# payakorn/InteriorPointMethod

Hardware: AMD Instinct MI355X
Metric: IPM iterations/sec (m=4096,n=8192 dense LP) (higher is better)
Workload: dtype f64; 1 GPU; dense synthetic LP m=4096 n=8192 fp64, seed 0, start x=s=1 y=0 (BASELINE.json configs[1]); replicas per GPU

## Files before the change

### include/ipm_hip.h

```cpp
#ifndef IPM_HIP_H
#define IPM_HIP_H

#include <stddef.h>
#include <stdint.h>

#ifdef __cplusplus
extern "C" {
#endif

#define IPM_ABI_VERSION 4

enum {
    IPM_OK = 0,
    IPM_ERR_INVALID_ARG = -1,
    IPM_ERR_HIP = -2,
    IPM_ERR_NO_DEVICE = -3,
    IPM_ERR_WORKSPACE = -4,
    IPM_ERR_STATE = -5,
    IPM_ERR_INVALID_INPUT = -6,
    IPM_ERR_SINGULAR = -7
};

enum {
    IPM_STATUS_RUNNING = 0,
    IPM_STATUS_CONVERGED = 1,
    IPM_STATUS_MAX_ITER = 2,
    IPM_STATUS_NAN = 3,
    IPM_STATUS_PRIMAL_INFEASIBLE = 5,
    IPM_STATUS_DUAL_INFEASIBLE = 6
};

enum {
    IPM_FLAG_NO_DEVICE_POLLING = 1,
    IPM_FLAG_NO_AUTO_REGULARIZE = 2,
    IPM_FLAG_SINGLE_STREAM = 4,
    IPM_FLAG_SPARSE_FACTOR = 8,
    IPM_FLAG_LOCKSTEP = 16,
    IPM_FLAG_DETECT_INFEASIBILITY = 32
};

typedef struct ipm_handle ipm_handle;

typedef struct ipm_options {
    double eta;
    double pivot_guard_eps;
    double pivot_guard_big;
    int32_t check_every;
    int32_t flags;
    int64_t sparse_nnz;
    double regularize;
} ipm_options;

typedef struct ipm_stats {
    int32_t status;
    int32_t iterations;
    int32_t pivots_fixed;
    int32_t auto_regularized;
    double objective;
    double rp_norm;
    double rd_norm;
    double gap;
    double b_norm, c_norm;
    double mu, mu_aff, sigma;
    double alpha_aff_p, alpha_aff_d;
    double alpha_p, alpha_d;
    double solve_ms;
    double objective_last_finite;
} ipm_stats;

typedef struct ipm_iter_record {
    int32_t k;
    int32_t pivots_fixed;
    double objective, rp_norm, rd_norm, gap, mu, sigma;
    double alpha_aff_p, alpha_aff_d, alpha_p, alpha_d;
} ipm_iter_record;
#define IPM_HISTORY_CAPACITY 1024

int ipm_abi_version(void);
int ipm_device_count(int* count);
void ipm_default_options(ipm_options* opts);

int ipm_workspace_bytes(int64_t m, int64_t n, size_t* bytes);
int ipm_workspace_bytes_csc(int64_t m, int64_t n, int64_t nnz, size_t* bytes);
int ipm_workspace_bytes_opts(int64_t m, int64_t n, const ipm_options* opts, size_t* bytes);

int ipm_create(int device, int64_t m, int64_t n, const ipm_options* opts,
               void* workspace, size_t workspace_bytes, void* stream, ipm_handle** out);
int ipm_destroy(ipm_handle* h);
const char* ipm_last_error(const ipm_handle* h);

int ipm_set_A_dense(ipm_handle* h, const double* A, int64_t ld, int is_device);
int ipm_set_A_csc(ipm_handle* h, const int32_t* colptr, const int32_t* rowind,
                  const double* val, int64_t nnz);
int ipm_set_bc(ipm_handle* h, const double* b, const double* c);

int ipm_set_state(ipm_handle* h, const double* x, const double* y, const double* s);
int ipm_get_state(ipm_handle* h, double* x, double* y, double* s);
int ipm_init_state(ipm_handle* h, double y0);
int ipm_init_state_mehrotra(ipm_handle* h, int32_t* pivots_fixed);

int ipm_set_bounds(ipm_handle* h, const double* u);
int ipm_set_bound_state(ipm_handle* h, const double* w, const double* z);
int ipm_get_bound_state(ipm_handle* h, double* w, double* z);

int ipm_equilibrate(ipm_handle* h, int32_t max_passes, double info[4]);
int ipm_get_scaling(ipm_handle* h, double* r, double* c);

int ipm_newton_direction(ipm_handle* h, int corrector, double* dx, double* dy, double* ds,
                         ipm_stats* stats);

int ipm_iterate(ipm_handle* h, int32_t n_steps, ipm_stats* stats);
int ipm_solve(ipm_handle* h, double tol_p, double tol_d, double tol_gap, int32_t max_iter,
              ipm_stats* stats);
int ipm_solve_batch(ipm_handle** handles, int32_t n, double tol_p, double tol_d, double tol_gap, int32_t max_iter, ipm_stats* stats);
typedef struct ipm_batch ipm_batch;
int ipm_batch_create(int device, void* stream, ipm_batch** out);
int ipm_batch_destroy(ipm_batch* b);
const char* ipm_batch_last_error(const ipm_batch* b);
int ipm_batch_add(ipm_batch* b, ipm_handle* h, double tol_p, double tol_d, double tol_gap, int32_t max_iter, int32_t* index);
int ipm_batch_step(ipm_batch* b, int32_t* finished, int32_t cap, int32_t* n_finished, int32_t* n_active);
int ipm_batch_stats(ipm_batch* b, int32_t index, ipm_stats* stats);
int ipm_solve_small_batch(ipm_handle** handles, int32_t n, double tol_p, double tol_d, double tol_gap, int32_t max_iter, void* stream,
                          ipm_stats* stats);
int ipm_init_small_batch_mehrotra(ipm_handle** handles, int32_t n, void* stream, int32_t* pivots_fixed);
int ipm_set_infeasibility_tol(ipm_handle* h, double eps_p, double eps_d);
int ipm_get_certificate(ipm_handle* h, double* y, double* z, double* x, double info[4]);
int ipm_get_history(ipm_handle* h, ipm_iter_record* out, int32_t capacity, int32_t* count);
int ipm_get_schedule(ipm_handle* h, int32_t out[12]);

int ipm_order_rows(int64_t m, int64_t n, const int32_t* colptr, const int32_t* rowind, int32_t* perm, double info[8]);
int ipm_get_factor_info(ipm_handle* h, int64_t out[8]);

int ipm_solve_linear(ipm_handle* h, const double* B, int64_t ldb, const double* rhs, double* z,
                     int32_t* pivots_fixed);
int ipm_lu_solve(int device, int64_t n, const double* A, int64_t lda, int64_t nrhs, const double* B, int64_t ldb,
                 double* X, int64_t ldx, int64_t* info);
int ipm_lu_factor(int device, int64_t n, const double* A, int64_t lda, double* LU, int64_t ldlu, int32_t* ipiv,
                  int64_t* info);
int ipm_normal_solve(ipm_handle* h, const double* d, const double* rhs, double* z, int reuse_factor,
                     int32_t* pivots_fixed);
int ipm_form_normal_matrix(ipm_handle* h, const double* d, double* B, int64_t ldb);
int ipm_get_factor(ipm_handle* h, double* L, int64_t ldl);
int ipm_set_profiling(ipm_handle* h, int enable);
int ipm_debug_get_stamps(ipm_handle* h, long long* out);
int ipm_debug_ff_schedule(int32_t nblk, int32_t q, int32_t workers, unsigned char* items, int32_t capacity, int32_t* count,
                          int32_t* tile_items, double sim_us[2]);
int ipm_get_phase_ms(ipm_handle* h, double out[4]);
int ipm_debug_get_block_inverse(ipm_handle* h, int32_t k, double* out);
int ipm_debug_ff_trace(ipm_handle* h, long long* out, int64_t capacity, int64_t* count, unsigned char* items, int32_t* nitems);
int ipm_debug_ls_merge(int32_t n, const int32_t* off, const int32_t* types_flat, int32_t max_group, int32_t aligned,
                       int32_t* out_steps, int32_t cap_steps, int32_t* out_members);

#ifdef __cplusplus
}
#endif
#endif
```

### interiorpointmethod_amd/_lib.py

```python
from __future__ import annotations

import ctypes as C
import os

_HERE = os.path.dirname(os.path.abspath(__file__))
LIB_PATH = os.path.join(_HERE, "libipm_hip.so")

EXPORTS = [
    "ipm_abi_version", "ipm_device_count", "ipm_default_options", "ipm_workspace_bytes", "ipm_workspace_bytes_csc", "ipm_workspace_bytes_opts",
    "ipm_create", "ipm_destroy", "ipm_last_error", "ipm_set_A_dense", "ipm_set_A_csc",
    "ipm_set_bc", "ipm_set_state", "ipm_get_state", "ipm_init_state", "ipm_init_state_mehrotra", "ipm_set_bounds", "ipm_set_bound_state", "ipm_get_bound_state", "ipm_equilibrate", "ipm_get_scaling", "ipm_newton_direction",
    "ipm_iterate", "ipm_solve", "ipm_solve_batch", "ipm_solve_small_batch", "ipm_init_small_batch_mehrotra", "ipm_batch_create", "ipm_batch_destroy", "ipm_batch_last_error", "ipm_batch_add", "ipm_batch_step", "ipm_batch_stats", "ipm_get_history", "ipm_set_infeasibility_tol", "ipm_get_certificate", "ipm_get_schedule", "ipm_order_rows", "ipm_get_factor_info", "ipm_solve_linear", "ipm_lu_solve", "ipm_lu_factor", "ipm_normal_solve", "ipm_form_normal_matrix", "ipm_get_factor",
    "ipm_set_profiling", "ipm_get_phase_ms", "ipm_debug_get_stamps", "ipm_debug_ff_schedule", "ipm_debug_ff_trace", "ipm_debug_get_block_inverse", "ipm_debug_ls_merge",
]

IPM_OK = 0
STATUS_RUNNING, STATUS_CONVERGED, STATUS_MAX_ITER, STATUS_NAN = 0, 1, 2, 3
STATUS_PRIMAL_INFEASIBLE, STATUS_DUAL_INFEASIBLE = 5, 6
FLAG_NO_DEVICE_POLLING = 1
FLAG_NO_AUTO_REGULARIZE = 2
FLAG_SINGLE_STREAM = 4
FLAG_SPARSE_FACTOR = 8
FLAG_LOCKSTEP = 16
FLAG_DETECT_INFEASIBILITY = 32
ERR_WORKSPACE = -4
ABI_VERSION = 4
HISTORY_CAPACITY = 1024
ERR_INVALID_INPUT = -6
ERR_SINGULAR = -7


class IpmLibraryError(RuntimeError):
    """libipm_hip.so is missing or does not export the ABI."""


class IpmError(RuntimeError):
    def __init__(self, code, msg):
        super().__init__("libipm_hip status %d: %s" % (code, msg))
        self.code = code


class Options(C.Structure):
    _fields_ = [("eta", C.c_double), ("pivot_guard_eps", C.c_double), ("pivot_guard_big", C.c_double),
                ("check_every", C.c_int32), ("flags", C.c_int32), ("sparse_nnz", C.c_int64),
                ("regularize", C.c_double)]


class Stats(C.Structure):
    _fields_ = [("status", C.c_int32), ("iterations", C.c_int32), ("pivots_fixed", C.c_int32),
                ("auto_regularized", C.c_int32), ("objective", C.c_double), ("rp_norm", C.c_double),
                ("rd_norm", C.c_double), ("gap", C.c_double), ("b_norm", C.c_double),
                ("c_norm", C.c_double), ("mu", C.c_double), ("mu_aff", C.c_double),
                ("sigma", C.c_double), ("alpha_aff_p", C.c_double), ("alpha_aff_d", C.c_double),
                ("alpha_p", C.c_double), ("alpha_d", C.c_double), ("solve_ms", C.c_double),
                ("objective_last_finite", C.c_double)]

    def as_dict(self):
        return {k: getattr(self, k) for k, _ in self._fields_}


class IterRecord(C.Structure):
    _fields_ = [("k", C.c_int32), ("pivots_fixed", C.c_int32), ("objective", C.c_double), ("rp_norm", C.c_double),
                ("rd_norm", C.c_double), ("gap", C.c_double), ("mu", C.c_double), ("sigma", C.c_double),
                ("alpha_aff_p", C.c_double), ("alpha_aff_d", C.c_double), ("alpha_p", C.c_double),
                ("alpha_d", C.c_double)]


_lib = None


def load():
    global _lib
    if _lib is not None:
        return _lib
    try:
        import torch
    except ImportError:
        pass
    if not os.path.exists(LIB_PATH):
        raise IpmLibraryError(
            "%s not found: the HIP extension has not been built. Build it with "
            "`python -c 'import __graft_entry__ as g; g.build()'` (needs hipcc). "
            "There is no CPU fallback." % LIB_PATH)
    try:
        lib = C.CDLL(LIB_PATH)
    except OSError as e:
        raise IpmLibraryError("cannot load %s: %s" % (LIB_PATH, e)) from e
    missing = [s for s in EXPORTS if not hasattr(lib, s)]
    if missing:
        raise IpmLibraryError("%s lacks symbols %s" % (LIB_PATH, missing))
    vp, i32, i64, dbl = C.c_void_p, C.c_int32, C.c_int64, C.c_double
    pd = C.POINTER(C.c_double)
    lib.ipm_abi_version.restype = C.c_int
    lib.ipm_device_count.argtypes = [C.POINTER(C.c_int)]
    lib.ipm_default_options.argtypes = [C.POINTER(Options)]
    lib.ipm_default_options.restype = None
    lib.ipm_workspace_bytes.argtypes = [i64, i64, C.POINTER(C.c_size_t)]
    lib.ipm_workspace_bytes_csc.argtypes = [i64, i64, i64, C.POINTER(C.c_size_t)]
    lib.ipm_workspace_bytes_opts.argtypes = [i64, i64, C.POINTER(Options), C.POINTER(C.c_size_t)]
    lib.ipm_create.argtypes = [C.c_int, i64, i64, C.POINTER(Options), vp, C.c_size_t, vp, C.POINTER(vp)]
    lib.ipm_destroy.argtypes = [vp]
    lib.ipm_last_error.argtypes = [vp]
    lib.ipm_last_error.restype = C.c_char_p
    lib.ipm_set_A_dense.argtypes = [vp, vp, i64, C.c_int]
    lib.ipm_set_A_csc.argtypes = [vp, C.POINTER(i32), C.POINTER(i32), pd, i64]
    lib.ipm_set_bc.argtypes = [vp, pd, pd]
    lib.ipm_set_state.argtypes = [vp, pd, pd, pd]
    lib.ipm_get_state.argtypes = [vp, pd, pd, pd]
    lib.ipm_init_state.argtypes = [vp, dbl]
    lib.ipm_init_state_mehrotra.argtypes = [vp, C.POINTER(i32)]
    lib.ipm_set_bounds.argtypes = [vp, pd]
    lib.ipm_set_bound_state.argtypes = [vp, pd, pd]
    lib.ipm_get_bound_state.argtypes = [vp, pd, pd]
    lib.ipm_equilibrate.argtypes = [vp, i32, pd]
    lib.ipm_get_scaling.argtypes = [vp, pd, pd]
    lib.ipm_newton_direction.argtypes = [vp, C.c_int, pd, pd, pd, C.POINTER(Stats)]
    lib.ipm_iterate.argtypes = [vp, i32, C.POINTER(Stats)]
    lib.ipm_solve.argtypes = [vp, dbl, dbl, dbl, i32, C.POINTER(Stats)]
    lib.ipm_solve_batch.argtypes = [C.POINTER(vp), i32, dbl, dbl, dbl, i32, C.POINTER(Stats)]
    lib.ipm_solve_small_batch.argtypes = [C.POINTER(vp), i32, dbl, dbl, dbl, i32, vp, C.POINTER(Stats)]
    lib.ipm_init_small_batch_mehrotra.argtypes = [C.POINTER(vp), i32, vp, C.POINTER(i32)]
    lib.ipm_batch_create.argtypes = [C.c_int, vp, C.POINTER(vp)]
    lib.ipm_batch_destroy.argtypes = [vp]
    lib.ipm_batch_last_error.argtypes = [vp]
    lib.ipm_batch_last_error.restype = C.c_char_p
    lib.ipm_batch_add.argtypes = [vp, vp, dbl, dbl, dbl, i32, C.POINTER(i32)]
    lib.ipm_batch_step.argtypes = [vp, C.POINTER(i32), i32, C.POINTER(i32), C.POINTER(i32)]
    lib.ipm_batch_stats.argtypes = [vp, i32, C.POINTER(Stats)]
    lib.ipm_get_history.argtypes = [vp, C.POINTER(IterRecord), i32, C.POINTER(i32)]
    lib.ipm_get_schedule.argtypes = [vp, C.POINTER(i32)]
    lib.ipm_set_infeasibility_tol.argtypes = [vp, dbl, dbl]
    lib.ipm_get_certificate.argtypes = [vp, pd, pd, pd, pd]
    lib.ipm_order_rows.argtypes = [i64, i64, C.POINTER(i32), C.POINTER(i32), C.POINTER(i32), pd]
    lib.ipm_get_factor_info.argtypes = [vp, C.POINTER(i64)]
    lib.ipm_solve_linear.argtypes = [vp, pd, i64, pd, pd, C.POINTER(i32)]
    lib.ipm_lu_solve.argtypes = [C.c_int, i64, pd, i64, i64, pd, i64, pd, i64, C.POINTER(i64)]
    lib.ipm_lu_factor.argtypes = [C.c_int, i64, pd, i64, pd, i64, C.POINTER(i32), C.POINTER(i64)]
    lib.ipm_normal_solve.argtypes = [vp, pd, pd, pd, C.c_int, C.POINTER(i32)]
    lib.ipm_form_normal_matrix.argtypes = [vp, pd, pd, i64]
    lib.ipm_get_factor.argtypes = [vp, pd, i64]
    lib.ipm_set_profiling.argtypes = [vp, C.c_int]
    lib.ipm_get_phase_ms.argtypes = [vp, pd]
    lib.ipm_debug_get_stamps.argtypes = [vp, C.POINTER(C.c_longlong)]
    lib.ipm_debug_ff_schedule.argtypes = [i32, i32, i32, C.POINTER(C.c_ubyte), i32, C.POINTER(i32), C.POINTER(i32), pd]
    lib.ipm_debug_get_block_inverse.argtypes = [vp, i32, pd]
    lib.ipm_debug_ff_trace.argtypes = [vp, C.POINTER(C.c_longlong), i64, C.POINTER(i64), C.POINTER(C.c_ubyte), C.POINTER(i32)]
    lib.ipm_debug_ls_merge.argtypes = [i32, C.POINTER(i32), C.POINTER(i32), i32, i32, C.POINTER(i32), i32, C.POINTER(i32)]
    for name in EXPORTS:
        fn = getattr(lib, name)
        if name not in ("ipm_default_options", "ipm_last_error", "ipm_batch_last_error"):
            fn.restype = C.c_int
    _lib = lib
    return lib


def check(handle, code):
    if code != IPM_OK:
        msg = load().ipm_last_error(handle)
        raise IpmError(code, (msg or b"").decode("utf-8", "replace"))


def device_count():
    n = C.c_int(0)
    load().ipm_device_count(C.byref(n))
    return n.value
```

### interiorpointmethod_amd/csrc/handoff.h

```cpp
#pragma once
#include <hip/hip_runtime.h>

namespace ipm {

__device__ unsigned ipm_spin_limit = 1u << 22;

enum { HD_COUNT = 0, HD_TAG, HD_KIND, HD_TARGET, HD_SEEN, HD_WORDS = 8 };
enum HandoffKind : unsigned {
    HK_FCOUNT = 1,
    HK_TPROG = 2,
    HK_LFINAL_ROW = 3,
    HK_LFINAL_COL = 4,
    HK_POTRFDONE = 5,
    HK_ROLES = 6,
    HK_GEMM = 6,
    HK_POTRF = 7,
    HK_DCOUNT = 8,
};

__device__ __forceinline__ unsigned handoff_load(const unsigned* p) { return __hip_atomic_load(p, __ATOMIC_RELAXED, __HIP_MEMORY_SCOPE_AGENT); }

struct HandoffSink { unsigned* timeout; unsigned* dbg; };
template <int SLEEP, bool NULL_OK, class Ready, class Record>
__device__ __forceinline__ bool handoff_wait(Ready ready, HandoffSink sink, Record record) {
    unsigned* const timeout = sink.timeout; unsigned* const dbg = sink.dbg;
    unsigned spins = 0;
    bool ok = true;
    while (!ready()) {
        __builtin_amdgcn_s_sleep(SLEEP);
        ++spins;
        if (spins > ipm_spin_limit || ((spins & 1023u) == 1u && (!NULL_OK || timeout) && handoff_load(timeout))) {
            if (spins > ipm_spin_limit && dbg && __hip_atomic_fetch_add(dbg + HD_COUNT, 1u, __ATOMIC_RELAXED, __HIP_MEMORY_SCOPE_AGENT) == 0u) record();
            if (!NULL_OK || timeout) __hip_atomic_store(timeout, 1u, __ATOMIC_RELAXED, __HIP_MEMORY_SCOPE_AGENT);
            ok = false;
            break;
        }
    }
    return ok;
}

__device__ __forceinline__ void handoff_record_ge(unsigned* dbg, unsigned tag, unsigned kind, unsigned target, const unsigned* p) {
    dbg[HD_TAG] = tag; dbg[HD_KIND] = kind; dbg[HD_TARGET] = target; dbg[HD_SEEN] = handoff_load(p);
}

template <int SLEEP, bool NULL_OK>
__device__ __forceinline__ bool handoff_wait_ge(const unsigned* p, unsigned count, HandoffSink sink, unsigned tag, unsigned kind) {
    return handoff_wait<SLEEP, NULL_OK>([=] { return handoff_load(p) >= count; }, sink, [=] { handoff_record_ge(sink.dbg, tag, kind, count, p); });
}

template <bool WAIT = true>
__device__ __forceinline__ void handoff_acquire() {
    __builtin_amdgcn_fence(__ATOMIC_ACQUIRE, "agent");
    if (WAIT) asm volatile("s_waitcnt vmcnt(0)" ::: "memory");
}
__device__ __forceinline__ void handoff_acquire_barrier(bool polled) {
    if (polled) handoff_acquire();
    __syncthreads();
}

__device__ __forceinline__ void handoff_publish_begin() {
    asm volatile("s_waitcnt vmcnt(0)" ::: "memory");
    __syncthreads();
    if (threadIdx.x == 0) {
        __builtin_amdgcn_fence(__ATOMIC_RELEASE, "agent");
        asm volatile("s_waitcnt vmcnt(0)" ::: "memory");
    }
}

__device__ __forceinline__ bool handoff_skipped(const int* done, unsigned* signal) {
    if (done && *done) {
        if (signal && threadIdx.x == 0) __hip_atomic_fetch_add(signal, 1u, __ATOMIC_RELAXED, __HIP_MEMORY_SCOPE_AGENT);
        return true;
    }
    return false;
}

}
```

### interiorpointmethod_amd/csrc/host_factor_solve.h

```cpp
#pragma once
static inline bool sp_on(const ipm_handle* h) { return h->spf && !h->spf_off; }
static inline bool sp_level(const ipm_handle* h) {
    if (h->sp_serial || h->sp_level_mode < 0) return false;
    if (h->sp_level_mode > 0 || (h->opt.flags & IPM_FLAG_NO_DEVICE_POLLING)) return true;
    return !alone_on_device(h);
}
static inline unsigned sp_launch_grid(ipm_handle* h) {
    if (h->sp_serial) { ++h->sp_serial_launches; return 1u; }
    return (unsigned)h->sp_grid;
}
template <class Launch>
static void sp_walk(ipm_handle* h, bool by_level, bool leaves_first, Launch launch) {
    if (!by_level) { launch(sp_launch_grid(h), h->spF.rec, 0); return; }
    const size_t nlev = h->sp_lvlptr.empty() ? 0 : h->sp_lvlptr.size() - 1;
    for (size_t i = 0; i < nlev; ++i) {
        const size_t l = leaves_first ? i : nlev - 1 - i;
        const int cnt = h->sp_lvlptr[l + 1] - h->sp_lvlptr[l];
        launch((unsigned)std::min(cnt, h->sp_grid), h->sp_rec_level + h->sp_lvlptr[l], cnt);
    }
}

static int ensure_dense_B(ipm_handle* h) {
    if (h->B && h->invD) return IPM_OK;
    if (!h->no_dense) return fail(h, IPM_ERR_STATE, "handle has no dense normal-matrix buffer");
    if ((!h->B_own && dev_malloc(h->device, h->stream, (void**)&h->B_own, sizeof(double) * (size_t)h->mp * h->mp) != hipSuccess) ||
        (!h->invD_own && dev_malloc(h->device, h->stream, (void**)&h->invD_own, sizeof(double) * (size_t)h->nblk * NB * NB) != hipSuccess))
        return fail(h, IPM_ERR_HIP, "dense normal-matrix buffer (%lld x %lld doubles) could not be allocated", (long long)h->mp, (long long)h->mp);
    HIP_TRY(h, hipMemsetAsync(h->invD_own, 0, sizeof(double) * (size_t)h->nblk * NB * NB, h->stream));
    h->B = h->B_own; h->invD = h->invD_own;
    return IPM_OK;
}

static int enqueue_form(ipm_handle* h, const double* d, bool dense_image = false) {
    if (sp_on(h) && !dense_image) {
        hipLaunchKernelGGL(sp_form_kernel, dim3((unsigned)((h->sp_nslot + 255) / 256)), dim3(256), 0, h->stream, h->sp_fptr, h->sp_fcol,
                           h->sp_fcoef, h->sp_nslot, d, h->spF.L, &h->sc->maxdiag, &h->sc->done);
        hipLaunchKernelGGL(sp_maxdiag_kernel, dim3((unsigned)((h->m + 255) / 256)), dim3(256), 0, h->stream, h->spF.L, h->sp_diagpos, (int)h->m, &h->sc->maxdiag,
                           &h->sc->done);
        HIP_TRY(h, hipGetLastError());
        return IPM_OK;
    }
    if (int rc_ = ensure_dense_B(h)) return rc_;
    if (h->sparse && h->list_form) {
        const int64_t nB = h->mp * h->mp;
        const unsigned zgrid = (unsigned)std::min<int64_t>((nB / 2 + 255) / 256, 4096);
        launch_twin<LS_ZERO>(h, zgrid, {h->B, nB, &h->sc->done});
        const int work = h->sm_nb + (int)(h->mp - h->m);
        launch_twin<LS_ADAT_LIST>(h, (unsigned)((work + 255) / 256), {h->sm_bptr, h->ls_bi, h->ls_bk, h->sm_bcol, h->sm_bcoef, h->ls_bak, h->sm_nb, d, h->B, h->mp, (int)h->m, (int)h->mp, &h->sc->done});
        HIP_TRY(h, hipGetLastError());
        return IPM_OK;
    }
    if (h->sparse) {
        const LsAdatSp ps{sparse_view(h), d, h->B, h->mp, (int)h->mp, &h->sc->done};
        if (h->mp <= SP_LDS_MAX_MP) launch_twin<LS_ADAT_SPARSE>(h, (unsigned)h->mp, ps, nullptr, (unsigned)(h->mp * sizeof(double)));
        else launch_twin<LS_ADAT_SPARSE_GLOBAL>(h, (unsigned)h->mp, ps);
        HIP_TRY(h, hipGetLastError());
        return IPM_OK;
    }
    HIP_TRY(h, launch_adat_syrk(h->A, h->np, d, h->B, h->mp, (int)h->mp, (int)h->np, (int)h->m, factor_done(h),
                                h->d_tile_order, h->stream, h->slab, 512));
    return IPM_OK;
}

static int enqueue_group_inverses(ipm_handle* h, int g0 = 0, int g1 = -1, hipStream_t st = nullptr) {
    if (sp_on(h)) return IPM_OK;
    if (!h->grouped_trsv) return IPM_OK;
    const int GS = h->gsz;
    const int64_t GR = (int64_t)GS * 128;
    if (g1 < 0) g1 = h->nblk / GS;
    if (!st) st = h->stream;
    const int nG = g1 - g0;
    if (nG <= 0) return IPM_OK;
    const int* done = &h->sc->done;
    launch_twin<LS_GROUP_DIAG_T>(h, 16u * (unsigned)(nG * GS), {h->invD, h->gXT, h->gX, g0 * GS, GS, done}, st);
    const int64_t gXs = GR * GR, gL = GR * (h->mp + 1), gSs = (GR / 2) * (GR / 2);
    double* gXT = h->gXT + g0 * gXs; double* gX = h->gX + g0 * gXs; double* gS = h->gS + g0 * gSs;
    const double* Lg = h->B + g0 * gL;
    for (int hs = 128; hs < GR; hs *= 2) {
        const int np = (int)(GR / (2 * hs));
        GemmNT t = gemm_defaults();
        t.done = done;
        t.M = hs; t.N = hs; t.K = hs; t.batch = np; t.batch2 = nG;
        const int64_t pX = (int64_t)2 * hs * (GR + 1);
        const int64_t pL = (int64_t)2 * hs * (h->mp + 1);
        const int64_t pS = (int64_t)hs * hs;
        GemmNT a = t;
        a.P = gXT; a.ldp = GR; a.sP = pX; a.sP2 = gXs;
        a.Q = Lg + (int64_t)hs * h->mp; a.ldq = h->mp; a.sQ = pL; a.sQ2 = gL;
        a.C = gS; a.ldc = hs; a.sC = pS; a.sC2 = gSs;
        HIP_TRY(h, (launch_gemm_nt<32, 32, 32, 2, 2>(a, st)));
        GemmNT b = t;
        b.P = gX + (int64_t)hs * GR + hs; b.ldp = GR; b.sP = pX; b.sP2 = gXs;
        b.Q = gS; b.ldq = hs; b.sQ = pS; b.sQ2 = gSs;
        b.C = gX + (int64_t)hs * GR; b.ldc = GR; b.sC = pX; b.sC2 = gXs; b.alpha = -1.0;
        HIP_TRY(h, (launch_gemm_nt<32, 32, 32, 2, 2>(b, st)));
        GemmNT c = t;
        c.P = gS; c.ldp = hs; c.sP = pS; c.sP2 = gSs;
        c.Q = gX + (int64_t)hs * GR + hs; c.ldq = GR; c.sQ = pX; c.sQ2 = gXs;
        c.C = gXT + hs; c.ldc = GR; c.sC = pX; c.sC2 = gXs; c.alpha = -1.0;
        HIP_TRY(h, (launch_gemm_nt<32, 32, 32, 2, 2>(c, st)));
    }
    HIP_TRY(h, hipGetLastError());
    return IPM_OK;
}

static inline int potrf_panels(const ipm_handle* h, int k) {
    if (h->shift_rel != 0.0) return NB / 16;
    const int64_t real = h->m - (int64_t)k * NB;
    return real >= NB ? NB / 16 : (int)std::max<int64_t>(1, (real + 15) / 16);
}

static int enqueue_factor(ipm_handle* h, bool use_env = false, int mid_step = -1, int ginv_step = -1, const double* sp_fwd_rhs = nullptr) {
    if (sp_on(h)) {
        if (!h->sp_fuse_fwd) sp_fwd_rhs = nullptr;
        h->sp_fwd_fused = sp_fwd_rhs;
        const unsigned ep = ++h->sp_epoch;
        sp_walk(h, sp_level(h), true, [&](unsigned grid, const SpRec* recs, int count) {
            hipLaunchKernelGGL((sp_chol_kernel<SPC_THREADS>), dim3(grid), dim3(SPC_THREADS), h->sp_lds_chol, h->stream, h->spF, ep,
                               &h->sc->maxdiag, h->opt.pivot_guard_eps, h->opt.pivot_guard_big, h->shift_rel, &h->sc->fixed,
                               h->sp_lds_doubles, recs, count, sp_fwd_rhs, h->t2, h->sp_fv_off);
        });
        HIP_TRY(h, hipGetLastError());
        return IPM_OK;
    }
    if (int rc_ = ensure_dense_B(h)) return rc_;
    const int* done = factor_done(h);
    use_env = use_env && h->use_env;
    launch_twin<LS_MAXDIAG>(h, 1u, {h->B, h->mp, (int)h->m, &h->sc->maxdiag, done});
    const bool la = lookahead_on(h);
    int gs = 1;
    if (la && !use_env && h->two_level != 0) {
        if (h->group_steps > 0) gs = h->nblk >= 8 ? h->group_steps : 1;
        else if (h->nblk >= 96) gs = 4;
        else if (h->nblk >= 48) gs = 3;
    }
    std::vector<int> grp_lo(h->nblk), grp_hi(h->nblk);
    for (int k = 0; k < h->nblk; ++k) {
        if (gs > 1) { grp_lo[k] = (k / gs) * gs; grp_hi[k] = std::min(grp_lo[k] + gs, h->nblk); }
        else { grp_lo[k] = k; grp_hi[k] = k + 1; }
    }
    h->last_gs = gs;
    hipStream_t sm = h->stream, sb = la ? h->stream2 : h->stream;
    const bool fs = polls_device(h);
    h->n_counter_steps = 0; h->n_event_steps = 0;
    std::vector<unsigned> bulk_wgs(h->nblk, 0u);
    if (la) {
        if (fs) HIP_TRY(h, hipMemsetAsync(h->d_bulk_done, 0, sizeof(unsigned) * 2 * (size_t)h->nblk, sm));
        HIP_TRY(h, hipEventRecord(h->ev_fork, sm));
        HIP_TRY(h, hipStreamWaitEvent(sb, h->ev_fork, 0));
    }
    for (int k = 0; k < h->nblk; ++k) {
        PotrfDiag pd;
        pd.Bkk = h->B + (int64_t)k * NB * (h->mp + 1); pd.ld = h->mp;
        pd.inv = h->invD + (int64_t)k * NB * NB;
        pd.maxdiag = &h->sc->maxdiag; pd.eps = h->opt.pivot_guard_eps; pd.big = h->opt.pivot_guard_big; pd.shift_rel = h->shift_rel;
        pd.fixed = &h->sc->fixed; pd.done = done; pd.stamps = nullptr;
        pd.wait_on = nullptr; pd.wait_count = 0; pd.signal = nullptr; pd.timeout = nullptr; pd.dbg = nullptr; pd.dbg_tag = 0;
        pd.trace = nullptr;
        pd.nt = potrf_panels(h, k);
        pd.rows = (int)(h->m - (int64_t)k * NB);
        if (h->stamp_buf && k == 0) {
            pd.stamps = h->stamp_buf;
            if (getenv("IPM_POTRF_SKIP")) pd.dbg_tag = (unsigned)atoi(getenv("IPM_POTRF_SKIP"));
            launch_untwinned(h, potrf_diag_kernel<true>, dim3(1), dim3(PD_THREADS), sm, pd);
        } else launch_twin<LS_POTRF>(h, 1u, pd, sm);
        if (k == ginv_step) {
            HIP_TRY(h, hipEventRecord(h->ev_grp, sm));
            HIP_TRY(h, hipStreamWaitEvent(h->stream3, h->ev_grp, 0));
            int rc_ = enqueue_group_inverses(h, 0, (k + 1) / h->gsz, h->stream3);
            if (rc_) return rc_;
        }
        if (k == mid_step) { int rc_ = enqueue_residual_stream(h, sm); if (rc_) return rc_; }
        int rem = (int)(h->mp - (int64_t)(k + 1) * NB);
        if (rem <= 0) break;
        if (use_env) {
            rem = std::min(rem, (h->env_last[k] - k) * NB);
            if (rem <= 0) {
                if (la) HIP_TRY(h, hipEventRecord(h->ev_bulk[k], sb));
                continue;
            }
        }
        double* panel = h->B + (int64_t)(k + 1) * NB * h->mp + (int64_t)k * NB;
        GemmNT t = gemm_defaults();
        t.P = panel; t.ldp = h->mp; t.Q = pd.inv; t.ldq = NB;
        t.C = panel; t.ldc = h->mp; t.M = rem; t.N = NB; t.K = NB;
        t.lower = 0; t.done = done;
        GemmNT u = gemm_defaults();
        u.P = panel; u.ldp = h->mp; u.Q = panel; u.ldq = h->mp;
        u.C = h->B + (int64_t)(k + 1) * NB * (h->mp + 1); u.ldc = h->mp; u.M = rem; u.N = rem; u.K = NB;
        u.alpha = -1.0; u.beta = 1.0; u.lower = 1; u.done = done;
        if (!la) {
            if (rem <= h->ss_small_blocks * NB) {
                HIP_TRY(h, (launch_gemm_nt<32, 128, 32, 1, 8>(t, sm)));
                HIP_TRY(h, (launch_gemm_nt<64, 64, 16, 2, 2>(u, sm)));
                continue;
            }
            HIP_TRY(h, (launch_gemm_nt<64, 128, 16, 2, 2>(t, sm)));
            if (h->bulk_variant == 7) HIP_TRY(h, (launch_gemm_nt<128, 128, 16, 2, 2>(u, sm)));
            else HIP_TRY(h, launch_chol_update(u, sm));
            continue;
        }
        GemmNT tc = t; tc.M = NB;
        if (k >= 1) {
            if (bulk_wgs[k - 1] > 0) { tc.wait_on = h->d_bulk_done + (k - 1); tc.wait_count = bulk_wgs[k - 1]; tc.timeout = timeout_word(h); }
            else HIP_TRY(h, hipStreamWaitEvent(sm, h->ev_bulk[k - 1], 0));
        }
        const int tb_wgs = (rem - NB) / 64;
        const bool crit_flag = fs && rem > NB && tb_wgs <= 64;
        if (crit_flag) tc.signal = h->d_bulk_done + h->nblk + k;
        HIP_TRY(h, (launch_gemm_nt<32, 128, 32, 1, 8>(tc, sm)));
        if (!crit_flag) HIP_TRY(h, hipEventRecord(h->ev_crit[k], sm));
        const int g0 = grp_lo[k], gend = grp_hi[k];
        const bool grouped = gend - g0 > 1;
        const bool grp_inner = grouped && k + 1 < gend;
        const bool grp_last = grouped && !grp_inner;
        if (grp_last && k > g0) {
            u.P = panel - (int64_t)(k - g0) * NB; u.Q = u.P; u.K = (k - g0 + 1) * NB;
        }
        GemmNT uc = u; uc.M = NB; uc.N = NB;
        HIP_TRY(h, (launch_gemm_nt<32, 32, 32, 2, 2>(uc, sm)));
        if (!crit_flag) HIP_TRY(h, hipStreamWaitEvent(sb, h->ev_crit[k], 0));
        if (rem > NB) {
            GemmNT tb = t; tb.C = panel + (int64_t)NB * h->mp; tb.P = tb.C; tb.M = rem - NB;
            if (crit_flag) { tb.wait_on = h->d_bulk_done + h->nblk + k; tb.wait_count = NB / 32; tb.timeout = timeout_word(h); }
            HIP_TRY(h, (launch_gemm_nt<64, 128, 16, 2, 2>(tb, sb)));
            GemmNT ub = u;
            const int nt = rem / NB;
            if (grp_inner) {
                const int wn = gend - (k + 1);
                ub.P = panel + (int64_t)NB * h->mp; ub.Q = panel;
                ub.C = h->B + (int64_t)(k + 2) * NB * h->mp + (int64_t)(k + 1) * NB;
                ub.M = rem - NB; ub.N = std::min(wn * NB, rem); ub.lower = 0;
                if (fs) { bulk_wgs[k] = (unsigned)((ub.M / NB) * (ub.N / NB)); ub.signal = h->d_bulk_done + k; ++h->n_counter_steps; }
                else ++h->n_event_steps;
                if (h->bulk_variant == 7) HIP_TRY(h, (launch_gemm_nt<128, 128, 16, 2, 2>(ub, sb)));
                else HIP_TRY(h, launch_chol_update(ub, sb));
                HIP_TRY(h, hipEventRecord(h->ev_bulk[k], sb));
                continue;
            }
            const int ub_wgs = nt * (nt + 1) / 2 - 1;
            if (fs && ub_wgs <= 1024) {
                bulk_wgs[k] = (unsigned)ub_wgs;
                ub.signal = h->d_bulk_done + k;
                ++h->n_counter_steps;
            } else ++h->n_event_steps;
            if (h->bulk_variant == 7) HIP_TRY(h, (launch_gemm_nt<128, 128, 16, 2, 2>(ub, sb, nullptr, 512, 1)));
            else HIP_TRY(h, launch_chol_update(ub, sb, 1));
        }
        HIP_TRY(h, hipEventRecord(h->ev_bulk[k], sb));
    }
    if (la) HIP_TRY(h, hipStreamWaitEvent(sm, h->ev_bulk[h->nblk - 2], 0));
    HIP_TRY(h, hipGetLastError());
    return IPM_OK;
}

static void launch_dense_gemv_n(ipm_handle* h, const double* A, int64_t lda, int rows, int cols, const double* v, double sa,
                                double sb, const double* add, double* out) {
    launch_twin<LS_GEMV_N>(h, (unsigned)((rows + 3) / 4), {A, lda, rows, cols, v, sa, sb, add, out, &h->sc->done});
}

static void enqueue_block_steps(ipm_handle* h, int k0, double* r, double* z, double* out) {
    TrsvStep a;
    a.L = h->B; a.ld = h->mp; a.inv = h->invD; a.done = &h->sc->done;
    a.r = r; a.z = z; a.j0 = 0;
    for (int k = k0; k < h->nblk; ++k) {
        a.k = k;
        const int nb = h->use_env ? h->env_last[k] - k + 1 : h->nblk - k;
        launch_twin<LS_TRSV_FWD>(h, (unsigned)nb, a);
    }
    a.r = z; a.z = out;
    for (int k = h->nblk - 1; k >= k0; --k) {
        a.k = k;
        a.j0 = h->use_env ? h->env_first[k] : 0;
        launch_twin<LS_TRSV_BWD>(h, (unsigned)(k - a.j0 + 1), a);
    }
}

static int enqueue_potrs_grouped(ipm_handle* h, double* r, double* out, hipEvent_t wait_last = nullptr) {
    const int GS = h->gsz;
    const int GR = GS * 128;
    const int nG = h->nblk / GS;
    const int* done = &h->sc->done;
    double* z = h->t2;
    for (int g = 0; g < nG; ++g) {
        if (wait_last && g == nG - 1) HIP_TRY(h, hipStreamWaitEvent(h->stream, wait_last, 0));
        launch_dense_gemv_n(h, h->gX + (int64_t)g * GR * GR, GR, GR, GR, r + (int64_t)g * GR, 1.0, 0.0, nullptr, z + (int64_t)g * GR);
        int below = (int)(h->mp - (int64_t)(g + 1) * GR);
        if (h->use_env) below = std::min(below, (int)((int64_t)(h->env_last[(g + 1) * GS - 1] + 1) * NB - (int64_t)(g + 1) * GR));
        if (below > 0) {
            double* rb = r + (int64_t)(g + 1) * GR;
            launch_dense_gemv_n(h, h->B + (int64_t)(g + 1) * GR * h->mp + (int64_t)g * GR, h->mp, below, GR, z + (int64_t)g * GR, -1.0, 1.0,
                                rb, rb);
        }
    }
    enqueue_block_steps(h, nG * GS, r, z, out);
    for (int g = nG - 1; g >= 0; --g) {
        launch_dense_gemv_n(h, h->gXT + (int64_t)g * GR * GR, GR, GR, GR, z + (int64_t)g * GR, 1.0, 0.0, nullptr, out + (int64_t)g * GR);
        int left = g * GR;
        const int c0 = h->use_env ? std::min(left, h->env_first[g * GS] * NB) : 0;
        left -= c0;
        if (left > 0) {
            const unsigned gx = (unsigned)((left + 511) / 512);
            launch_twin<LS_GEMV_T>(h, gx * 16u, {h->B + (int64_t)g * GR * h->mp + c0, h->mp, GR / 16, left, out + (int64_t)g * GR, h->gPart, done, gx});
            launch_twin<LS_SUB_PARTIALS>(h, (unsigned)((left + 255) / 256), {z + c0, h->gPart, left, 16, done});
        }
    }
    HIP_TRY(h, hipGetLastError());
    return IPM_OK;
}

static int enqueue_potrs(ipm_handle* h, double* r, double* out, hipEvent_t wait_last = nullptr) {
    if (sp_on(h)) {
        const int rm = std::max(16, h->sp_rmax);
        unsigned ep = ++h->sp_epoch;
        const bool fwd_done = h->sp_fwd_fused != nullptr && h->sp_fwd_fused == r;
        h->sp_fwd_fused = nullptr;
        const bool by_level = sp_level(h);
        if (!fwd_done) sp_walk(h, by_level, true, [&](unsigned grid, const SpRec* recs, int count) {
            hipLaunchKernelGGL((sp_fwd_kernel<SPC_THREADS>), dim3(grid), dim3(SPC_THREADS), h->sp_lds_solve, h->stream, h->spF, ep, r, h->t2, rm, recs, count);
        });
        if (!by_level) ep = ++h->sp_epoch;
        sp_walk(h, by_level, false, [&](unsigned grid, const SpRec* recs, int count) {
            hipLaunchKernelGGL((sp_bwd_kernel<SPC_THREADS>), dim3(grid), dim3(SPC_THREADS), 0, h->stream, h->spF, ep, h->t2, out, recs, count);
        });
        HIP_TRY(h, hipGetLastError());
        return IPM_OK;
    }
    if (h->grouped_trsv) return enqueue_potrs_grouped(h, r, out, wait_last);
    if (wait_last) HIP_TRY(h, hipStreamWaitEvent(h->stream, wait_last, 0));
    enqueue_block_steps(h, 0, r, h->t2, out);
    HIP_TRY(h, hipGetLastError());
    return IPM_OK;
}

static int enqueue_mehrotra_start(ipm_handle* h) {
    int rc;
    const unsigned gn = (unsigned)((h->n + 255) / 256);
    hipLaunchKernelGGL(fill_kernel, dim3(gn), dim3(256), 0, h->stream, h->d, (int)h->n, 1.0);
    if ((rc = enqueue_form(h, h->d))) return rc;
    if ((rc = enqueue_factor(h, true))) return rc;
    if ((rc = enqueue_group_inverses(h))) return rc;
    const VecArgs va = vec_args(h);
    const dim3 g(h->vblk), b(VBLK);
    HIP_TRY(h, hipMemcpyAsync(h->t1, h->b, sizeof(double) * h->mp, hipMemcpyDeviceToDevice, h->stream));
    if ((rc = enqueue_potrs(h, h->t1, h->dy))) return rc;
    launch_gemv_t(h, h->dy);
    if (h->bnd) hipLaunchKernelGGL(start_primal_bounded_kernel, g, b, 0, h->stream, va, bnd_args(h));
    else hipLaunchKernelGGL(start_primal_kernel, g, b, 0, h->stream, va);
    launch_gemv_n(h, h->c, 1.0, 0.0, nullptr, h->t1);
    if ((rc = enqueue_potrs(h, h->t1, h->dy))) return rc;
    launch_gemv_t(h, h->dy);
    if (h->bnd) {
        const BndArgs bd = bnd_args(h);
        hipLaunchKernelGGL(start_dual_bounded_kernel, g, b, 0, h->stream, va, bd);
        hipLaunchKernelGGL(start_shift_bounded_kernel, g, b, 0, h->stream, va, bd);
        hipLaunchKernelGGL(start_primal_correct_bounded_kernel, g, b, 0, h->stream, va, bd);
        hipLaunchKernelGGL(start_dual_correct_bounded_kernel, g, b, 0, h->stream, va, bd);
    } else {
        hipLaunchKernelGGL(start_dual_kernel, g, b, 0, h->stream, va);
        hipLaunchKernelGGL(start_shift_kernel, g, b, 0, h->stream, va);
        hipLaunchKernelGGL(start_primal_correct_kernel, g, b, 0, h->stream, va);
        hipLaunchKernelGGL(start_dual_correct_kernel, g, b, 0, h->stream, va);
    }
    HIP_TRY(h, hipGetLastError());
    return IPM_OK;
}
```

### interiorpointmethod_amd/csrc/host_handle.h

```cpp
#pragma once
static thread_local char g_err[512] = "";

static const int MAX_DEVICES = 64;
static std::atomic<int> g_live[MAX_DEVICES];
static std::atomic<bool> g_attr_set[MAX_DEVICES];

struct ipm_handle {
    int device = 0;
    hipStream_t stream = nullptr;
    bool own_stream = false;
    hipStream_t stream2 = nullptr;
    hipStream_t stream3 = nullptr;
    hipEvent_t ev_mid = nullptr, ev_res = nullptr, ev_grp = nullptr, ev_last = nullptr;
    std::vector<hipEvent_t> ev_crit, ev_bulk;
    hipEvent_t ev_fork = nullptr;
    int lookahead = 1;
    int grouped_trsv = 1;
    int gsz = 0;
    double *gXT = nullptr, *gX = nullptr, *gS = nullptr, *gPart = nullptr;
    unsigned* d_bulk_done = nullptr;
    bool no_dense = false;
    double* B_own = nullptr; double* invD_own = nullptr;
    int group_steps = 0;
    int two_level = 1;
    int bulk_variant = 0;
    int ss_small_blocks = 16;
    int flag_sync = 1;
    int last_gs = 1, n_counter_steps = 0, n_event_steps = 0, timeouts_recovered = 0;
    bool counted = false;
    bool small = false;
    int fused_small = 1;
    bool list_form = false;
    int list_form_opt = 1;
    int *ls_bi = nullptr, *ls_bk = nullptr;
    double* ls_bak = nullptr;
    int sm_nb = 0;
    int *sm_bptr = nullptr, *sm_bcol = nullptr;
    unsigned short *sm_bi = nullptr, *sm_bk = nullptr;
    double* sm_bcoef = nullptr;
    bool spf = false;
    bool spf_off = false;
    bool sp_serial = false;
    SpFactor spF;
    std::vector<void*> sp_allocs;
    int *sp_fptr = nullptr, *sp_fcol = nullptr;
    double* sp_fcoef = nullptr;
    long long* sp_diagpos = nullptr;
    long long sp_nslot = 0, sp_nu = 0, sp_terms = 0;
    int sp_height = 0, sp_rmax = 0, sp_grid = 1, sp_serial_launches = 0, sp_nvirtual = 0;
    size_t sp_lds_chol = 0, sp_lds_solve = 0;
    int sp_fv_off = 0;
    int sp_fuse_fwd = 1;
    const double* sp_fwd_fused = nullptr;
    int sp_lds_doubles = 16, sp_threads = 256;
    int sp_level_mode = 0;
    std::vector<int> sp_lvlptr;
    SpRec* sp_rec_level = nullptr;
    unsigned sp_epoch = 0;
    double shift_rel = 0.0;
    int auto_reg = 0;
    unsigned* d_flags = nullptr;
    int64_t m = 0, n = 0, mp = 0, np = 0;
    int nblk = 0, rc_chunks = 0, rows_per_chunk = 0, vblk = 0;
    ipm_options opt;
    void* ws = nullptr;
    size_t ws_bytes = 0;
    bool own_ws = false;
    double *A = nullptr, *B = nullptr, *invD = nullptr;
    double *x = nullptr, *s = nullptr, *c = nullptr, *rc = nullptr, *d = nullptr, *v = nullptr, *q = nullptr;
    double *dxa = nullptr, *dsa = nullptr, *dx = nullptr, *ds = nullptr;
    double *y = nullptr, *b = nullptr, *rb = nullptr, *t1 = nullptr, *t2 = nullptr, *dya = nullptr, *dy = nullptr;
    double *atp = nullptr, *part = nullptr, *slab = nullptr;
    int ff_enabled = 1;
    int ff_min_nblk = 16, ff_max_nblk = 72;
    bool ff_forced = false;
    bool ff_ref_engine = false;
    int ff_q = 4;
    int ff_workers = 0;
    int* d_ff_tile_items = nullptr;
    int ff_qmax = 16;
    bool ff_built = false, ff_last = false;
    FFSchedule ff_sched;
    FFItem* d_ff_items = nullptr;
    unsigned* d_ff_flags = nullptr;
    size_t ff_flag_words = 0;
    double* ff_slab = nullptr;
    long long* ff_trace = nullptr;
    long long* ff_prof = nullptr;
    const int* fdone = nullptr;
    std::vector<int> env_last, env_first;
    bool use_env = false;
    int envelope = 1;
    bool sparse = false;
    int64_t nnz_cap = 0, nnz = 0;
    int* d_tile_order = nullptr;
    int *d_rowptr = nullptr, *d_colind = nullptr, *d_colptr = nullptr, *d_rowind = nullptr;
    double *d_rval = nullptr, *d_cval = nullptr;
    long long* stamp_buf = nullptr;
    unsigned* ff_potrfdone = nullptr;
    Scalars* sc = nullptr;
    IterRec* hist = nullptr;
    double* snap = nullptr;
    bool bnd = false;
    int bnd_nU = 0;
    double* bnd_mem = nullptr;
    bool detect = false;
    double det_eps_p = 1e-8, det_eps_d = 1e-8;
    double* det = nullptr;
    double* cert_mem = nullptr;
    bool scaled = false;
    std::vector<double> eq_r, eq_c;
    int* fixed = nullptr;
    Scalars* h_sc = nullptr;
    bool haveA = false, haveBC = false, haveState = false, predictor_valid = false;
    bool fresh_state = true;
    int profiling = 0;
    double phase_ms[4] = {0, 0, 0, 0};
    hipEvent_t ev0 = nullptr, ev1 = nullptr;
    std::vector<struct LsLaunch>* ls_rec = nullptr;
    bool ls_cut = false;
    int lockstep = 0;
    unsigned spin_limit = 1u << 22;
    bool ragged_groups = true;
    bool ls_block_steps = false, potrf_stamps = false, ff_chain_mode0 = false;
    char err[512] = "";
};
struct LsLaunch { int type; LsRec rec; };
template <LsType T> static void record_twin(ipm_handle* h, unsigned gridx, const LsArgs<T>& a, unsigned lds = 0) {
    LsLaunch L{};
    L.type = T; L.rec.gridx = gridx; L.rec.lds = lds;
    memcpy(L.rec.args, &a, sizeof a);
    h->ls_rec->push_back(L);
}
template <LsType T> static void launch_twin(ipm_handle* h, unsigned grid, const LsArgs<T>& a, hipStream_t st = nullptr, unsigned lds = 0) {
    if (h->ls_rec) record_twin<T>(h, grid, a, lds);
    else LsTwin<T>::single(a, grid, lds, st ? st : h->stream);
}
template <class... P, class... Q> static void launch_untwinned(ipm_handle* h, void (*kernel)(P...), dim3 grid, dim3 block, hipStream_t st, const Q&... args) {
    if (h->ls_rec) h->ls_cut = true;
    else hipLaunchKernelGGL(kernel, grid, block, 0, st ? st : h->stream, args...);
}

static int vfail(char* err, int code, const char* fmt, va_list ap) {
    char buf[512];
    vsnprintf(buf, sizeof buf, fmt, ap);
    snprintf(g_err, sizeof g_err, "%s", buf);
    if (err) snprintf(err, 512, "%s", buf);
    return code;
}
static int fail(ipm_handle* h, int code, const char* fmt, ...) { va_list ap; va_start(ap, fmt); code = vfail(h ? h->err : nullptr, code, fmt, ap); va_end(ap); return code; }

#define HIP_TRY(h, call)                                                                      \
    do {                                                                                      \
        hipError_t e_ = (call);                                                               \
        if (e_ != hipSuccess)                                                                 \
            return fail((h), IPM_ERR_HIP, "%s failed: %s (%s:%d)", #call, hipGetErrorString(e_), \
                        __FILE__, __LINE__);                                                  \
    } while (0)

static inline int64_t round_up(int64_t v, int64_t q) { return (v + q - 1) / q * q; }

static inline int live_on_device(const ipm_handle* h) { return h->device < MAX_DEVICES ? g_live[h->device].load(std::memory_order_acquire) : 1; }
static inline bool alone_on_device(const ipm_handle* h) { return live_on_device(h) <= 1; }
static inline bool lookahead_on(const ipm_handle* h) { return h->lookahead != 0 && h->nblk > 2 && h->stream2 != nullptr; }
static inline bool wants_polling(const ipm_handle* h) { return lookahead_on(h) && h->flag_sync != 0; }
static inline bool polls_device(const ipm_handle* h) { return wants_polling(h) && alone_on_device(h); }
static inline unsigned* timeout_word(const ipm_handle* h) { return h->d_flags + 2 * (size_t)h->nblk; }
static inline const int* factor_done(const ipm_handle* h) { return h->fdone ? h->fdone : &h->sc->done; }

static std::atomic<int> g_pool_state[64];
static hipMemPool_t g_pool[64];
static std::mutex g_pool_mutex;
static bool async_alloc_ok(int device) {
    if (device < 0 || device >= 64) return false;
    int st = g_pool_state[device].load(std::memory_order_acquire);
    if (st == 0) {
        std::lock_guard<std::mutex> lock(g_pool_mutex);
        st = g_pool_state[device].load(std::memory_order_acquire);
        if (st != 0) return st == 1;
        int supported = 0;
        if (hipDeviceGetAttribute(&supported, hipDeviceAttributeMemoryPoolsSupported, device) == hipSuccess && supported) {
            hipMemPoolProps props;
            memset(&props, 0, sizeof props);
            props.allocType = hipMemAllocationTypePinned;
            props.handleTypes = hipMemHandleTypeNone;
            props.location.type = hipMemLocationTypeDevice;
            props.location.id = device;
            hipMemPool_t pool = nullptr;
            if (hipMemPoolCreate(&pool, &props) == hipSuccess && pool) {
                uint64_t keep = (uint64_t)2 << 30;
                (void)hipMemPoolSetAttribute(pool, hipMemPoolAttrReleaseThreshold, &keep);
                g_pool[device] = pool;
                st = 1;
            }
        }
        if (st == 0) st = 2;
        g_pool_state[device].store(st, std::memory_order_release);
    }
    return st == 1;
}
static hipError_t dev_malloc(int device, hipStream_t stream, void** p, size_t bytes) {
    if (bytes == 0) bytes = 16;
    if (async_alloc_ok(device)) return hipMallocFromPoolAsync(p, bytes, g_pool[device], stream);
    return hipMalloc(p, bytes);
}
static void dev_free(int device, hipStream_t stream, void* p) {
    if (!p) return;
    if (async_alloc_ok(device)) (void)hipFreeAsync(p, stream); else (void)hipFree(p);
}
static std::mutex g_hsc_mutex;
static std::vector<Scalars*> g_hsc_pool;

static GemmNT gemm_defaults() {
    GemmNT g;
    memset(&g, 0, sizeof g);
    g.alpha = 1.0; g.unit_diag_from = -1; g.batch = 1; g.batch2 = 1;
    return g;
}

struct Layout {
    int64_t mp, np;
    int nblk, rc_chunks, rows_per_chunk, vblk;
    size_t off_A, off_B, off_inv, off_nvec, off_mvec, off_atp, off_part, off_det, off_sc, off_fixed, off_hist, off_snap, off_slab, total;
    size_t off_rowptr, off_colind, off_rval, off_colptr, off_rowind, off_cval, off_order;
};
static const int N_NVEC = 11;
static const int N_MVEC = 7;

static bool layout_no_dense(int64_t m, int64_t sparse_nnz, unsigned flags) { return sparse_nnz > 0 && (flags & IPM_FLAG_SPARSE_FACTOR) && m > 128; }
static Layout make_layout(int64_t m, int64_t n, int64_t sparse_nnz = 0, bool no_dense = false) {
    Layout L;
    L.mp = round_up(m, NB);
    {
        const int64_t nb = L.mp / NB, nb8 = round_up(nb, 8);
        if (nb >= 16 && (nb8 - nb) * 8 <= nb) L.mp = nb8 * NB;
    }
    L.np = round_up(n, 64);
    L.nblk = (int)(L.mp / NB);
    int64_t c64 = L.mp / 64;
    L.rc_chunks = (int)(c64 <= 32 ? c64 : 32);
    while (L.mp % L.rc_chunks) --L.rc_chunks;
    L.rows_per_chunk = (int)(L.mp / L.rc_chunks);
    while ((int64_t)L.rc_chunks * L.rows_per_chunk < L.mp) ++L.rows_per_chunk;
    int64_t mx = m > n ? m : n;
    int64_t vb = (mx + VBLK - 1) / VBLK;
    L.vblk = (int)(vb < 1 ? 1 : (vb > MAXPART ? MAXPART : vb));
    size_t off = 0;
    auto take = [&](size_t bytes) { size_t o = off; off += (bytes + 255) / 256 * 256; return o; };
    if (sparse_nnz > 0) { L.rc_chunks = 1; L.rows_per_chunk = (int)L.mp; }
    L.off_A = take(sparse_nnz > 0 ? 0 : sizeof(double) * L.mp * L.np);
    L.off_B = take(no_dense ? 0 : sizeof(double) * L.mp * L.mp);
    L.off_inv = take(no_dense ? 0 : sizeof(double) * L.nblk * NB * NB);
    L.off_nvec = take(sizeof(double) * L.np * N_NVEC);
    L.off_mvec = take(sizeof(double) * L.mp * N_MVEC);
    L.off_atp = take(sizeof(double) * L.rc_chunks * L.np);
    L.off_part = take(sizeof(double) * P_NSLOT_DETECT * MAXPART);
    L.off_det = take(sizeof(double) * 4);
    L.off_sc = take(sizeof(Scalars));
    L.off_fixed = take(256);
    L.off_hist = take(sizeof(IterRec) * HIST_CAP);
    L.off_snap = take(sizeof(double) * (2 * L.np + L.mp) + sizeof(Scalars));
    L.off_slab = take(no_dense ? 0 : sizeof(double) * (size_t)kSlabTiles * 128 * 128);
    L.off_order = take(sizeof(int) * ((size_t)L.nblk * (L.nblk + 1) / 2));
    L.off_rowptr = take(sparse_nnz > 0 ? sizeof(int) * (m + 1) : 0);
    L.off_colptr = take(sparse_nnz > 0 ? sizeof(int) * (n + 1) : 0);
    L.off_colind = take(sparse_nnz > 0 ? sizeof(int) * sparse_nnz : 0);
    L.off_rowind = take(sparse_nnz > 0 ? sizeof(int) * sparse_nnz : 0);
    L.off_rval = take(sparse_nnz > 0 ? sizeof(double) * sparse_nnz : 0);
    L.off_cval = take(sparse_nnz > 0 ? sizeof(double) * sparse_nnz : 0);
    L.total = off;
    return L;
}

__global__ void set_params_kernel(Scalars* sc, double e1, double e2, double e3, double eta, int max_iter,
                                  int force, int reset) { start_solve(sc, e1, e2, e3, eta, max_iter, force, reset); }

static VecArgs vec_args(ipm_handle* h) {
    VecArgs a;
    a.m = (int)h->m; a.n = (int)h->n; a.np = (int)h->np; a.rc_chunks = h->rc_chunks; a.nblk = h->vblk;
    a.atp = h->atp; a.x = h->x; a.y = h->y; a.s = h->s; a.b = h->b; a.c = h->c;
    a.rb = h->rb; a.rc = h->rc; a.d = h->d; a.v = h->v; a.q = h->q;
    a.dxa = h->dxa; a.dya = h->dya; a.dsa = h->dsa; a.dx = h->dx; a.dy = h->dy; a.ds = h->ds;
    a.part = h->part; a.sc = h->sc; a.hist = h->hist;
    return a;
}

static SparseA sparse_view(const ipm_handle* h) {
    SparseA A;
    A.rowptr = h->d_rowptr; A.colind = h->d_colind; A.rval = h->d_rval;
    A.colptr = h->d_colptr; A.rowind = h->d_rowind; A.cval = h->d_cval;
    A.m = (int)h->m; A.n = (int)h->n;
    return A;
}

static const int BND_VECS = 10;
static BndArgs bnd_args(ipm_handle* h) {
    const size_t np = (size_t)h->np;
    double* p = h->bnd_mem;
    BndArgs b;
    b.u = p; b.w = p + np; b.z = p + 2 * np; b.dwa = p + 3 * np; b.dza = p + 4 * np; b.dw = p + 5 * np; b.dz = p + 6 * np;
    b.qz = p + 7 * np; b.nU = h->bnd_nU;
    return b;
}

static DetArgs det_args(const ipm_handle* h) { return DetArgs{h->det_eps_p, h->det_eps_d, h->det}; }
```

### interiorpointmethod_amd/csrc/host_iteration.h

```cpp
#pragma once
static int enqueue_solve_direction(ipm_handle* h, hipEvent_t* ev, double* dy, int corr, hipEvent_t wait_last = nullptr) {
    if (ev) HIP_TRY(h, hipEventRecord(ev[0], h->stream));
    int rc = enqueue_potrs(h, h->t1, dy, wait_last);
    if (rc) return rc;
    if (ev) HIP_TRY(h, hipEventRecord(ev[1], h->stream));
    launch_gemv_t(h, dy);
    launch_direction(h, corr);
    HIP_TRY(h, hipGetLastError());
    return IPM_OK;
}
static int enqueue_predictor(ipm_handle* h, hipEvent_t* ev, bool have_rhs = false, hipEvent_t wait_last = nullptr) {
    if (!have_rhs) launch_gemv_n(h, h->v, -1.0, -1.0, h->rb, h->t1);
    return enqueue_solve_direction(h, ev, h->dya, 0, wait_last);
}
static int enqueue_corrector(ipm_handle* h, hipEvent_t* ev) {
    launch_mu_aff(h);
    launch_corrector_rhs(h);
    launch_gemv_n(h, h->v, -1.0, -1.0, h->rb, h->t1);
    return enqueue_solve_direction(h, ev, h->dy, 1);
}

static const int EV_PER_IT = 9;

static int enqueue_iteration(ipm_handle* h, hipEvent_t* ev) {
    int rc;
    const bool all = ev && h->profiling >= 2;
    if (overlap_residuals(h)) {
        launch_scaling(h);
        const bool fused = ff_use(h);
        if (ev && !fused) HIP_TRY(h, hipEventRecord(ev[1], h->stream));
        struct Latch { ipm_handle* h; ~Latch() { h->fdone = nullptr; } } latch{h};
        h->fdone = &h->sc->done_f;
        h->ff_last = false;
        if (!fused) {
            if ((rc = enqueue_form(h, h->d))) return rc;
            if (ev) HIP_TRY(h, hipEventRecord(ev[2], h->stream));
        }
        const int rstep = h->nblk * 13 / 16;
        const int nG = h->grouped_trsv ? h->nblk / h->gsz : 0;
        const int gstep = (nG >= 2 && (nG - 1) * h->gsz - 1 < rstep) ? (nG - 1) * h->gsz - 1 : -1;
        if (fused) { if ((rc = enqueue_form_factor(h, ev, rstep, gstep))) return rc; }
        else if ((rc = enqueue_factor(h, true, rstep, gstep))) return rc;
        h->fdone = nullptr;
        if (gstep >= 0) {
            if (h->ff_last && h->ff_potrfdone) {
                hipLaunchKernelGGL(ff_gate_kernel, dim3(1), dim3(64), 0, h->stream3, h->ff_potrfdone + (h->nblk - 1), 1u, timeout_word(h), &h->sc->done);
            } else {
                HIP_TRY(h, hipEventRecord(h->ev_grp, h->stream));
                HIP_TRY(h, hipStreamWaitEvent(h->stream3, h->ev_grp, 0));
            }
            if ((rc = enqueue_group_inverses(h, nG - 1, nG, h->stream3))) return rc;
            HIP_TRY(h, hipEventRecord(h->ev_last, h->stream3));
            HIP_TRY(h, hipStreamWaitEvent(h->stream, h->ev_res, 0));
            if ((rc = enqueue_predictor(h, nullptr, true, h->ev_last))) return rc;
        } else {
            if ((rc = enqueue_group_inverses(h, 0, nG, nullptr))) return rc;
            HIP_TRY(h, hipStreamWaitEvent(h->stream, h->ev_res, 0));
            if ((rc = enqueue_predictor(h, nullptr, true))) return rc;
        }
        if ((rc = enqueue_corrector(h, nullptr))) return rc;
        launch_update(h);
        HIP_TRY(h, hipGetLastError());
        return IPM_OK;
    }
    if (all) HIP_TRY(h, hipEventRecord(ev[0], h->stream));
    if ((rc = enqueue_residuals(h))) return rc;
    h->ff_last = false;
    bool have_rhs = false;
    if (h->profiling < 2 && ff_use(h)) {
        if ((rc = enqueue_form_factor(h, ev, -1, -1))) return rc;
    } else {
        if (ev) HIP_TRY(h, hipEventRecord(ev[1], h->stream));
        if ((rc = enqueue_form(h, h->d))) return rc;
        if (ev) HIP_TRY(h, hipEventRecord(ev[2], h->stream));
        if (sp_on(h) && h->sp_fuse_fwd) {
            launch_gemv_n(h, h->v, -1.0, -1.0, h->rb, h->t1);
            have_rhs = true;
            if ((rc = enqueue_factor(h, true, -1, -1, h->t1))) return rc;
        } else if ((rc = enqueue_factor(h, true))) return rc;
    }
    if ((rc = enqueue_group_inverses(h))) return rc;
    if (all) HIP_TRY(h, hipEventRecord(ev[3], h->stream));
    if ((rc = enqueue_predictor(h, all ? ev + 4 : nullptr, have_rhs))) return rc;
    if ((rc = enqueue_corrector(h, all ? ev + 6 : nullptr))) return rc;
    launch_update(h);
    HIP_TRY(h, hipGetLastError());
    if (all) HIP_TRY(h, hipEventRecord(ev[8], h->stream));
    return IPM_OK;
}

static int read_scalars(ipm_handle* h, bool* timed_out = nullptr) {
    unsigned tmo = 0;
    unsigned* word = timeout_word(h);
    HIP_TRY(h, hipMemcpyAsync(h->h_sc, h->sc, sizeof(Scalars), hipMemcpyDeviceToHost, h->stream));
    HIP_TRY(h, hipMemcpyAsync(&tmo, word, sizeof(unsigned), hipMemcpyDeviceToHost, h->stream));
    HIP_TRY(h, hipStreamSynchronize(h->stream));
    if (tmo) {
        if (h->stream2) HIP_TRY(h, hipStreamSynchronize(h->stream2));
        if (h->ff_built && h->ff_last && getenv("IPM_FF_DEBUG")) ff_dump_handoffs(h);
        HIP_TRY(h, hipMemsetAsync(word, 0, sizeof(unsigned), h->stream));
        if (!timed_out) return fail(h, IPM_ERR_HIP, "a device-side hand-off poll timed out (persistent solve)");
    }
    if (timed_out) *timed_out = tmo != 0;
    return IPM_OK;
}

static void poll_fallback(ipm_handle* h) {
    if (h->spf) h->sp_serial = true;
    if (h->ff_last) h->ff_enabled = 0;
    else h->flag_sync = 0;
    ++h->timeouts_recovered;
}

__global__ __launch_bounds__(256) void snapshot_kernel(double* x, double* y, double* s, Scalars* sc, double* snap, int np,
                                                       int mp, int restore) {
    const int gid = blockIdx.x * 256 + threadIdx.x, gsz = gridDim.x * 256;
    double *sx = snap, *ss = snap + np, *sy = snap + 2 * (size_t)np;
    Scalars* ssc = (Scalars*)(snap + 2 * (size_t)np + mp);
    if (restore) {
        for (int j = gid; j < np; j += gsz) { x[j] = sx[j]; s[j] = ss[j]; }
        for (int i = gid; i < mp; i += gsz) y[i] = sy[i];
        if (gid == 0) *sc = *ssc;
    } else {
        for (int j = gid; j < np; j += gsz) { sx[j] = x[j]; ss[j] = s[j]; }
        for (int i = gid; i < mp; i += gsz) sy[i] = y[i];
        if (gid == 0) *ssc = *sc;
    }
}
__global__ __launch_bounds__(256) void snapshot_bounds_kernel(double* w, double* z, double* sw, double* sz, int np, int restore) {
    const int gid = blockIdx.x * 256 + threadIdx.x, gsz = gridDim.x * 256;
    for (int j = gid; j < np; j += gsz) {
        if (restore) { w[j] = sw[j]; z[j] = sz[j]; }
        else { sw[j] = w[j]; sz[j] = z[j]; }
    }
}
static int enqueue_snapshot(ipm_handle* h, int restore, hipStream_t st = nullptr) {
    const int64_t mx = h->np > h->mp ? h->np : h->mp;
    const unsigned grid = (unsigned)std::min<int64_t>((mx + 255) / 256, 256);
    hipLaunchKernelGGL(snapshot_kernel, dim3(grid), dim3(256), 0, st ? st : h->stream, h->x, h->y, h->s, h->sc, h->snap, (int)h->np,
                       (int)h->mp, restore);
    if (h->bnd) {
        const BndArgs b = bnd_args(h);
        double* sw = h->bnd_mem + 8 * (size_t)h->np;
        hipLaunchKernelGGL(snapshot_bounds_kernel, dim3(grid), dim3(256), 0, st ? st : h->stream, b.w, b.z, sw, sw + h->np, (int)h->np, restore);
    }
    HIP_TRY(h, hipGetLastError());
    return IPM_OK;
}
static bool may_poll(const ipm_handle* h) { return (h->spf && !h->sp_serial && !sp_level(h)) || wants_polling(h); }

static void fill_stats(ipm_handle* h, ipm_stats* st, double ms) {
    if (!st) return;
    const Scalars& s = *h->h_sc;
    memset(st, 0, sizeof *st);
    st->status = s.status; st->iterations = s.k; st->pivots_fixed = s.fixed; st->auto_regularized = h->auto_reg;
    st->objective_last_finite = s.obj_last_finite;
    st->objective = s.obj; st->rp_norm = s.rb_norm; st->rd_norm = s.rc_norm; st->gap = s.gap;
    st->b_norm = s.b_norm; st->c_norm = s.c_norm; st->mu = s.mu; st->mu_aff = s.mu_aff; st->sigma = s.sigma;
    st->alpha_aff_p = s.alpha_aff_p; st->alpha_aff_d = s.alpha_aff_d; st->alpha_p = s.alpha_p; st->alpha_d = s.alpha_d;
    st->solve_ms = ms;
}

static int check_ready(ipm_handle* h, const char* who) {
    if (!h) return fail(h, IPM_ERR_INVALID_ARG, "%s: NULL handle", who);
    if (!h->haveA || !h->haveBC || !h->haveState) return fail(h, IPM_ERR_STATE, "%s: A, (b,c) and a state must be set first", who);
    return IPM_OK;
}

extern "C" int ipm_newton_direction(ipm_handle* h, int corrector, double* dx, double* dy, double* ds, ipm_stats* stats) {
    int rc = check_ready(h, "ipm_newton_direction");
    if (rc) return rc;
    HIP_TRY(h, hipSetDevice(h->device));
    if (!corrector) {
        for (int attempt = 0;; ++attempt) {
            hipLaunchKernelGGL(set_params_kernel, dim3(1), dim3(1), 0, h->stream, h->sc, 1e-8, 1e-8, 1e-8, h->opt.eta, 1 << 30, 1, 0);
            if ((rc = enqueue_residuals(h))) return rc;
            if ((rc = enqueue_form(h, h->d))) return rc;
            if ((rc = enqueue_factor(h, true))) return rc;
            if ((rc = enqueue_group_inverses(h))) return rc;
            if ((rc = enqueue_predictor(h, nullptr))) return rc;
            launch_mu_aff(h);
            bool tmo = false;
            if ((rc = read_scalars(h, &tmo))) return rc;
            if (!tmo) break;
            if (attempt) return fail(h, IPM_ERR_HIP, "hand-off time-out persists with stream events");
            poll_fallback(h);
        }
        h->predictor_valid = true;
        if (dx) HIP_TRY(h, hipMemcpyAsync(dx, h->dxa, sizeof(double) * h->n, hipMemcpyDeviceToHost, h->stream));
        if (dy) HIP_TRY(h, hipMemcpyAsync(dy, h->dya, sizeof(double) * h->m, hipMemcpyDeviceToHost, h->stream));
        if (ds) HIP_TRY(h, hipMemcpyAsync(ds, h->dsa, sizeof(double) * h->n, hipMemcpyDeviceToHost, h->stream));
    } else {
        if (!h->predictor_valid) return fail(h, IPM_ERR_STATE, "corrector requested without a predictor at this state");
        if ((rc = enqueue_corrector(h, nullptr))) return rc;
        if (dx) HIP_TRY(h, hipMemcpyAsync(dx, h->dx, sizeof(double) * h->n, hipMemcpyDeviceToHost, h->stream));
        if (dy) HIP_TRY(h, hipMemcpyAsync(dy, h->dy, sizeof(double) * h->m, hipMemcpyDeviceToHost, h->stream));
        if (ds) HIP_TRY(h, hipMemcpyAsync(ds, h->ds, sizeof(double) * h->n, hipMemcpyDeviceToHost, h->stream));
    }
    if (corrector && (rc = read_scalars(h))) return rc;
    HIP_TRY(h, hipStreamSynchronize(h->stream));
    eq_out(h, dx, h->eq_c, false); eq_out(h, dy, h->eq_r, false); eq_out(h, ds, h->eq_c, true);
    fill_stats(h, stats, 0.0);
    return IPM_OK;
}

static SmallLP small_args(ipm_handle* h, int max_steps, int auto_reg) {
    SmallLP a;
    a.A = sparse_view(h); a.m = (int)h->m; a.n = (int)h->n; a.nt = (int)((h->m + 15) / 16);
    a.bptr = h->sm_bptr; a.bi = h->sm_bi; a.bk = h->sm_bk; a.bcol = h->sm_bcol; a.bcoef = h->sm_bcoef; a.nb = h->sm_nb;
    a.x = h->x; a.y = h->y; a.s = h->s; a.b = h->b; a.c = h->c;
    a.rc = h->rc; a.d = h->d; a.v = h->v; a.q = h->q; a.dxa = h->dxa; a.dsa = h->dsa; a.dx = h->dx; a.ds = h->ds;
    a.sc = h->sc; a.hist = h->hist;
    a.eps = h->opt.pivot_guard_eps; a.big = h->opt.pivot_guard_big; a.shift_rel = h->shift_rel;
    a.max_steps = max_steps; a.auto_reg = auto_reg;
    return a;
}

static int small_variant(const ipm_handle* h) { return (h->bnd ? SMALL_BOUNDED : 0) | (h->detect ? SMALL_DETECT : 0); }
static SmallItem small_item(ipm_handle* h, int index, int max_steps, int auto_reg) {
    SmallItem it;
    memset(&it, 0, sizeof it);
    it.lp = small_args(h, max_steps, auto_reg);
    if (h->bnd) it.bd = bnd_args(h);
    it.dt = det_args(h);
    it.eta = h->opt.eta;
    it.variant = small_variant(h);
    it.index = index;
    return it;
}
static void launch_small(int v, hipStream_t S, const SmallItem* one, const SmallItem* d_items, unsigned grid) {
    const dim3 g(one ? 1u : grid), b(PD_THREADS);
    if (v == SMALL_PLAIN) { if (one) hipLaunchKernelGGL(small_lp_kernel, g, b, 0, S, one->lp); else hipLaunchKernelGGL(small_lp_batch_kernel, g, b, 0, S, d_items); }
    else if (v == SMALL_BOUNDED) { if (one) hipLaunchKernelGGL(small_lp_bounded_kernel, g, b, 0, S, one->lp, one->bd); else hipLaunchKernelGGL(small_lp_batch_bounded_kernel, g, b, 0, S, d_items); }
    else if (v == SMALL_DETECT) { if (one) hipLaunchKernelGGL(small_lp_detect_kernel, g, b, 0, S, one->lp, one->dt); else hipLaunchKernelGGL(small_lp_batch_detect_kernel, g, b, 0, S, d_items); }
    else { if (one) hipLaunchKernelGGL(small_lp_bounded_detect_kernel, g, b, 0, S, one->lp, one->bd, one->dt); else hipLaunchKernelGGL(small_lp_batch_bounded_detect_kernel, g, b, 0, S, d_items); }
}

static int enqueue_small(ipm_handle* h, int max_steps, int auto_reg) {
    const SmallItem it = small_item(h, 0, max_steps, auto_reg);
    launch_small(it.variant, h->stream, &it, nullptr, 1);
    HIP_TRY(h, hipGetLastError());
    return IPM_OK;
}

static void launch_small_start(bool bounded, hipStream_t S, const SmallItem* one, const SmallItem* d_items, unsigned grid) {
    const dim3 g(one ? 1u : grid), b(PD_THREADS);
    if (!bounded) { if (one) hipLaunchKernelGGL(small_start_kernel, g, b, 0, S, one->lp); else hipLaunchKernelGGL(small_start_batch_kernel, g, b, 0, S, d_items); }
    else { if (one) hipLaunchKernelGGL(small_start_bounded_kernel, g, b, 0, S, one->lp, one->bd); else hipLaunchKernelGGL(small_start_batch_bounded_kernel, g, b, 0, S, d_items); }
}

static void mark_fresh_state(ipm_handle* h) {
    h->haveState = true; h->predictor_valid = false; h->fresh_state = true;
    h->h_sc->status = 0;
}

extern "C" int ipm_init_state_mehrotra(ipm_handle* h, int32_t* pivots_fixed) {
    if (!h) return fail(h, IPM_ERR_INVALID_ARG, "ipm_init_state_mehrotra: NULL handle");
    if (!h->haveA) return fail(h, IPM_ERR_STATE, "ipm_init_state_mehrotra: A not set");
    if (!h->haveBC) return fail(h, IPM_ERR_STATE, "ipm_init_state_mehrotra: (b, c) not set");
    HIP_TRY(h, hipSetDevice(h->device));
    int rc;
    for (int attempt = 0;; ++attempt) {
        hipLaunchKernelGGL(set_params_kernel, dim3(1), dim3(1), 0, h->stream, h->sc, 1e-8, 1e-8, 1e-8, h->opt.eta, 1 << 30, 1, 1);
        if (h->small) {
            const SmallItem it = small_item(h, 0, 0, 0);
            launch_small_start(h->bnd, h->stream, &it, nullptr, 1);
            HIP_TRY(h, hipGetLastError());
        } else if ((rc = enqueue_mehrotra_start(h))) return rc;
        bool tmo = false;
        if ((rc = read_scalars(h, &tmo))) return rc;
        if (!tmo) break;
        if (attempt) return fail(h, IPM_ERR_HIP, "hand-off time-out persists with stream events");
        poll_fallback(h);
    }
    if (pivots_fixed) *pivots_fixed = h->h_sc->fixed;
    mark_fresh_state(h);
    return IPM_OK;
}

extern "C" int ipm_iterate(ipm_handle* h, int32_t n_steps, ipm_stats* stats) {
    int rc = check_ready(h, "ipm_iterate");
    if (rc) return rc;
    if (n_steps < 0) return fail(h, IPM_ERR_INVALID_ARG, "n_steps < 0");
    HIP_TRY(h, hipSetDevice(h->device));
    h->predictor_valid = false;
    std::vector<hipEvent_t> evs;
    struct EvGuard {
        std::vector<hipEvent_t>& v;
        ~EvGuard() { for (auto& e : v) if (e) (void)hipEventDestroy(e); }
    } guard{evs};
    if (h->profiling) {
        evs.assign((size_t)EV_PER_IT * n_steps, nullptr);
        for (auto& e : evs) HIP_TRY(h, hipEventCreate(&e));
    }
    float ms = 0.f;
    const int reset_k = h->fresh_state ? 1 : 0;
    h->fresh_state = false;
    if (h->small && !h->profiling) {
        hipLaunchKernelGGL(set_params_kernel, dim3(1), dim3(1), 0, h->stream, h->sc, 1e-8, 1e-8, 1e-8, h->opt.eta, 1 << 30, 1, reset_k);
        HIP_TRY(h, hipEventRecord(h->ev0, h->stream));
        if ((rc = enqueue_small(h, n_steps, 0))) return rc;
        HIP_TRY(h, hipEventRecord(h->ev1, h->stream));
        if ((rc = read_scalars(h))) return rc;
        HIP_TRY(h, hipEventElapsedTime(&ms, h->ev0, h->ev1));
        fill_stats(h, stats, ms);
        return IPM_OK;
    }
    for (int attempt = 0;; ++attempt) {
        hipLaunchKernelGGL(set_params_kernel, dim3(1), dim3(1), 0, h->stream, h->sc, 1e-8, 1e-8, 1e-8, h->opt.eta, 1 << 30, 1,
                           attempt == 0 ? reset_k : 0);
        const bool guard_poll = may_poll(h) && n_steps > 0;
        if (guard_poll && (rc = enqueue_snapshot(h, 0))) return rc;
        HIP_TRY(h, hipEventRecord(h->ev0, h->stream));
        for (int it = 0; it < n_steps; ++it)
            if ((rc = enqueue_iteration(h, h->profiling ? &evs[(size_t)it * EV_PER_IT] : nullptr))) return rc;
        if ((rc = enqueue_residuals(h))) return rc;
        HIP_TRY(h, hipEventRecord(h->ev1, h->stream));
        bool tmo = false;
        if ((rc = read_scalars(h, &tmo))) return rc;
        if (!tmo) break;
        if (attempt >= 2 || !guard_poll) return fail(h, IPM_ERR_HIP, "hand-off time-out persists with stream events");
        poll_fallback(h);
        if ((rc = enqueue_snapshot(h, 1))) return rc;
    }
    HIP_TRY(h, hipEventElapsedTime(&ms, h->ev0, h->ev1));
    if (h->profiling && n_steps > 0) {
        double ph[4] = {0, 0, 0, 0};
        for (int it = 0; it < n_steps; ++it) {
            hipEvent_t* e = &evs[(size_t)it * EV_PER_IT];
            float f = 0.f, total = 0.f;
            (void)hipEventElapsedTime(&f, e[1], e[2]); ph[0] += f;
            if (h->profiling < 2) continue;
            (void)hipEventElapsedTime(&f, e[2], e[3]); ph[1] += f;
            float s1 = 0.f, s2 = 0.f;
            (void)hipEventElapsedTime(&s1, e[4], e[5]); (void)hipEventElapsedTime(&s2, e[6], e[7]); ph[2] += s1 + s2;
            (void)hipEventElapsedTime(&total, e[0], e[8]);
            float f12 = 0.f, f23 = 0.f;
            (void)hipEventElapsedTime(&f12, e[1], e[2]); (void)hipEventElapsedTime(&f23, e[2], e[3]);
            ph[3] += total - f12 - f23 - s1 - s2;
        }
        for (int i = 0; i < 4; ++i) h->phase_ms[i] = ph[i] / n_steps;
    }
    fill_stats(h, stats, ms);
    return IPM_OK;
}

extern "C" int ipm_solve(ipm_handle* h, double tol_p, double tol_d, double tol_gap, int32_t max_iter, ipm_stats* stats) {
    int rc = check_ready(h, "ipm_solve");
    if (rc) return rc;
    if (max_iter < 0) return fail(h, IPM_ERR_INVALID_ARG, "max_iter < 0");
    HIP_TRY(h, hipSetDevice(h->device));
    h->predictor_valid = false; h->fresh_state = false;
    if (h->auto_reg) { h->auto_reg = 0; h->shift_rel = h->opt.regularize; }
    hipLaunchKernelGGL(set_params_kernel, dim3(1), dim3(1), 0, h->stream, h->sc, tol_p, tol_d, tol_gap, h->opt.eta, max_iter, 0, 1);
    HIP_TRY(h, hipEventRecord(h->ev0, h->stream));
    const int chunk = h->opt.check_every;
    const bool may_auto = h->opt.regularize == 0.0 && !(h->opt.flags & IPM_FLAG_NO_AUTO_REGULARIZE);
    if (h->small) {
        if ((rc = enqueue_small(h, 1 << 30, may_auto ? 1 : 0))) return rc;
        if ((rc = read_scalars(h))) return rc;
        if (h->h_sc->status == IPM_STATUS_NEEDS_SHIFT) {
            h->shift_rel = 1e-14; h->auto_reg = 1;
            hipLaunchKernelGGL(set_params_kernel, dim3(1), dim3(1), 0, h->stream, h->sc, tol_p, tol_d, tol_gap, h->opt.eta, max_iter, 0, 1);
            if ((rc = enqueue_small(h, 1 << 30, 0))) return rc;
            if ((rc = read_scalars(h))) return rc;
        }
        HIP_TRY(h, hipEventRecord(h->ev1, h->stream));
        HIP_TRY(h, hipEventSynchronize(h->ev1));
        float ms_ = 0.f;
        HIP_TRY(h, hipEventElapsedTime(&ms_, h->ev0, h->ev1));
        fill_stats(h, stats, ms_);
        return IPM_OK;
    }
    bool first = true;
    int recovered = 0;
    for (;;) {
        const bool snap = first || may_poll(h);
        if (snap && (rc = enqueue_snapshot(h, 0))) return rc;
        for (int i = 0; i < chunk; ++i)
            if ((rc = enqueue_iteration(h, nullptr))) return rc;
        bool tmo = false;
        if ((rc = read_scalars(h, &tmo))) return rc;
        if (tmo) {
            if (!snap || ++recovered > 2) return fail(h, IPM_ERR_HIP, "hand-off time-out persists with stream events");
            poll_fallback(h);
            if ((rc = enqueue_snapshot(h, 1))) return rc;
            continue;
        }
        if (first && may_auto && h->h_sc->k > 0 && (double)h->h_sc->fixed_first > 0.05 * (double)h->m) {
            h->shift_rel = 1e-14; h->auto_reg = 1;
            if ((rc = enqueue_snapshot(h, 1))) return rc;
            first = false;
            continue;
        }
        first = false;
        if (h->h_sc->done) break;
    }
    HIP_TRY(h, hipEventRecord(h->ev1, h->stream));
    HIP_TRY(h, hipEventSynchronize(h->ev1));
    float ms = 0.f;
    HIP_TRY(h, hipEventElapsedTime(&ms, h->ev0, h->ev1));
    fill_stats(h, stats, ms);
    return IPM_OK;
}
```

### interiorpointmethod_amd/csrc/host_residuals.h

```cpp
#pragma once
static void launch_gemv_n(ipm_handle* h, const double* v, double sa, double sb, const double* add, double* out,
                          hipStream_t st = nullptr) {
    if (h->sparse) launch_twin<LS_SPMV_CSR>(h, (unsigned)((h->mp + 15) / 16), {sparse_view(h), (int)h->mp, v, sa, sb, add, out, &h->sc->done}, st);
    else launch_untwinned(h, gemv_n_kernel, dim3((unsigned)(h->mp / 4)), dim3(256), st, h->A, h->np, (int)h->mp, (int)h->np, v, sa, sb, add, out, &h->sc->done);
}
static void launch_gemv_t(ipm_handle* h, const double* u, hipStream_t st = nullptr) {
    if (h->sparse) launch_twin<LS_SPMV_CSC_T>(h, (unsigned)((h->np + 15) / 16), {sparse_view(h), (int)h->np, u, h->atp, &h->sc->done}, st);
    else launch_untwinned(h, gemv_t_kernel, dim3((unsigned)((h->np + 511) / 512), (unsigned)h->rc_chunks), dim3(256), st, h->A, h->np, h->rows_per_chunk, (int)h->np, u, h->atp, &h->sc->done);
}

template <LsType T> static void launch_vec_step(ipm_handle* h, void (*bounded)(VecArgs, BndArgs), hipStream_t st = nullptr) {
    if (h->bnd) launch_untwinned(h, bounded, dim3(h->vblk), dim3(VBLK), st, vec_args(h), bnd_args(h));
    else launch_twin<T>(h, (unsigned)h->vblk, {vec_args(h), 0}, st);
}
static void launch_prepare(ipm_handle* h, hipStream_t st) {
    if (h->bnd && h->detect) launch_untwinned(h, prepare_bounded_detect_kernel, dim3(h->vblk), dim3(VBLK), st, vec_args(h), bnd_args(h));
    else if (h->detect) launch_twin<LS_PREPARE_DETECT>(h, (unsigned)h->vblk, {vec_args(h), det_args(h)}, st);
    else launch_vec_step<LS_PREPARE>(h, prepare_bounded_kernel, st);
}
static void launch_stop_test(ipm_handle* h, hipStream_t st) {
    if (h->bnd && h->detect) launch_untwinned(h, stop_test_bounded_detect_kernel, dim3(1), dim3(64), st, vec_args(h), bnd_args(h), det_args(h));
    else if (h->bnd) launch_untwinned(h, stop_test_bounded_kernel, dim3(1), dim3(64), st, vec_args(h), bnd_args(h));
    else if (h->detect) launch_twin<LS_STOP_TEST_DETECT>(h, 1u, {vec_args(h), det_args(h)}, st);
    else launch_twin<LS_STOP_TEST>(h, 1u, {vec_args(h), 0}, st);
}
static void launch_scaling(ipm_handle* h) {
    if (h->bnd) hipLaunchKernelGGL(scaling_bounded_kernel, dim3(h->vblk), dim3(VBLK), 0, h->stream, vec_args(h), bnd_args(h));
    else hipLaunchKernelGGL(scaling_kernel, dim3(h->vblk), dim3(VBLK), 0, h->stream, vec_args(h));
}
static void launch_direction(ipm_handle* h, int corr) {
    if (h->bnd) launch_untwinned(h, direction_bounded_kernel, dim3(h->vblk), dim3(VBLK), nullptr, vec_args(h), corr, bnd_args(h));
    else launch_twin<LS_DIRECTION>(h, (unsigned)h->vblk, {vec_args(h), corr});
}
static void launch_mu_aff(ipm_handle* h) { launch_vec_step<LS_MU_AFF>(h, mu_aff_bounded_kernel); }
static void launch_corrector_rhs(ipm_handle* h) { launch_vec_step<LS_CORR_RHS>(h, corrector_rhs_bounded_kernel); }
static void launch_update(ipm_handle* h) { launch_vec_step<LS_UPDATE>(h, update_bounded_kernel); }

static int enqueue_residuals(ipm_handle* h, hipStream_t st = nullptr) {
    launch_gemv_n(h, h->x, 1.0, -1.0, h->b, h->rb, st);
    launch_gemv_t(h, h->y, st);
    launch_prepare(h, st);
    launch_stop_test(h, st);
    HIP_TRY(h, hipGetLastError());
    return IPM_OK;
}

static int enqueue_residual_stream(ipm_handle* h, hipStream_t chain) {
    HIP_TRY(h, hipEventRecord(h->ev_mid, chain));
    HIP_TRY(h, hipStreamWaitEvent(h->stream3, h->ev_mid, 0));
    int rc = enqueue_residuals(h, h->stream3);
    if (rc) return rc;
    launch_gemv_n(h, h->v, -1.0, -1.0, h->rb, h->t1, h->stream3);
    HIP_TRY(h, hipEventRecord(h->ev_res, h->stream3));
    HIP_TRY(h, hipGetLastError());
    return IPM_OK;
}
static bool overlap_residuals(const ipm_handle* h) {
    return h->stream3 != nullptr && h->profiling < 2;
}
```

### interiorpointmethod_amd/csrc/ipm_api.hip

```cpp
#include <hip/hip_runtime.h>
#include <hip/hip_ext.h>
#include <math.h>
#include <stdarg.h>
#include <stdio.h>
#include <stdlib.h>
#include <string.h>

#include <deque>
#include <vector>

#include "../../include/ipm_hip.h"
#include "gemm_nt_f64.h"
#include "adat_syrk_f64.h"
#include "chol_update_f64.h"
#include "potrf_f64.h"
#include "sparse_ops.h"
#include "trsv_grouped.h"
#include "getrf_f64.h"
#include "small_lp.h"
#include "sparse_chol.h"
#include "sparse_symbolic.h"
#include "vector_ops.h"
#include "form_factor.h"
#include "lockstep.h"
#include "lockstep_merge.h"
#include "equilibrate.h"

#include <algorithm>
#include <atomic>
#include <mutex>
#include <chrono>
#include <limits>
#include <utility>

using namespace ipm;

#include "host_handle.h"
#include "host_equilibrate.h"
#include "host_sparse_setup.h"
#include "host_residuals.h"
#include "host_factor_solve.h"
#include "host_fused.h"
#include "host_iteration.h"
#include "host_lockstep.h"
#include "host_lu.h"
#include "host_small_batch.h"

extern "C" int ipm_abi_version(void) { return IPM_ABI_VERSION; }

extern "C" int ipm_device_count(int* count) {
    if (!count) return fail(nullptr, IPM_ERR_INVALID_ARG, "count is NULL");
    int c = 0;
    hipError_t e = hipGetDeviceCount(&c);
    if (e != hipSuccess) { *count = 0; return fail(nullptr, IPM_ERR_NO_DEVICE, "hipGetDeviceCount: %s", hipGetErrorString(e)); }
    *count = c;
    return IPM_OK;
}

extern "C" void ipm_default_options(ipm_options* o) {
    if (!o) return;
    memset(o, 0, sizeof *o);
    o->eta = 0.91;
    o->pivot_guard_eps = 1e-30;
    o->pivot_guard_big = 1e64;
    o->check_every = 4;
}

extern "C" const char* ipm_last_error(const ipm_handle* h) { return h ? h->err : g_err; }

extern "C" int ipm_workspace_bytes(int64_t m, int64_t n, size_t* bytes) {
    if (!bytes || m <= 0 || n <= 0) return fail(nullptr, IPM_ERR_INVALID_ARG, "bad arguments to ipm_workspace_bytes");
    *bytes = make_layout(m, n).total;
    return IPM_OK;
}

extern "C" int ipm_workspace_bytes_csc(int64_t m, int64_t n, int64_t nnz, size_t* bytes) {
    if (!bytes || m <= 0 || n <= 0 || nnz <= 0) return fail(nullptr, IPM_ERR_INVALID_ARG, "bad arguments to ipm_workspace_bytes_csc");
    *bytes = make_layout(m, n, nnz).total;
    return IPM_OK;
}

extern "C" int ipm_workspace_bytes_opts(int64_t m, int64_t n, const ipm_options* opts, size_t* bytes) {
    if (!bytes || m <= 0 || n <= 0) return fail(nullptr, IPM_ERR_INVALID_ARG, "bad arguments to ipm_workspace_bytes_opts");
    const int64_t nnz = opts && opts->sparse_nnz > 0 ? opts->sparse_nnz : 0;
    *bytes = make_layout(m, n, nnz, layout_no_dense(m, nnz, opts ? opts->flags : 0u)).total;
    return IPM_OK;
}

static void read_env_switches(ipm_handle* h) {
    if (const char* e = getenv("IPM_TEST_SPIN_LIMIT")) h->spin_limit = (unsigned)std::max(1, atoi(e));
    if (const char* e = getenv("IPM_ENVELOPE")) h->envelope = atoi(e);
    if (const char* e = getenv("IPM_LOOKAHEAD")) h->lookahead = atoi(e);
    if (const char* e = getenv("IPM_GROUPED_TRSV")) h->grouped_trsv = atoi(e);
    if (getenv("IPM_LS_BLOCK_STEPS")) h->ls_block_steps = true;
    if (const char* e = getenv("IPM_RAGGED_GROUPS")) h->ragged_groups = atoi(e) != 0;
    if (const char* e = getenv("IPM_FLAG_SYNC")) h->flag_sync = atoi(e);
    if (const char* e = getenv("IPM_BULK_VARIANT")) h->bulk_variant = atoi(e);
    if (const char* e = getenv("IPM_TWO_LEVEL")) h->two_level = atoi(e);
    if (const char* e = getenv("IPM_GROUP_STEPS")) h->group_steps = atoi(e);
    if (const char* e = getenv("IPM_FUSED_SMALL")) h->fused_small = atoi(e);
    if (const char* e = getenv("IPM_LIST_FORM")) h->list_form_opt = atoi(e);
    if (getenv("IPM_POTRF_STAMPS")) h->potrf_stamps = true;
    if (const char* e = getenv("IPM_FUSED_FACTOR")) { if (!strcmp(e, "force")) { h->ff_enabled = 1; h->ff_min_nblk = 3; h->ff_forced = true; } else h->ff_enabled = atoi(e); }
    if (const char* e = getenv("IPM_FF_MAX_NBLK")) h->ff_max_nblk = atoi(e);
    if (const char* e = getenv("IPM_FF_CHAIN_MODE")) h->ff_chain_mode0 = atoi(e) == 0;
    if (const char* e = getenv("IPM_FF_REF_ENGINE")) h->ff_ref_engine = atoi(e) != 0;
    if (const char* e = getenv("IPM_FF_Q")) h->ff_q = std::max(1, std::min(16, atoi(e)));
}

extern "C" int ipm_create(int device, int64_t m, int64_t n, const ipm_options* opts, void* workspace,
                          size_t workspace_bytes, void* stream, ipm_handle** out) {
    if (!out) return fail(nullptr, IPM_ERR_INVALID_ARG, "out is NULL");
    *out = nullptr;
    if (m <= 0 || n <= 0 || m > (1 << 20) || n > (1 << 24)) return fail(nullptr, IPM_ERR_INVALID_ARG, "bad problem size %lld x %lld", (long long)m, (long long)n);
    int ndev = 0;
    if (hipGetDeviceCount(&ndev) != hipSuccess || ndev <= 0) return fail(nullptr, IPM_ERR_NO_DEVICE, "no HIP device visible");
    if (device < 0 || device >= ndev) return fail(nullptr, IPM_ERR_INVALID_ARG, "device %d out of range (%d visible)", device, ndev);
    ipm_handle* h = new ipm_handle();
    h->device = device;
    if (opts) h->opt = *opts; else ipm_default_options(&h->opt);
    if (h->opt.check_every < 1) h->opt.check_every = 1;
    if (!(h->opt.eta > 0.0)) h->opt.eta = 0.91;
    if (!(h->opt.pivot_guard_big > 0.0)) h->opt.pivot_guard_big = 1e64;
    if (!(h->opt.regularize >= 0.0)) h->opt.regularize = 0.0;
    h->shift_rel = h->opt.regularize;
    read_env_switches(h);
    if (h->opt.sparse_nnz < 0) h->opt.sparse_nnz = 0;
    h->sparse = h->opt.sparse_nnz > 0;
    h->nnz_cap = h->opt.sparse_nnz;
    h->no_dense = layout_no_dense(m, h->opt.sparse_nnz, h->opt.flags);
    Layout L = make_layout(m, n, h->opt.sparse_nnz, h->no_dense);
    h->m = m; h->n = n; h->mp = L.mp; h->np = L.np; h->nblk = L.nblk;
    h->rc_chunks = L.rc_chunks; h->rows_per_chunk = L.rows_per_chunk; h->vblk = L.vblk;
    h->ws_bytes = L.total;
#define CREATE_TRY(call)                                                                       \
    do {                                                                                       \
        hipError_t e_ = (call);                                                                \
        if (e_ != hipSuccess) {                                                                \
            int rc_ = fail(nullptr, IPM_ERR_HIP, "%s failed: %s", #call, hipGetErrorString(e_)); \
            ipm_destroy(h);                                                                    \
            return rc_;                                                                        \
        }                                                                                      \
    } while (0)
    CREATE_TRY(hipSetDevice(device));
    if (stream) { h->stream = (hipStream_t)stream; }
    else { CREATE_TRY(hipStreamCreateWithFlags(&h->stream, hipStreamNonBlocking)); h->own_stream = true; }
    if (workspace) {
        if (workspace_bytes < L.total || ((uintptr_t)workspace & 255)) {
            int rc_ = fail(nullptr, IPM_ERR_WORKSPACE, "workspace too small or not 256-byte aligned (%zu < %zu)", workspace_bytes, L.total);
            ipm_destroy(h);
            return rc_;
        }
        h->ws = workspace;
    } else {
        CREATE_TRY(hipMalloc(&h->ws, L.total));
        h->own_ws = true;
    }
    char* base = (char*)h->ws;
    h->A = (double*)(base + L.off_A);
    h->B = h->no_dense ? nullptr : (double*)(base + L.off_B);
    h->invD = h->no_dense ? nullptr : (double*)(base + L.off_inv);
    double* nv = (double*)(base + L.off_nvec);
    h->x = nv; h->s = nv + L.np; h->c = nv + 2 * L.np; h->rc = nv + 3 * L.np; h->d = nv + 4 * L.np;
    h->v = nv + 5 * L.np; h->q = nv + 6 * L.np; h->dxa = nv + 7 * L.np; h->dsa = nv + 8 * L.np;
    h->dx = nv + 9 * L.np; h->ds = nv + 10 * L.np;
    double* mv = (double*)(base + L.off_mvec);
    h->y = mv; h->b = mv + L.mp; h->rb = mv + 2 * L.mp; h->t1 = mv + 3 * L.mp; h->t2 = mv + 4 * L.mp;
    h->dya = mv + 5 * L.mp; h->dy = mv + 6 * L.mp;
    h->atp = (double*)(base + L.off_atp);
    h->part = (double*)(base + L.off_part);
    h->det = (double*)(base + L.off_det);
    h->sc = (Scalars*)(base + L.off_sc);
    h->fixed = (int*)(base + L.off_fixed);
    h->hist = (IterRec*)(base + L.off_hist);
    h->snap = (double*)(base + L.off_snap);
    h->slab = h->no_dense ? nullptr : (double*)(base + L.off_slab);
    h->d_tile_order = (int*)(base + L.off_order);
    {
        std::vector<int> order;
        const int nT = L.nblk, PB = 8;
        order.reserve((size_t)nT * (nT + 1) / 2);
        for (int I = 0; I * PB < nT; ++I)
            for (int J = 0; J <= I; ++J)
                for (int ti = I * PB; ti < nT && ti < (I + 1) * PB; ++ti)
                    for (int tj = J * PB; tj <= ti && tj < (J + 1) * PB; ++tj) order.push_back((ti << 16) | tj);
        CREATE_TRY(hipMemcpyAsync(h->d_tile_order, order.data(), sizeof(int) * order.size(), hipMemcpyHostToDevice, h->stream));
        CREATE_TRY(hipStreamSynchronize(h->stream));
    }
    h->d_rowptr = (int*)(base + L.off_rowptr); h->d_colptr = (int*)(base + L.off_colptr);
    h->d_colind = (int*)(base + L.off_colind); h->d_rowind = (int*)(base + L.off_rowind);
    h->d_rval = (double*)(base + L.off_rval); h->d_cval = (double*)(base + L.off_cval);
    {
        CREATE_TRY(hipMemcpyToSymbolAsync(HIP_SYMBOL(ipm_spin_limit), &h->spin_limit, sizeof h->spin_limit, 0, hipMemcpyHostToDevice, h->stream));
        CREATE_TRY(hipStreamSynchronize(h->stream));
    }
    CREATE_TRY(hipMemsetAsync(base + L.off_inv, 0, L.off_slab - L.off_inv, h->stream));
    {
        std::lock_guard<std::mutex> lock(g_hsc_mutex);
        if (!g_hsc_pool.empty()) { h->h_sc = g_hsc_pool.back(); g_hsc_pool.pop_back(); }
    }
    if (!h->h_sc) CREATE_TRY(hipHostMalloc((void**)&h->h_sc, sizeof(Scalars), hipHostMallocDefault));
    memset(h->h_sc, 0, sizeof(Scalars));
    CREATE_TRY(hipEventCreate(&h->ev0));
    CREATE_TRY(hipEventCreate(&h->ev1));
    h->detect = (h->opt.flags & IPM_FLAG_DETECT_INFEASIBILITY) != 0;
    if (h->opt.flags & IPM_FLAG_LOCKSTEP) { h->lockstep = 1; h->opt.flags |= IPM_FLAG_SINGLE_STREAM | IPM_FLAG_NO_DEVICE_POLLING; }
    if (h->opt.flags & IPM_FLAG_SINGLE_STREAM) h->lookahead = 0;
    if (h->lockstep && h->ls_block_steps) h->grouped_trsv = 0;
    if (h->lockstep) h->ss_small_blocks = 1 << 20;
    if (h->no_dense) h->grouped_trsv = 0;
    h->gsz = 0;
    if (h->grouped_trsv) {
        const bool ragged = h->ragged_groups;
        if (h->nblk >= 2 * GS_MAX) { if (ragged || h->nblk % GS_MAX == 0) h->gsz = GS_MAX; }
        else {
            for (int p2 = GS_MAX; p2 >= 2; p2 /= 2) if (h->nblk % p2 == 0) { h->gsz = p2; break; }
            if (ragged && h->nblk > GS_MAX && h->gsz < 4) h->gsz = GS_MAX;
        }
    }
    if (h->gsz > 0) {
        const size_t nG = (size_t)h->nblk / h->gsz, GR = (size_t)h->gsz * 128;
        CREATE_TRY(dev_malloc(device, h->stream, (void**)&h->gXT, sizeof(double) * nG * GR * GR));
        CREATE_TRY(dev_malloc(device, h->stream, (void**)&h->gX, sizeof(double) * nG * GR * GR));
        CREATE_TRY(dev_malloc(device, h->stream, (void**)&h->gS, sizeof(double) * nG * (GR / 2) * (GR / 2)));
        CREATE_TRY(dev_malloc(device, h->stream, (void**)&h->gPart, sizeof(double) * 16 * (size_t)h->mp));
        CREATE_TRY(hipMemsetAsync(h->gXT, 0, sizeof(double) * nG * GR * GR, h->stream));
        CREATE_TRY(hipMemsetAsync(h->gX, 0, sizeof(double) * nG * GR * GR, h->stream));
    } else {
        h->grouped_trsv = 0;
    }
    CREATE_TRY(dev_malloc(device, h->stream, (void**)&h->d_flags, sizeof(unsigned) * (2 * (size_t)h->nblk + 4)));
    CREATE_TRY(hipMemsetAsync(h->d_flags, 0, sizeof(unsigned) * (2 * (size_t)h->nblk + 4), h->stream));
    CREATE_TRY(dev_malloc(device, h->stream, (void**)&h->d_bulk_done, sizeof(unsigned) * (2 * (size_t)h->nblk + 4)));
    CREATE_TRY(hipMemsetAsync(h->d_bulk_done, 0, sizeof(unsigned) * (2 * (size_t)h->nblk + 4), h->stream));
    if (h->opt.flags & IPM_FLAG_NO_DEVICE_POLLING) h->flag_sync = 0;
    if (h->potrf_stamps) { CREATE_TRY(dev_malloc(device, h->stream, (void**)&h->stamp_buf, 8 * 64 * sizeof(long long))); CREATE_TRY(hipMemsetAsync(h->stamp_buf, 0, 8 * 64 * sizeof(long long), h->stream)); }
    if (h->lookahead != 0 && h->nblk > 2)
        CREATE_TRY(hipStreamCreateWithFlags(&h->stream2, hipStreamNonBlocking));
    CREATE_TRY(hipEventCreateWithFlags(&h->ev_fork, hipEventDisableTiming));
    if (!h->sparse && h->lookahead != 0 && h->nblk >= 16)
        CREATE_TRY(hipStreamCreateWithFlags(&h->stream3, hipStreamNonBlocking));
    CREATE_TRY(hipEventCreateWithFlags(&h->ev_mid, hipEventDisableTiming));
    CREATE_TRY(hipEventCreateWithFlags(&h->ev_res, hipEventDisableTiming));
    CREATE_TRY(hipEventCreateWithFlags(&h->ev_grp, hipEventDisableTiming));
    CREATE_TRY(hipEventCreateWithFlags(&h->ev_last, hipEventDisableTiming));
    if (h->ff_chain_mode0) {
        int rc_ = fail(nullptr, IPM_ERR_INVALID_ARG, "IPM_FF_CHAIN_MODE=0 is not supported (that structure of the fused launch was removed)");
        ipm_destroy(h);
        return rc_;
    }
    h->ev_crit.assign(h->nblk, nullptr); h->ev_bulk.assign(h->nblk, nullptr);
    for (int k = 0; k < h->nblk; ++k) {
        CREATE_TRY(hipEventCreateWithFlags(&h->ev_crit[k], hipEventDisableTiming));
        CREATE_TRY(hipEventCreateWithFlags(&h->ev_bulk[k], hipEventDisableTiming));
    }
    if (h->sparse && h->mp <= SP_LDS_MAX_MP && device < MAX_DEVICES && !g_attr_set[device].load(std::memory_order_acquire)) {
        CREATE_TRY(hipFuncSetAttribute((const void*)adat_sparse_kernel, hipFuncAttributeMaxDynamicSharedMemorySize, SP_LDS_MAX_MP * 8));
        g_attr_set[device].store(true, std::memory_order_release);
    }
    hipLaunchKernelGGL(set_params_kernel, dim3(1), dim3(1), 0, h->stream, h->sc, 1e-8, 1e-8, 1e-8, h->opt.eta, 5000, 0, 1);
    CREATE_TRY(hipGetLastError());
    CREATE_TRY(hipStreamSynchronize(h->stream));
#undef CREATE_TRY
    if (device < MAX_DEVICES) { g_live[device].fetch_add(1, std::memory_order_acq_rel); h->counted = true; }
    *out = h;
    return IPM_OK;
}

extern "C" int ipm_destroy(ipm_handle* h) {
    if (!h) return IPM_OK;
    (void)hipSetDevice(h->device);
    if (h->ff_prof) ff_dump_profile(h);
    if (h->counted) g_live[h->device].fetch_sub(1, std::memory_order_acq_rel);
    if (h->stream) (void)hipStreamSynchronize(h->stream);
    if (h->stream2) (void)hipStreamSynchronize(h->stream2);
    for (auto& v : {&h->ev_crit, &h->ev_bulk})
        for (hipEvent_t e : *v) if (e) (void)hipEventDestroy(e);
    if (h->ev_fork) (void)hipEventDestroy(h->ev_fork);
    if (h->stream3) { (void)hipStreamSynchronize(h->stream3); (void)hipStreamDestroy(h->stream3); }
    if (h->ev_mid) (void)hipEventDestroy(h->ev_mid);
    if (h->ev_res) (void)hipEventDestroy(h->ev_res);
    if (h->ev_grp) (void)hipEventDestroy(h->ev_grp);
    if (h->ev_last) (void)hipEventDestroy(h->ev_last);
    if (h->stream2) (void)hipStreamDestroy(h->stream2);
    if (h->ev0) (void)hipEventDestroy(h->ev0);
    if (h->ev1) (void)hipEventDestroy(h->ev1);
    if (h->h_sc) { std::lock_guard<std::mutex> lock(g_hsc_mutex); g_hsc_pool.push_back(h->h_sc); h->h_sc = nullptr; }
    for (void* p : {(void*)h->stamp_buf, (void*)h->d_flags, (void*)h->d_bulk_done, (void*)h->B_own, (void*)h->invD_own, (void*)h->bnd_mem, (void*)h->cert_mem, (void*)h->gXT, (void*)h->gX, (void*)h->gS, (void*)h->gPart})
        dev_free(h->device, h->stream, p);
    ff_release(h);
    free_sparse_factor(h);
    for (void* p : {(void*)h->sm_bptr, (void*)h->sm_bcol, (void*)h->sm_bi, (void*)h->sm_bk, (void*)h->sm_bcoef, (void*)h->ls_bi, (void*)h->ls_bk, (void*)h->ls_bak})
        dev_free(h->device, h->stream, p);
    if (h->own_ws && h->ws) (void)hipFree(h->ws);
    if (h->own_stream && h->stream) (void)hipStreamDestroy(h->stream);
    delete h;
    return IPM_OK;
}

static bool all_finite(const double* p, int64_t rows, int64_t cols, int64_t ld) {
    for (int64_t i = 0; i < rows; ++i)
        for (int64_t j = 0; j < cols; ++j)
            if (!isfinite(p[i * ld + j])) return false;
    return true;
}

extern "C" int ipm_set_A_dense(ipm_handle* h, const double* A, int64_t ld, int is_device) {
    if (!h || !A || ld < h->n) return fail(h, IPM_ERR_INVALID_ARG, "ipm_set_A_dense: bad arguments");
    if (h->sparse) return fail(h, IPM_ERR_STATE, "ipm_set_A_dense: the handle was created for a sparse A (sparse_nnz > 0)");
    HIP_TRY(h, hipSetDevice(h->device));
    if (!is_device && !all_finite(A, h->m, h->n, ld)) return fail(h, IPM_ERR_INVALID_INPUT, "A has non-finite entries");
    if (int rc_ = eq_reset(h)) return rc_;
    HIP_TRY(h, hipMemsetAsync(h->A, 0, sizeof(double) * h->mp * h->np, h->stream));
    HIP_TRY(h, hipMemcpy2DAsync(h->A, sizeof(double) * h->np, A, sizeof(double) * ld, sizeof(double) * h->n, h->m,
                                is_device ? hipMemcpyDeviceToDevice : hipMemcpyHostToDevice, h->stream));
    HIP_TRY(h, hipStreamSynchronize(h->stream));
    h->haveA = true; h->predictor_valid = false;
    return IPM_OK;
}

extern "C" int ipm_set_bc(ipm_handle* h, const double* b, const double* c) {
    if (!h || !b || !c) return fail(h, IPM_ERR_INVALID_ARG, "ipm_set_bc: bad arguments");
    if (!all_finite(b, 1, h->m, h->m) || !all_finite(c, 1, h->n, h->n)) return fail(h, IPM_ERR_INVALID_INPUT, "b or c has non-finite entries");
    HIP_TRY(h, hipSetDevice(h->device));
    std::vector<double> bs, cs;
    const double *b0 = b, *c0 = c;
    b = eq_in(h, bs, b, h->eq_r, false); c = eq_in(h, cs, c, h->eq_c, false);
    if (!eq_in_range(h, b0, b, (size_t)h->m) || !eq_in_range(h, c0, c, (size_t)h->n))
        return fail(h, IPM_ERR_INVALID_INPUT, "ipm_set_bc: the handle's scaling would push an entry of b or c out of the normal fp64 range");
    HIP_TRY(h, hipMemcpyAsync(h->b, b, sizeof(double) * h->m, hipMemcpyHostToDevice, h->stream));
    HIP_TRY(h, hipMemcpyAsync(h->c, c, sizeof(double) * h->n, hipMemcpyHostToDevice, h->stream));
    enqueue_bc_norms(h);
    HIP_TRY(h, hipGetLastError());
    HIP_TRY(h, hipStreamSynchronize(h->stream));
    h->haveBC = true; h->predictor_valid = false;
    return IPM_OK;
}

extern "C" int ipm_set_state(ipm_handle* h, const double* x, const double* y, const double* s) {
    if (!h || !x || !y || !s) return fail(h, IPM_ERR_INVALID_ARG, "ipm_set_state: bad arguments");
    HIP_TRY(h, hipSetDevice(h->device));
    std::vector<double> xs, ys, ss;
    x = eq_in(h, xs, x, h->eq_c, true); y = eq_in(h, ys, y, h->eq_r, true); s = eq_in(h, ss, s, h->eq_c, false);
    HIP_TRY(h, hipMemcpyAsync(h->x, x, sizeof(double) * h->n, hipMemcpyHostToDevice, h->stream));
    HIP_TRY(h, hipMemcpyAsync(h->y, y, sizeof(double) * h->m, hipMemcpyHostToDevice, h->stream));
    HIP_TRY(h, hipMemcpyAsync(h->s, s, sizeof(double) * h->n, hipMemcpyHostToDevice, h->stream));
    HIP_TRY(h, hipStreamSynchronize(h->stream));
    mark_fresh_state(h);
    return IPM_OK;
}

extern "C" int ipm_get_state(ipm_handle* h, double* x, double* y, double* s) {
    if (!h) return fail(h, IPM_ERR_INVALID_ARG, "ipm_get_state: NULL handle");
    HIP_TRY(h, hipSetDevice(h->device));
    if (x) HIP_TRY(h, hipMemcpyAsync(x, h->x, sizeof(double) * h->n, hipMemcpyDeviceToHost, h->stream));
    if (y) HIP_TRY(h, hipMemcpyAsync(y, h->y, sizeof(double) * h->m, hipMemcpyDeviceToHost, h->stream));
    if (s) HIP_TRY(h, hipMemcpyAsync(s, h->s, sizeof(double) * h->n, hipMemcpyDeviceToHost, h->stream));
    HIP_TRY(h, hipStreamSynchronize(h->stream));
    eq_out(h, x, h->eq_c, false); eq_out(h, y, h->eq_r, false); eq_out(h, s, h->eq_c, true);
    return IPM_OK;
}

extern "C" int ipm_set_bounds(ipm_handle* h, const double* u) {
    if (!h) return fail(h, IPM_ERR_INVALID_ARG, "ipm_set_bounds: NULL handle");
    HIP_TRY(h, hipSetDevice(h->device));
    int nU = 0;
    if (u) {
        for (int64_t j = 0; j < h->n; ++j) {
            const double v = u[j];
            if (!(v >= 0.0)) return fail(h, IPM_ERR_INVALID_INPUT, "ipm_set_bounds: u[%lld] = %g (bounds must be >= 0, +inf for none)", (long long)j, v);
            if (v < std::numeric_limits<double>::infinity()) ++nU;
        }
    }
    h->predictor_valid = false;
    if (nU == 0) {
        h->bnd = false; h->bnd_nU = 0;
        if (h->haveBC) hipLaunchKernelGGL(norm2_kernel, dim3(1), dim3(VBLK), 0, h->stream, h->b, (int)h->m, &h->sc->b_norm);
        HIP_TRY(h, hipGetLastError());
        HIP_TRY(h, hipStreamSynchronize(h->stream));
        return IPM_OK;
    }
    const size_t np = (size_t)h->np;
    if (!h->bnd_mem) {
        if (dev_malloc(h->device, h->stream, (void**)&h->bnd_mem, sizeof(double) * BND_VECS * np) != hipSuccess)
            return fail(h, IPM_ERR_HIP, "ipm_set_bounds: %d x %lld doubles could not be allocated", BND_VECS, (long long)np);
        HIP_TRY(h, hipMemsetAsync(h->bnd_mem, 0, sizeof(double) * BND_VECS * np, h->stream));
    }
    std::vector<double> uu(np, std::numeric_limits<double>::infinity());
    std::copy(u, u + h->n, uu.begin());
    eq_out(h, uu.data(), h->eq_c, true);
    if (!eq_in_range(h, u, uu.data(), (size_t)h->n))
        return fail(h, IPM_ERR_INVALID_INPUT, "ipm_set_bounds: the handle's scaling would push a bound out of the normal fp64 range");
    HIP_TRY(h, hipMemcpyAsync(h->bnd_mem, uu.data(), sizeof(double) * np, hipMemcpyHostToDevice, h->stream));
    h->bnd = true; h->bnd_nU = nU;
    const BndArgs bd = bnd_args(h);
    hipLaunchKernelGGL(bnd_fill_kernel, dim3((unsigned)((np + 255) / 256)), dim3(256), 0, h->stream, bd.u, bd.w, bd.z, (int)np, 1.0, 0);
    if (h->haveBC) hipLaunchKernelGGL(bnd_norm2_kernel, dim3(1), dim3(VBLK), 0, h->stream, h->b, (int)h->m, bd.u, (int)h->n, &h->sc->b_norm);
    HIP_TRY(h, hipGetLastError());
    HIP_TRY(h, hipStreamSynchronize(h->stream));
    return IPM_OK;
}

extern "C" int ipm_set_bound_state(ipm_handle* h, const double* w, const double* z) {
    if (!h || !w || !z) return fail(h, IPM_ERR_INVALID_ARG, "ipm_set_bound_state: bad arguments");
    if (!h->bnd) return fail(h, IPM_ERR_STATE, "ipm_set_bound_state: no finite bound is set (ipm_set_bounds)");
    HIP_TRY(h, hipSetDevice(h->device));
    const BndArgs bd = bnd_args(h);
    std::vector<double> wsc, zsc;
    w = eq_in(h, wsc, w, h->eq_c, true); z = eq_in(h, zsc, z, h->eq_c, false);
    HIP_TRY(h, hipMemcpyAsync(bd.w, w, sizeof(double) * h->n, hipMemcpyHostToDevice, h->stream));
    HIP_TRY(h, hipMemcpyAsync(bd.z, z, sizeof(double) * h->n, hipMemcpyHostToDevice, h->stream));
    hipLaunchKernelGGL(bnd_fill_kernel, dim3((unsigned)((h->n + 255) / 256)), dim3(256), 0, h->stream, bd.u, bd.w, bd.z, (int)h->n, 0.0, 1);
    HIP_TRY(h, hipGetLastError());
    HIP_TRY(h, hipStreamSynchronize(h->stream));
    h->predictor_valid = false; h->fresh_state = true;
    return IPM_OK;
}

extern "C" int ipm_get_bound_state(ipm_handle* h, double* w, double* z) {
    if (!h) return fail(h, IPM_ERR_INVALID_ARG, "ipm_get_bound_state: NULL handle");
    if (!h->bnd) return fail(h, IPM_ERR_STATE, "ipm_get_bound_state: no finite bound is set (ipm_set_bounds)");
    HIP_TRY(h, hipSetDevice(h->device));
    const BndArgs bd = bnd_args(h);
    if (w) HIP_TRY(h, hipMemcpyAsync(w, bd.w, sizeof(double) * h->n, hipMemcpyDeviceToHost, h->stream));
    if (z) HIP_TRY(h, hipMemcpyAsync(z, bd.z, sizeof(double) * h->n, hipMemcpyDeviceToHost, h->stream));
    HIP_TRY(h, hipStreamSynchronize(h->stream));
    eq_out(h, w, h->eq_c, false); eq_out(h, z, h->eq_c, true);
    return IPM_OK;
}

static int enqueue_init_state(ipm_handle* h, double y0) {
    int gn = (int)((h->n + 255) / 256), gm = (int)((h->m + 255) / 256);
    hipLaunchKernelGGL(fill_kernel, dim3(gn), dim3(256), 0, h->stream, h->x, (int)h->n, 1.0);
    hipLaunchKernelGGL(fill_kernel, dim3(gn), dim3(256), 0, h->stream, h->s, (int)h->n, 1.0);
    hipLaunchKernelGGL(fill_kernel, dim3(gm), dim3(256), 0, h->stream, h->y, (int)h->m, y0);
    if (h->bnd) {
        const BndArgs bd = bnd_args(h);
        hipLaunchKernelGGL(bnd_fill_kernel, dim3(gn), dim3(256), 0, h->stream, bd.u, bd.w, bd.z, (int)h->n, 1.0, 0);
    }
    HIP_TRY(h, hipGetLastError());
    return IPM_OK;
}

extern "C" int ipm_init_state(ipm_handle* h, double y0) {
    if (!h) return fail(h, IPM_ERR_INVALID_ARG, "ipm_init_state: NULL handle");
    HIP_TRY(h, hipSetDevice(h->device));
    int rc = enqueue_init_state(h, y0);
    if (rc) return rc;
    HIP_TRY(h, hipStreamSynchronize(h->stream));
    mark_fresh_state(h);
    return IPM_OK;
}

extern "C" int ipm_debug_get_stamps(ipm_handle* h, long long* out) {
    if (!h || !out || !h->stamp_buf) return fail(h, IPM_ERR_STATE, "stamps not enabled (IPM_POTRF_STAMPS=1)");
    HIP_TRY(h, hipMemcpyAsync(out, h->stamp_buf, 8 * 64 * sizeof(long long), hipMemcpyDeviceToHost, h->stream));
    HIP_TRY(h, hipStreamSynchronize(h->stream));
    return IPM_OK;
}

extern "C" int ipm_set_profiling(ipm_handle* h, int enable) {
    if (!h) return fail(h, IPM_ERR_INVALID_ARG, "ipm_set_profiling: NULL handle");
    h->profiling = enable < 0 ? 0 : (enable > 2 ? 2 : enable);
    return IPM_OK;
}
extern "C" int ipm_get_phase_ms(ipm_handle* h, double out[4]) {
    if (!h || !out) return fail(h, IPM_ERR_INVALID_ARG, "ipm_get_phase_ms: bad arguments");
    for (int i = 0; i < 4; ++i) out[i] = h->phase_ms[i];
    return IPM_OK;
}

extern "C" int ipm_set_infeasibility_tol(ipm_handle* h, double eps_p, double eps_d) {
    if (!h || !(eps_p > 0.0) || !(eps_d > 0.0) || !(eps_p < 1.0) || !(eps_d < 1.0))
        return fail(h, IPM_ERR_INVALID_ARG, "ipm_set_infeasibility_tol: tolerances must lie in (0, 1)");
    h->det_eps_p = eps_p; h->det_eps_d = eps_d;
    return IPM_OK;
}

extern "C" int ipm_get_certificate(ipm_handle* h, double* y, double* z, double* x, double info[4]) {
    if (!h) return fail(h, IPM_ERR_INVALID_ARG, "ipm_get_certificate: NULL handle");
    const int status = h->h_sc ? h->h_sc->status : 0;
    if (status != IPM_STATUS_PRIMAL_INFEASIBLE && status != IPM_STATUS_DUAL_INFEASIBLE)
        return fail(h, IPM_ERR_STATE, "ipm_get_certificate: the last solve ended in status %d, not in an infeasibility detection (5 / 6)", status);
    HIP_TRY(h, hipSetDevice(h->device));
    const size_t n = (size_t)h->n, m = (size_t)h->m;
    if (!h->cert_mem) HIP_TRY(h, dev_malloc(h->device, h->stream, (void**)&h->cert_mem, sizeof(double) * (2 * n + m)));
    const unsigned grid = (unsigned)std::min<size_t>((std::max(n, m) + 255) / 256, 256);
    hipLaunchKernelGGL(certificate_kernel, dim3(grid), dim3(256), 0, h->stream, h->x, h->y, h->bnd ? bnd_args(h).z : nullptr, h->det,
                       (int)m, (int)n, h->cert_mem);
    HIP_TRY(h, hipGetLastError());
    double rec[4];
    HIP_TRY(h, hipMemcpyAsync(rec, h->det, sizeof rec, hipMemcpyDeviceToHost, h->stream));
    if (x) HIP_TRY(h, hipMemcpyAsync(x, h->cert_mem, sizeof(double) * n, hipMemcpyDeviceToHost, h->stream));
    if (y) HIP_TRY(h, hipMemcpyAsync(y, h->cert_mem + n, sizeof(double) * m, hipMemcpyDeviceToHost, h->stream));
    if (z) HIP_TRY(h, hipMemcpyAsync(z, h->cert_mem + n + m, sizeof(double) * n, hipMemcpyDeviceToHost, h->stream));
    HIP_TRY(h, hipStreamSynchronize(h->stream));
    eq_out(h, x, h->eq_c, false); eq_out(h, y, h->eq_r, false); eq_out(h, z, h->eq_c, true);
    if (info) for (int i = 0; i < 4; ++i) info[i] = rec[i];
    return IPM_OK;
}

extern "C" int ipm_get_history(ipm_handle* h, ipm_iter_record* out, int32_t capacity, int32_t* count) {
    if (!h || !count || capacity < 0 || (capacity > 0 && !out)) return fail(h, IPM_ERR_INVALID_ARG, "ipm_get_history: bad arguments");
    static_assert(sizeof(ipm_iter_record) == sizeof(IterRec), "history record layout");
    HIP_TRY(h, hipSetDevice(h->device));
    int k = 0;
    HIP_TRY(h, hipMemcpyAsync(&k, &h->sc->k, sizeof(int), hipMemcpyDeviceToHost, h->stream));
    HIP_TRY(h, hipStreamSynchronize(h->stream));
    int nrec = std::min(std::min(k, HIST_CAP), (int)capacity);
    if (nrec > 0) {
        std::vector<IterRec> ring(HIST_CAP);
        HIP_TRY(h, hipMemcpyAsync(ring.data(), h->hist, sizeof(IterRec) * HIST_CAP, hipMemcpyDeviceToHost, h->stream));
        HIP_TRY(h, hipStreamSynchronize(h->stream));
        for (int i = 0; i < nrec; ++i) memcpy(&out[i], &ring[(size_t)(k - nrec + i) % HIST_CAP], sizeof(IterRec));
    }
    *count = nrec;
    return IPM_OK;
}

extern "C" int ipm_get_schedule(ipm_handle* h, int32_t out[12]) {
    if (!h || !out) return fail(h, IPM_ERR_INVALID_ARG, "ipm_get_schedule: bad arguments");
    const int live = live_on_device(h);
    out[0] = h->nblk; out[1] = h->last_gs; out[2] = h->grouped_trsv;
    out[3] = (may_poll(h) && live <= 1) ? 1 : 0;
    out[4] = h->n_counter_steps; out[5] = h->n_event_steps; out[6] = h->use_env ? 1 : 0; out[7] = live;
    out[8] = h->timeouts_recovered; out[9] = h->small ? 1 : 0;
    out[10] = h->ff_last ? 1 : 0; out[11] = (h->spf && sp_level(h)) ? 1 : 0;
    return IPM_OK;
}

extern "C" int ipm_form_normal_matrix(ipm_handle* h, const double* d, double* B, int64_t ldb) {
    if (!h || !d || !B || ldb < h->m) return fail(h, IPM_ERR_INVALID_ARG, "ipm_form_normal_matrix: bad arguments");
    if (!h->haveA) return fail(h, IPM_ERR_STATE, "ipm_form_normal_matrix: A not set");
    HIP_TRY(h, hipSetDevice(h->device));
    hipLaunchKernelGGL(set_params_kernel, dim3(1), dim3(1), 0, h->stream, h->sc, 1e-8, 1e-8, 1e-8, h->opt.eta, 1 << 30, 1, 0);
    HIP_TRY(h, hipMemcpyAsync(h->d, d, sizeof(double) * h->n, hipMemcpyHostToDevice, h->stream));
    int rc = enqueue_form(h, h->d, true);
    if (rc) return rc;
    std::vector<double> tmp((size_t)h->mp * h->mp);
    HIP_TRY(h, hipMemcpyAsync(tmp.data(), h->B, sizeof(double) * h->mp * h->mp, hipMemcpyDeviceToHost, h->stream));
    HIP_TRY(h, hipStreamSynchronize(h->stream));
    for (int64_t i = 0; i < h->m; ++i)
        for (int64_t j = 0; j < h->m; ++j)
            B[i * ldb + j] = (j <= i) ? tmp[i * h->mp + j] : tmp[j * h->mp + i];
    h->predictor_valid = false;
    return IPM_OK;
}

extern "C" int ipm_normal_solve(ipm_handle* h, const double* d, const double* rhs, double* z, int reuse_factor,
                                int32_t* pivots_fixed) {
    if (!h || !rhs || !z) return fail(h, IPM_ERR_INVALID_ARG, "ipm_normal_solve: bad arguments");
    if (!h->haveA) return fail(h, IPM_ERR_STATE, "ipm_normal_solve: A not set");
    HIP_TRY(h, hipSetDevice(h->device));
    int rc;
    for (int attempt = 0;; ++attempt) {
        hipLaunchKernelGGL(set_params_kernel, dim3(1), dim3(1), 0, h->stream, h->sc, 1e-8, 1e-8, 1e-8, h->opt.eta, 1 << 30, 1, 1);
        if (!reuse_factor) {
            if (d) {
                HIP_TRY(h, hipMemcpyAsync(h->d, d, sizeof(double) * h->n, hipMemcpyHostToDevice, h->stream));
            } else {
                hipLaunchKernelGGL(fill_kernel, dim3((unsigned)((h->n + 255) / 256)), dim3(256), 0, h->stream, h->d, (int)h->n, 1.0);
            }
            if ((rc = enqueue_form(h, h->d))) return rc;
            if ((rc = enqueue_factor(h, true))) return rc;
            if ((rc = enqueue_group_inverses(h))) return rc;
        }
        HIP_TRY(h, hipMemsetAsync(h->t1, 0, sizeof(double) * h->mp, h->stream));
        HIP_TRY(h, hipMemcpyAsync(h->t1, rhs, sizeof(double) * h->m, hipMemcpyHostToDevice, h->stream));
        if ((rc = enqueue_potrs(h, h->t1, h->dy))) return rc;
        bool tmo = false;
        if ((rc = read_scalars(h, &tmo))) return rc;
        if (!tmo) break;
        if (attempt || reuse_factor) return fail(h, IPM_ERR_HIP, "hand-off time-out persists with stream events");
        poll_fallback(h);
    }
    HIP_TRY(h, hipMemcpyAsync(z, h->dy, sizeof(double) * h->m, hipMemcpyDeviceToHost, h->stream));
    HIP_TRY(h, hipStreamSynchronize(h->stream));
    if (pivots_fixed) *pivots_fixed = h->h_sc->fixed;
    h->predictor_valid = false;
    return IPM_OK;
}

extern "C" int ipm_get_factor(ipm_handle* h, double* L, int64_t ldl) {
    if (!h || !L || ldl < h->m) return fail(h, IPM_ERR_INVALID_ARG, "ipm_get_factor: bad arguments");
    HIP_TRY(h, hipSetDevice(h->device));
    if (int rc_ = ensure_dense_B(h)) return rc_;
    if (h->spf) {
        HIP_TRY(h, hipMemsetAsync(h->B, 0, sizeof(double) * h->mp * h->mp, h->stream));
        hipLaunchKernelGGL(sp_expand_kernel, dim3((unsigned)h->spF.nsn), dim3(256), 0, h->stream, h->spF, h->B, (long long)h->mp);
        HIP_TRY(h, hipGetLastError());
    }
    std::vector<double> tmp((size_t)h->mp * h->mp);
    HIP_TRY(h, hipMemcpyAsync(tmp.data(), h->B, sizeof(double) * h->mp * h->mp, hipMemcpyDeviceToHost, h->stream));
    HIP_TRY(h, hipStreamSynchronize(h->stream));
    for (int64_t i = 0; i < h->m; ++i)
        for (int64_t j = 0; j < h->m; ++j) L[i * ldl + j] = (j <= i) ? tmp[i * h->mp + j] : 0.0;
    return IPM_OK;
}

extern "C" int ipm_solve_linear(ipm_handle* h, const double* B, int64_t ldb, const double* rhs, double* z, int32_t* pivots_fixed) {
    if (!h || !B || !rhs || !z || ldb < h->m) return fail(h, IPM_ERR_INVALID_ARG, "ipm_solve_linear: bad arguments");
    HIP_TRY(h, hipSetDevice(h->device));
    if (int rc_ = ensure_dense_B(h)) return rc_;
    const int64_t m = h->m, mp = h->mp;
    std::vector<double> img((size_t)mp * mp, 0.0);
    for (int64_t i = 0; i < mp; ++i) {
        if (i < m) memcpy(&img[(size_t)i * mp], B + i * ldb, sizeof(double) * m);
        else img[(size_t)i * mp + i] = 1.0;
    }
    const bool saved_env = h->use_env;
    h->use_env = false;
    struct SpOff { ipm_handle* h; ~SpOff() { h->spf_off = false; } } sp_off{h};
    h->spf_off = true;
    int rc = IPM_OK;
    for (int attempt = 0;; ++attempt) {
        hipLaunchKernelGGL(set_params_kernel, dim3(1), dim3(1), 0, h->stream, h->sc, 1e-8, 1e-8, 1e-8, h->opt.eta, 1 << 30, 1, 1);
        hipError_t e = hipMemcpyAsync(h->B, img.data(), sizeof(double) * mp * mp, hipMemcpyHostToDevice, h->stream);
        if (e == hipSuccess) e = hipMemsetAsync(h->t1, 0, sizeof(double) * mp, h->stream);
        if (e == hipSuccess) e = hipMemcpyAsync(h->t1, rhs, sizeof(double) * m, hipMemcpyHostToDevice, h->stream);
        if (e != hipSuccess) { h->use_env = saved_env; return fail(h, IPM_ERR_HIP, "ipm_solve_linear: upload failed: %s", hipGetErrorString(e)); }
        rc = enqueue_factor(h);
        if (!rc) rc = enqueue_group_inverses(h);
        if (!rc) rc = enqueue_potrs(h, h->t1, h->dy);
        bool tmo = false;
        if (!rc) rc = read_scalars(h, &tmo);
        if (rc || !tmo) break;
        if (attempt) { rc = fail(h, IPM_ERR_HIP, "hand-off time-out persists with stream events"); break; }
        poll_fallback(h);
    }
    h->use_env = saved_env;
    if (rc) return rc;
    HIP_TRY(h, hipMemcpyAsync(z, h->dy, sizeof(double) * m, hipMemcpyDeviceToHost, h->stream));
    HIP_TRY(h, hipStreamSynchronize(h->stream));
    if (pivots_fixed) *pivots_fixed = h->h_sc->fixed;
    h->predictor_valid = false;
    return IPM_OK;
}
```

### interiorpointmethod_amd/csrc/vector_ops.h

```cpp
#pragma once
#include <hip/hip_runtime.h>
#include <stdint.h>
#include "gemm_nt_f64.h"
#include "iteration_rules.h"

namespace ipm {

constexpr int VBLK = 256;
constexpr int MAXPART = 64;

enum { P_RC2 = 0, P_XS, P_CX, P_RB2, P_MINP_AFF, P_MIND_AFF, P_MUAFF, P_MINP, P_MIND, P_NSLOT };
enum { P_BY = P_NSLOT, P_UZ, P_MATY, P_MAX, P_MXU, P_NSLOT_DETECT };

__device__ __forceinline__ double block_sum(double v, double* red) {
    const int tid = threadIdx.x;
    red[tid] = v;
    __syncthreads();
    for (int s = VBLK / 2; s > 0; s >>= 1) {
        if (tid < s) red[tid] += red[tid + s];
        __syncthreads();
    }
    double r = red[0];
    __syncthreads();
    return r;
}
__device__ __forceinline__ double block_min(double v, double* red) {
    const int tid = threadIdx.x;
    red[tid] = v;
    __syncthreads();
    for (int s = VBLK / 2; s > 0; s >>= 1) {
        if (tid < s) red[tid] = fmin(red[tid], red[tid + s]);
        __syncthreads();
    }
    double r = red[0];
    __syncthreads();
    return r;
}
__device__ __forceinline__ double block_max(double v, double* red) { return -block_min(-v, red); }
__device__ __forceinline__ double sum_partials(const double* part, int slot, int nblk) {
    double s = 0.0;
    for (int i = 0; i < nblk; ++i) s += part[slot * MAXPART + i];
    return s;
}
__device__ __forceinline__ double min_partials(const double* part, int slot, int nblk) {
    double s = 1.0;
    for (int i = 0; i < nblk; ++i) s = fmin(s, part[slot * MAXPART + i]);
    return s;
}
__device__ __forceinline__ double max_partials(const double* part, int slot, int nblk) {
    double s = 0.0;
    for (int i = 0; i < nblk; ++i) s = fmax(s, part[slot * MAXPART + i]);
    return s;
}

__device__ __forceinline__ void gemv_n_kernel_body(const double* __restrict__ A, int64_t lda, int mp,
                                                     int np, const double* __restrict__ v, double sa,
                                                     double sb, const double* __restrict__ add,
                                                     double* out, const int* done, const unsigned bx_, const unsigned gx_) {
    if (done && *done) return;
    const int lane = threadIdx.x & 63;
    const int row = bx_ * 4 + (threadIdx.x >> 6);
    if (row >= mp) return;
    const double* ar = A + (int64_t)row * lda;
    double acc0 = 0.0, acc1 = 0.0;
    for (int c = lane * 2; c < np; c += 128) {
        f64x2 a2 = *reinterpret_cast<const f64x2*>(ar + c);
        f64x2 v2 = *reinterpret_cast<const f64x2*>(v + c);
        acc0 += a2.x * v2.x;
        acc1 += a2.y * v2.y;
    }
    double s = acc0 + acc1;
    for (int off = 32; off > 0; off >>= 1) s += __shfl_xor(s, off, 64);
    if (lane == 0) out[row] = sa * s + (add ? sb * add[row] : 0.0);
}
__global__ __launch_bounds__(256) void gemv_n_kernel(const double* __restrict__ A, int64_t lda, int mp,
                                                     int np, const double* __restrict__ v, double sa,
                                                     double sb, const double* __restrict__ add,
                                                     double* out, const int* done) { gemv_n_kernel_body(A, lda, mp, np, v, sa, sb, add, out, done, blockIdx.x, gridDim.x); }

__device__ __forceinline__ void gemv_t_kernel_body(const double* __restrict__ A, int64_t lda, int rows_per_chunk,
                                                     int np, const double* __restrict__ u, double* part,
                                                     const int* done, const unsigned bx_, const unsigned by_) {
    if (done && *done) return;
    const int c = (bx_ * 256 + threadIdx.x) * 2;
    if (c >= np) return;
    const int r0 = by_ * rows_per_chunk;
    double a0 = 0.0, a1 = 0.0;
    const double* ap = A + (int64_t)r0 * lda + c;
#pragma unroll 8
    for (int r = 0; r < rows_per_chunk; ++r) {
        f64x2 a2 = *reinterpret_cast<const f64x2*>(ap + (int64_t)r * lda);
        double ur = u[r0 + r];
        a0 += a2.x * ur;
        a1 += a2.y * ur;
    }
    *reinterpret_cast<f64x2*>(part + (int64_t)by_ * np + c) = (f64x2){a0, a1};
}
__global__ __launch_bounds__(256) void gemv_t_kernel(const double* __restrict__ A, int64_t lda, int rows_per_chunk,
                                                     int np, const double* __restrict__ u, double* part,
                                                     const int* done) { gemv_t_kernel_body(A, lda, rows_per_chunk, np, u, part, done, blockIdx.x, blockIdx.y); }

struct VecArgs {
    int m, n, np, rc_chunks;
    int nblk;
    const double* atp;
    double *x, *y, *s;
    const double *b, *c;
    double *rb, *rc, *d, *v, *q;
    double *dxa, *dya, *dsa, *dx, *dy, *ds;
    double* part;
    Scalars* sc;
    IterRec* hist;
};

__device__ __forceinline__ double col_sum(const double* atp, int rc_chunks, int np, int j) {
    double s = 0.0;
    int r = 0;
    for (; r + 8 <= rc_chunks; r += 8) {
        double t[8];
#pragma unroll
        for (int q = 0; q < 8; ++q) t[q] = atp[(int64_t)(r + q) * np + j];
#pragma unroll
        for (int q = 0; q < 8; ++q) s += t[q];
    }
    for (; r < rc_chunks; ++r) s += atp[(int64_t)r * np + j];
    return s;
}

template <bool Bounded = false, bool Detect = false>
__device__ __forceinline__ void prepare_kernel_body(VecArgs a, const unsigned bx_, const unsigned gx_, BndArgs bd = BndArgs{}) {
    __shared__ double red[VBLK];
    const int gid = bx_ * VBLK + threadIdx.x, gsz = gx_ * VBLK;
    double rc2 = 0.0, xs = 0.0, cx = 0.0, rb2 = 0.0;
    double by = 0.0, uz = 0.0, maty = 0.0, max_ = 0.0, mxu = 0.0;
    for (int j = gid; j < a.n; j += gsz) {
        double xj = a.x[j], sj = a.s[j];
        if constexpr (Bounded) {
            const double uj = bd.u[j];
            if (bnd_in(uj)) {
                const double wj = bd.w[j], zj = bd.z[j];
                const double atyj = col_sum(a.atp, a.rc_chunks, a.np, j);
                const double rcj = atyj + sj - zj - a.c[j];
                const double ruj = xj + wj - uj;
                const double dj = bnd_theta(xj, sj, wj, zj);
                const double r3 = xj * sj, r4 = wj * zj;
                a.rc[j] = rcj;
                a.d[j] = dj;
                a.q[j] = r3 / xj;
                bd.qz[j] = r4 / wj;
                a.v[j] = dj * (rcj - r3 / xj + (r4 - zj * ruj) / wj);
                rc2 += rcj * rcj;
                xs += r3;
                xs += r4;
                cx += a.c[j] * xj;
                rb2 += ruj * ruj;
                if constexpr (Detect) { uz += uj * zj; maty = fmax(maty, atyj - zj); mxu = fmax(mxu, xj); }
                continue;
            }
        }
        const double atyj = col_sum(a.atp, a.rc_chunks, a.np, j);
        double rcj = atyj + sj - a.c[j];
        double dj = xj / sj;
        double r3 = xj * sj;
        a.rc[j] = rcj;
        a.d[j] = dj;
        a.q[j] = r3 / xj;
        a.v[j] = dj * (rcj - r3 / xj);
        rc2 += rcj * rcj;
        xs += r3;
        cx += a.c[j] * xj;
        if constexpr (Detect) maty = fmax(maty, atyj);
    }
    for (int i = gid; i < a.m; i += gsz) {
        double r = a.rb[i]; rb2 += r * r;
        if constexpr (Detect) { const double bi = a.b[i]; by += bi * a.y[i]; max_ = fmax(max_, fabs(r + bi)); }
    }
    rc2 = block_sum(rc2, red); xs = block_sum(xs, red); cx = block_sum(cx, red); rb2 = block_sum(rb2, red);
    if constexpr (Detect) { by = block_sum(by, red); uz = block_sum(uz, red); maty = block_max(maty, red); max_ = block_max(max_, red); mxu = block_max(mxu, red); }
    if (threadIdx.x == 0) {
        a.part[P_RC2 * MAXPART + bx_] = rc2;
        a.part[P_XS * MAXPART + bx_] = xs;
        a.part[P_CX * MAXPART + bx_] = cx;
        a.part[P_RB2 * MAXPART + bx_] = rb2;
        if constexpr (Detect) {
            a.part[P_BY * MAXPART + bx_] = by;
            a.part[P_UZ * MAXPART + bx_] = uz;
            a.part[P_MATY * MAXPART + bx_] = maty;
            a.part[P_MAX * MAXPART + bx_] = max_;
            a.part[P_MXU * MAXPART + bx_] = mxu;
        }
    }
}
__global__ __launch_bounds__(VBLK) void prepare_kernel(VecArgs a) { prepare_kernel_body(a, blockIdx.x, gridDim.x); }
__global__ __launch_bounds__(VBLK) void prepare_bounded_kernel(VecArgs a, BndArgs bd) { prepare_kernel_body<true>(a, blockIdx.x, gridDim.x, bd); }
__global__ __launch_bounds__(VBLK) void prepare_detect_kernel(VecArgs a) { prepare_kernel_body<false, true>(a, blockIdx.x, gridDim.x); }
__global__ __launch_bounds__(VBLK) void prepare_bounded_detect_kernel(VecArgs a, BndArgs bd) { prepare_kernel_body<true, true>(a, blockIdx.x, gridDim.x, bd); }

template <bool Bounded = false>
__device__ __forceinline__ void scaling_kernel_body(VecArgs a, BndArgs bd = BndArgs{}) {
    if (blockIdx.x == 0 && threadIdx.x == 0) a.sc->done_f = a.sc->done;
    if (a.sc->done) return;
    const int gid = blockIdx.x * VBLK + threadIdx.x, gsz = gridDim.x * VBLK;
    for (int j = gid; j < a.n; j += gsz) {
        if constexpr (Bounded) {
            if (bnd_in(bd.u[j])) { a.d[j] = bnd_theta(a.x[j], a.s[j], bd.w[j], bd.z[j]); continue; }
        }
        a.d[j] = a.x[j] / a.s[j];
    }
}
__global__ __launch_bounds__(VBLK) void scaling_kernel(VecArgs a) { scaling_kernel_body(a); }
__global__ __launch_bounds__(VBLK) void scaling_bounded_kernel(VecArgs a, BndArgs bd) { scaling_kernel_body<true>(a, bd); }

template <bool Bounded = false, bool Detect = false>
__device__ __forceinline__ void stop_test_kernel_body(VecArgs a, const unsigned bx_, const unsigned gx_, BndArgs bd = BndArgs{}, DetArgs dt = DetArgs{}) {
    if (threadIdx.x != 0 || bx_ != 0) return;
    Scalars* sc = a.sc;
    if (sc->done) return;
    double rb = sqrt(sum_partials(a.part, P_RB2, a.nblk));
    double rc = sqrt(sum_partials(a.part, P_RC2, a.nblk));
    double gap = sum_partials(a.part, P_XS, a.nblk);
    sc->rb_norm = rb; sc->rc_norm = rc; sc->gap = gap;
    const double obj = sum_partials(a.part, P_CX, a.nblk);
    sc->obj = obj;
    if (fabs(obj) < 1.7e308) sc->obj_last_finite = obj;
    if constexpr (Bounded) sc->mu = gap / (double)(a.n + bd.nU);
    else sc->mu = gap / (double)a.n;
    bool cont = (sc->e1 * (1.0 + sc->b_norm) < rb) || (sc->e2 * (1.0 + sc->c_norm) < rc) || (sc->e3 < gap);
    if (sc->force) return;
    if (!cont) {
        bool finite = (rb == rb) && (rc == rc) && (gap == gap) && (fabs(rb) < 1.7e308) && (fabs(rc) < 1.7e308) &&
                      (fabs(gap) < 1.7e308);
        sc->status = finite ? 1 : 3;
        sc->done = 1;
    } else if (Detect && detect_fire(dt, sc, sum_partials(a.part, P_BY, a.nblk) - sum_partials(a.part, P_UZ, a.nblk),
                                     max_partials(a.part, P_MATY, a.nblk), -obj,
                                     fmax(max_partials(a.part, P_MAX, a.nblk), max_partials(a.part, P_MXU, a.nblk)))) {
    } else if (sc->k >= sc->max_iter) {
        sc->status = 2;
        sc->done = 1;
    }
}
__global__ void stop_test_kernel(VecArgs a) { stop_test_kernel_body(a, blockIdx.x, gridDim.x); }
__global__ void stop_test_bounded_kernel(VecArgs a, BndArgs bd) { stop_test_kernel_body<true>(a, blockIdx.x, gridDim.x, bd); }
__global__ void stop_test_detect_kernel(VecArgs a, DetArgs dt) { stop_test_kernel_body<false, true>(a, blockIdx.x, gridDim.x, BndArgs{}, dt); }
__global__ void stop_test_bounded_detect_kernel(VecArgs a, BndArgs bd, DetArgs dt) { stop_test_kernel_body<true, true>(a, blockIdx.x, gridDim.x, bd, dt); }

__global__ __launch_bounds__(256) void certificate_kernel(const double* x, const double* y, const double* z, const double* det, int m, int n,
                                                          double* out) {
    const int gid = blockIdx.x * 256 + threadIdx.x, gsz = gridDim.x * 256;
    const bool primal = det[0] == (double)IPM_STATUS_PRIMAL_INFEASIBLE_;
    const double sc = 1.0 / det[1];
    double *ox = out, *oy = out + n, *oz = out + n + m;
    for (int j = gid; j < n; j += gsz) {
        ox[j] = primal ? 0.0 : x[j] * sc;
        oz[j] = (primal && z) ? z[j] * sc : 0.0;
    }
    for (int i = gid; i < m; i += gsz) oy[i] = primal ? y[i] * sc : 0.0;
}

template <bool Bounded = false>
__device__ __forceinline__ void direction_kernel_body(VecArgs a, int corr, const unsigned bx_, const unsigned gx_, BndArgs bd = BndArgs{}) {
    if (a.sc->done) return;
    __shared__ double red[VBLK];
    const int gid = bx_ * VBLK + threadIdx.x, gsz = gx_ * VBLK;
    double* DX = corr ? a.dx : a.dxa;
    double* DS = corr ? a.ds : a.dsa;
    double mp_ = 1.0, md_ = 1.0;
    for (int j = gid; j < a.n; j += gsz) {
        const double xj = a.x[j], sj = a.s[j];
        const double w = col_sum(a.atp, a.rc_chunks, a.np, j);
        direction_column<Bounded>(a, bd, j, w, DX, DS, corr ? bd.dw : bd.dwa, corr ? bd.dz : bd.dza, xj, sj, mp_, md_);
    }
    mp_ = block_min(mp_, red); md_ = block_min(md_, red);
    if (threadIdx.x == 0) {
        a.part[(corr ? P_MINP : P_MINP_AFF) * MAXPART + bx_] = mp_;
        a.part[(corr ? P_MIND : P_MIND_AFF) * MAXPART + bx_] = md_;
    }
}
__global__ __launch_bounds__(VBLK) void direction_kernel(VecArgs a, int corr) { direction_kernel_body(a, corr, blockIdx.x, gridDim.x); }
__global__ __launch_bounds__(VBLK) void direction_bounded_kernel(VecArgs a, int corr, BndArgs bd) { direction_kernel_body<true>(a, corr, blockIdx.x, gridDim.x, bd); }

template <bool Bounded = false>
__device__ __forceinline__ void mu_aff_kernel_body(VecArgs a, const unsigned bx_, const unsigned gx_, BndArgs bd = BndArgs{}) {
    if (a.sc->done) return;
    __shared__ double red[VBLK];
    const int gid = bx_ * VBLK + threadIdx.x, gsz = gx_ * VBLK;
    const double ap = min_partials(a.part, P_MINP_AFF, a.nblk);
    const double ad = min_partials(a.part, P_MIND_AFF, a.nblk);
    double acc = 0.0;
    for (int j = gid; j < a.n; j += gsz) mu_aff_column<Bounded>(a, bd, j, ap, ad, acc);
    acc = block_sum(acc, red);
    if (threadIdx.x == 0) {
        a.part[P_MUAFF * MAXPART + bx_] = acc;
        if (bx_ == 0) { a.sc->alpha_aff_p = ap; a.sc->alpha_aff_d = ad; }
    }
}
__global__ __launch_bounds__(VBLK) void mu_aff_kernel(VecArgs a) { mu_aff_kernel_body(a, blockIdx.x, gridDim.x); }
__global__ __launch_bounds__(VBLK) void mu_aff_bounded_kernel(VecArgs a, BndArgs bd) { mu_aff_kernel_body<true>(a, blockIdx.x, gridDim.x, bd); }

template <bool Bounded = false>
__device__ __forceinline__ void corrector_rhs_kernel_body(VecArgs a, const unsigned bx_, const unsigned gx_, BndArgs bd = BndArgs{}) {
    if (a.sc->done) return;
    const int gid = bx_ * VBLK + threadIdx.x, gsz = gx_ * VBLK;
    const double mu = a.sc->mu;
    const Centring ct = centring<Bounded>(sum_partials(a.part, P_MUAFF, a.nblk), mu, a.n, bd);
    const double sm = ct.sigma * mu;
    for (int j = gid; j < a.n; j += gsz) corrector_column<Bounded>(a, bd, j, sm);
    if (gid == 0) { a.sc->mu_aff = ct.mu_aff; a.sc->sigma = ct.sigma; }
}
__global__ __launch_bounds__(VBLK) void corrector_rhs_kernel(VecArgs a) { corrector_rhs_kernel_body(a, blockIdx.x, gridDim.x); }
__global__ __launch_bounds__(VBLK) void corrector_rhs_bounded_kernel(VecArgs a, BndArgs bd) { corrector_rhs_kernel_body<true>(a, blockIdx.x, gridDim.x, bd); }

template <bool Bounded = false>
__device__ __forceinline__ void update_kernel_body(VecArgs a, const unsigned bx_, const unsigned gx_, BndArgs bd = BndArgs{}) {
    if (a.sc->done) return;
    const int gid = bx_ * VBLK + threadIdx.x, gsz = gx_ * VBLK;
    const double eta = a.sc->eta;
    const double ap = damped_step(eta, min_partials(a.part, P_MINP, a.nblk));
    const double ad = damped_step(eta, min_partials(a.part, P_MIND, a.nblk));
    for (int j = gid; j < a.n; j += gsz) update_column<Bounded>(a, bd, j, ap, ad);
    for (int i = gid; i < a.m; i += gsz) a.y[i] += ad * a.dy[i];
    if (gid == 0) {
        Scalars* sc = a.sc;
        if (sc->k == 0) sc->fixed_first = sc->fixed;
        record_iteration(sc, a.hist, sc->mu, sc->sigma, sc->alpha_aff_p, sc->alpha_aff_d, ap, ad);
    }
}
__global__ __launch_bounds__(VBLK) void update_kernel(VecArgs a) { update_kernel_body(a, blockIdx.x, gridDim.x); }
__global__ __launch_bounds__(VBLK) void update_bounded_kernel(VecArgs a, BndArgs bd) { update_kernel_body<true>(a, blockIdx.x, gridDim.x, bd); }

enum { PS_MIN_P = 0, PS_MIN_D, PS_XS, PS_SS, PS_SX, PS_SX2 };

__device__ __forceinline__ double start_min_partials(const double* part, int slot, int nblk) {
    double s = __builtin_inf();
    for (int i = 0; i < nblk; ++i) s = fmin(s, part[slot * MAXPART + i]);
    return s;
}
struct StartSums { double xs, ss, sx; };
__device__ __forceinline__ StartSums start_sums(const double* part, int nblk) {
    return {0.5 * sum_partials(part, PS_XS, nblk), sum_partials(part, PS_SS, nblk), sum_partials(part, PS_SX, nblk)};
}

template <bool Bounded, bool Dual>
__device__ __forceinline__ void start_ls_kernel_body(VecArgs a, BndArgs bd = BndArgs{}) {
    __shared__ double red[VBLK];
    const int gid = blockIdx.x * VBLK + threadIdx.x, gsz = gridDim.x * VBLK;
    double mn = __builtin_inf();
    for (int j = gid; j < a.n; j += gsz) {
        const double t = col_sum(a.atp, a.rc_chunks, a.np, j);
        if constexpr (Dual) start_dual_column<Bounded>(a, bd, j, a.c[j] - t, mn);
        else start_primal_column<Bounded>(a, bd, j, t, mn);
    }
    if constexpr (Dual) for (int i = gid; i < a.m; i += gsz) a.y[i] = a.dy[i];
    mn = block_min(mn, red);
    if (threadIdx.x == 0) a.part[(Dual ? PS_MIN_D : PS_MIN_P) * MAXPART + blockIdx.x] = mn;
}
__global__ __launch_bounds__(VBLK) void start_primal_kernel(VecArgs a) { start_ls_kernel_body<false, false>(a); }
__global__ __launch_bounds__(VBLK) void start_primal_bounded_kernel(VecArgs a, BndArgs bd) { start_ls_kernel_body<true, false>(a, bd); }
__global__ __launch_bounds__(VBLK) void start_dual_kernel(VecArgs a) { start_ls_kernel_body<false, true>(a); }
__global__ __launch_bounds__(VBLK) void start_dual_bounded_kernel(VecArgs a, BndArgs bd) { start_ls_kernel_body<true, true>(a, bd); }

template <bool Bounded>
__device__ __forceinline__ void start_shift_kernel_body(VecArgs a, BndArgs bd = BndArgs{}) {
    __shared__ double red[VBLK];
    const int gid = blockIdx.x * VBLK + threadIdx.x, gsz = gridDim.x * VBLK;
    const double dp = start_shift(start_min_partials(a.part, PS_MIN_P, a.nblk));
    const double dd = start_shift(start_min_partials(a.part, PS_MIN_D, a.nblk));
    double xs = 0.0, ss = 0.0, sx = 0.0;
    for (int j = gid; j < a.n; j += gsz) start_shift_column<Bounded>(a, bd, j, dp, dd, xs, ss, sx);
    xs = block_sum(xs, red); ss = block_sum(ss, red); sx = block_sum(sx, red);
    if (threadIdx.x == 0) {
        a.part[PS_XS * MAXPART + blockIdx.x] = xs;
        a.part[PS_SS * MAXPART + blockIdx.x] = ss;
        a.part[PS_SX * MAXPART + blockIdx.x] = sx;
    }
}
__global__ __launch_bounds__(VBLK) void start_shift_kernel(VecArgs a) { start_shift_kernel_body<false>(a); }
__global__ __launch_bounds__(VBLK) void start_shift_bounded_kernel(VecArgs a, BndArgs bd) { start_shift_kernel_body<true>(a, bd); }

template <bool Bounded>
__device__ __forceinline__ void start_primal_correct_kernel_body(VecArgs a, BndArgs bd = BndArgs{}) {
    __shared__ double red[VBLK];
    const int gid = blockIdx.x * VBLK + threadIdx.x, gsz = gridDim.x * VBLK;
    const StartSums t = start_sums(a.part, a.nblk);
    if (start_degenerate(t.xs, t.ss, t.sx)) {
        for (int j = gid; j < a.n; j += gsz) start_reference_column<Bounded>(a, bd, j);
        for (int i = gid; i < a.m; i += gsz) a.y[i] = 1.0;
        return;
    }
    const double pc = t.xs / t.ss;
    double sx = 0.0;
    for (int j = gid; j < a.n; j += gsz) start_primal_correct_column<Bounded>(a, bd, j, pc, sx);
    sx = block_sum(sx, red);
    if (threadIdx.x == 0) a.part[PS_SX2 * MAXPART + blockIdx.x] = sx;
}
__global__ __launch_bounds__(VBLK) void start_primal_correct_kernel(VecArgs a) { start_primal_correct_kernel_body<false>(a); }
__global__ __launch_bounds__(VBLK) void start_primal_correct_bounded_kernel(VecArgs a, BndArgs bd) { start_primal_correct_kernel_body<true>(a, bd); }

template <bool Bounded>
__device__ __forceinline__ void start_dual_correct_kernel_body(VecArgs a, BndArgs bd = BndArgs{}) {
    const int gid = blockIdx.x * VBLK + threadIdx.x, gsz = gridDim.x * VBLK;
    const StartSums t = start_sums(a.part, a.nblk);
    if (start_degenerate(t.xs, t.ss, t.sx)) return;
    const double dc = t.xs / sum_partials(a.part, PS_SX2, a.nblk);
    for (int j = gid; j < a.n; j += gsz) start_dual_correct_column<Bounded>(a, bd, j, dc);
}
__global__ __launch_bounds__(VBLK) void start_dual_correct_kernel(VecArgs a) { start_dual_correct_kernel_body<false>(a); }
__global__ __launch_bounds__(VBLK) void start_dual_correct_bounded_kernel(VecArgs a, BndArgs bd) { start_dual_correct_kernel_body<true>(a, bd); }

__global__ void fill_kernel(double* out, int n, double value) {
    int i = blockIdx.x * blockDim.x + threadIdx.x;
    if (i < n) out[i] = value;
}

__global__ __launch_bounds__(VBLK) void norm2_kernel(const double* v, int n, double* out) {
    __shared__ double red[VBLK];
    double acc = 0.0;
    for (int i = threadIdx.x; i < n; i += VBLK) acc += v[i] * v[i];
    acc = block_sum(acc, red);
    if (threadIdx.x == 0) *out = sqrt(acc);
}

__global__ __launch_bounds__(VBLK) void bnd_norm2_kernel(const double* b, int m, const double* u, int n, double* out) {
    __shared__ double red[VBLK];
    double acc = 0.0;
    for (int i = threadIdx.x; i < m; i += VBLK) acc += b[i] * b[i];
    for (int j = threadIdx.x; j < n; j += VBLK) { const double uj = u[j]; if (bnd_in(uj)) acc += uj * uj; }
    acc = block_sum(acc, red);
    if (threadIdx.x == 0) *out = sqrt(acc);
}

__global__ void bnd_fill_kernel(const double* u, double* w, double* z, int n, double value, int mask_only) {
    const int j = blockIdx.x * blockDim.x + threadIdx.x;
    if (j >= n) return;
    if (!bnd_in(u[j])) { w[j] = 0.0; z[j] = 0.0; }
    else if (!mask_only) { w[j] = value; z[j] = value; }
}

}
```

### interiorpointmethod_amd/handle.py

```python
import ctypes as C
import os

import numpy as np

from . import _lib
from .analysis import _col, _is_sparse, prepare

STATUS_NAMES = {0: "running", 1: "converged", 2: "max_iter", 3: "nan", 5: "primal_infeasible", 6: "dual_infeasible"}


def _dptr(a):
    return a.ctypes.data_as(C.POINTER(C.c_double))


def wants_shift(pivots_fixed, m, regularize=0.0, auto_regularize=True):
    return shift_allowed(regularize, auto_regularize) and pivots_fixed > 0.05 * m


def shift_allowed(regularize=0.0, auto_regularize=True):
    return bool(auto_regularize) and not regularize


def mehrotra_started(make, regularize=0.0, auto_regularize=True):
    sv = make()
    try:
        if wants_shift(sv.init_state_mehrotra(), sv.m, regularize, auto_regularize):
            sv.close()
            sv = make(regularize=1e-14)
            sv.init_state_mehrotra()
    except Exception:
        sv.close()
        raise
    return sv


SCALE_PASSES = 16


def check_scale(scale):
    if scale not in (None, "ruiz"):
        raise ValueError('scale must be None or "ruiz", not %r' % (scale,))
    return scale


def _gap_tol(tol, tol_gap):
    return float(tol if tol_gap is None else tol_gap)


class IpmSolver:

    def __init__(self, A, b, c, device=0, eta=0.91, pivot_guard_eps=1e-30, pivot_guard_big=1e64,
                 check_every=4, use_torch=True, dense=False, regularize=0.0, reorder="auto", concurrent=False,
                 auto_regularize=True, factor=None, prepared=None, lockstep=False, ub=None, detect_infeasibility=False,
                 infeasibility_tol=(1e-8, 1e-8), scale=None, scale_passes=SCALE_PASSES):
        self.scale = check_scale(scale)
        if prepared is None:
            prepared = prepare(A, b, c, dense=dense, reorder=reorder, factor=factor, ub=ub)
        elif ub is not None:
            raise ValueError("pass ub to prepare() when a Prepared is given")
        lib = _lib.load()
        self._lib = lib
        self._h = None
        self._perm = prepared.perm
        self.m, self.n = prepared.m, prepared.n
        self._host = prepared.host
        self.factor, self.order_info = prepared.factor, prepared.order_info
        A, b, c = prepared.A, prepared.b, prepared.c
        opts = _lib.Options()
        lib.ipm_default_options(C.byref(opts))
        opts.eta, opts.pivot_guard_eps, opts.pivot_guard_big = eta, pivot_guard_eps, pivot_guard_big
        opts.check_every = int(os.environ.get("IPM_CHECK_EVERY") or check_every)
        opts.regularize = float(regularize)
        opts.flags = (_lib.FLAG_LOCKSTEP if lockstep else 0) | \
                     ((_lib.FLAG_NO_DEVICE_POLLING | _lib.FLAG_SINGLE_STREAM) if concurrent else 0) | \
                     (0 if auto_regularize else _lib.FLAG_NO_AUTO_REGULARIZE) | \
                     (_lib.FLAG_SPARSE_FACTOR if self.factor == "sparse" else 0) | \
                     (_lib.FLAG_DETECT_INFEASIBILITY if detect_infeasibility else 0)
        self.detect_infeasibility = bool(detect_infeasibility)
        nbytes = C.c_size_t(0)
        self.sparse = _is_sparse(A)
        if self.sparse:
            opts.sparse_nnz = int(A.nnz)
            _lib.check(None, lib.ipm_workspace_bytes_opts(self.m, self.n, C.byref(opts), C.byref(nbytes)))
        else:
            _lib.check(None, lib.ipm_workspace_bytes(self.m, self.n, C.byref(nbytes)))
        self.workspace_bytes = nbytes.value
        ws_ptr, stream = None, None
        self._ws = None
        if use_torch:
            import torch
            if not torch.cuda.is_available():
                raise _lib.IpmLibraryError("no ROCm device visible to torch; the HIP path cannot run")
            dev = torch.device("cuda", device)
            self._ws = torch.empty(self.workspace_bytes, dtype=torch.uint8, device=dev)
            ws_ptr = C.c_void_p(self._ws.data_ptr())
            stream = C.c_void_p(torch.cuda.current_stream(dev).cuda_stream)
        h = C.c_void_p()
        _lib.check(None, lib.ipm_create(int(device), self.m, self.n, C.byref(opts), ws_ptr,
                                        self.workspace_bytes if ws_ptr else 0, stream, C.byref(h)))
        self._h = h
        if self.sparse:
            indptr = np.ascontiguousarray(A.indptr, dtype=np.int32)
            indices = np.ascontiguousarray(A.indices, dtype=np.int32)
            data = np.ascontiguousarray(A.data, dtype=np.float64)
            self._check(lib.ipm_set_A_csc(h, indptr.ctypes.data_as(C.POINTER(C.c_int32)),
                                          indices.ctypes.data_as(C.POINTER(C.c_int32)), _dptr(data),
                                          int(data.shape[0])))
            if self.factor == "sparse" and self.schedule()["fused_small"]:
                self.factor, self.order_info = "dense", None
        else:
            self._check(lib.ipm_set_A_dense(h, C.c_void_p(A.ctypes.data), self.n, 0))
        self.ub = prepared.ub
        self.bounded = 0 if self.ub is None else int(np.isfinite(self.ub).sum())
        if self.ub is not None:
            self._check(lib.ipm_set_bounds(h, _dptr(self.ub)))
        self._check(lib.ipm_set_bc(h, _dptr(b), _dptr(c)))
        if detect_infeasibility:
            eps_p, eps_d = infeasibility_tol
            self._check(lib.ipm_set_infeasibility_tol(h, float(eps_p), float(eps_d)))
        self.scale_info = None
        if self.scale is not None:
            info = np.zeros(4)
            ev = None
            if use_torch:
                ev = torch.cuda.Event(enable_timing=True), torch.cuda.Event(enable_timing=True)
                ev[0].record(torch.cuda.current_stream(dev))
            self._check(lib.ipm_equilibrate(h, int(scale_passes), _dptr(info)))
            ms = None
            if ev is not None:
                ev[1].record(torch.cuda.current_stream(dev))
                ev[1].synchronize()
                ms = float(ev[0].elapsed_time(ev[1]))
            self.scale_info = dict(passes=int(info[0]), row_spread_before=float(info[1]), row_spread_after=float(info[2]),
                                   col_spread_after=float(info[3]), ms=ms)
        self.stats = None

    def _check(self, code):
        _lib.check(self._h, code)

    def close(self):
        if self._h is not None:
            self._lib.ipm_destroy(self._h)
            self._h = None
            self._ws = None

    def __del__(self):
        try:
            self.close()
        except Exception:
            pass

    def __enter__(self):
        return self

    def __exit__(self, *exc):
        self.close()

    def init_state(self, y0=1.0):
        self._check(self._lib.ipm_init_state(self._h, float(y0)))

    def init_state_mehrotra(self):
        nfix = C.c_int32(0)
        self._check(self._lib.ipm_init_state_mehrotra(self._h, C.byref(nfix)))
        self.last_pivots_fixed = nfix.value
        return nfix.value

    def _rows_in(self, v):
        return v if self._perm is None else np.ascontiguousarray(v[self._perm])

    def _rows_out(self, v):
        if self._perm is None:
            return v
        out = np.empty_like(v)
        out[self._perm] = v
        return out

    def scaling(self):
        r, c = np.empty(self.m), np.empty(self.n)
        self._check(self._lib.ipm_get_scaling(self._h, _dptr(r), _dptr(c)))
        return self._rows_out(r), c, self.scale_info

    def set_state(self, x, y, s, w=None, z=None):
        x, y, s = _col(x, self.n, "x"), self._rows_in(_col(y, self.m, "y")), _col(s, self.n, "s")
        if (w is None) != (z is None):
            raise ValueError("give both w and z or neither")
        if w is not None:
            if not self.bounded:
                raise ValueError("w / z given but the solver has no finite upper bound")
            w, z = _col(w, self.n, "w"), _col(z, self.n, "z")
        self._check(self._lib.ipm_set_state(self._h, _dptr(x), _dptr(y), _dptr(s)))
        if w is not None:
            self._check(self._lib.ipm_set_bound_state(self._h, _dptr(w), _dptr(z)))

    def get_bound_state(self):
        if not self.bounded:
            return None
        w, z = np.empty(self.n), np.empty(self.n)
        self._check(self._lib.ipm_get_bound_state(self._h, _dptr(w), _dptr(z)))
        return w.reshape(-1, 1), z.reshape(-1, 1)

    def get_state(self):
        x, y, s = np.empty(self.n), np.empty(self.m), np.empty(self.n)
        self._check(self._lib.ipm_get_state(self._h, _dptr(x), _dptr(y), _dptr(s)))
        return x.reshape(-1, 1), self._rows_out(y).reshape(-1, 1), s.reshape(-1, 1)

    def newton_direction(self, corrector=False):
        dx, dy, ds = np.empty(self.n), np.empty(self.m), np.empty(self.n)
        st = _lib.Stats()
        self._check(self._lib.ipm_newton_direction(self._h, 1 if corrector else 0, _dptr(dx), _dptr(dy),
                                                   _dptr(ds), C.byref(st)))
        self.stats = st.as_dict()
        return dx.reshape(-1, 1), self._rows_out(dy).reshape(-1, 1), ds.reshape(-1, 1)

    def iterate(self, n_steps):
        st = _lib.Stats()
        self._check(self._lib.ipm_iterate(self._h, int(n_steps), C.byref(st)))
        self.stats = st.as_dict()
        return self.stats

    def solve(self, tol=1e-8, max_iter=5000, tol_gap=None):
        st = _lib.Stats()
        self._check(self._lib.ipm_solve(self._h, float(tol), float(tol), _gap_tol(tol, tol_gap), int(max_iter), C.byref(st)))
        self.stats = st.as_dict()
        return self.stats

    def history(self):
        buf = (_lib.IterRecord * _lib.HISTORY_CAPACITY)()
        n = C.c_int32(0)
        self._check(self._lib.ipm_get_history(self._h, buf, _lib.HISTORY_CAPACITY, C.byref(n)))
        return [{k: getattr(buf[i], k) for k, _ in _lib.IterRecord._fields_} for i in range(n.value)]

    def certificate(self):
        if self.stats is None or self.stats["status"] not in (_lib.STATUS_PRIMAL_INFEASIBLE, _lib.STATUS_DUAL_INFEASIBLE):
            return None
        y, z, x, info = np.empty(self.m), np.empty(self.n), np.empty(self.n), np.empty(4)
        self._check(self._lib.ipm_get_certificate(self._h, _dptr(y), _dptr(z), _dptr(x), _dptr(info)))
        return {"kind": STATUS_NAMES[int(info[0])], "y": self._rows_out(y), "z": z, "x": x,
                "normalization": float(info[1]), "violation": float(info[2]), "k": int(info[3])}

    def schedule(self):
        out = (C.c_int32 * 12)()
        self._check(self._lib.ipm_get_schedule(self._h, out))
        keys = ("blocks", "group_steps", "grouped_trsv", "device_polling", "counter_steps", "event_steps", "envelope",
                "live_handles", "timeouts_recovered", "fused_small", "fused_factor", "sparse_level_mode")
        return dict(zip(keys, (int(v) for v in out)))

    def factor_info(self):
        if self.factor != "sparse":
            return None
        out = (C.c_int64 * 8)()
        self._check(self._lib.ipm_get_factor_info(self._h, out))
        keys = ("panels", "tasks", "height", "widest_front", "factor_entries", "update_entries", "product_terms",
                "serial_launches")
        return dict(zip(keys, (int(v) for v in out)))

    def set_profiling(self, level=2):
        level = 2 if level is True else (0 if level is False else int(level))
        self._check(self._lib.ipm_set_profiling(self._h, level))

    def phase_ms(self):
        out = (C.c_double * 4)()
        self._check(self._lib.ipm_get_phase_ms(self._h, out))
        return dict(form=out[0], factor=out[1], trisolve=out[2], other=out[3])

    def form_normal_matrix(self, d):
        d = _col(d, self.n, "d")
        B = np.empty((self.m, self.m))
        self._check(self._lib.ipm_form_normal_matrix(self._h, _dptr(d), _dptr(B), self.m))
        if self._perm is not None:
            out = np.empty_like(B)
            out[np.ix_(self._perm, self._perm)] = B
            return out
        return B

    def get_factor(self):
        L = np.empty((self.m, self.m))
        self._check(self._lib.ipm_get_factor(self._h, _dptr(L), self.m))
        return L

    def normal_solve(self, rhs, d=None, reuse_factor=False):
        rhs = self._rows_in(_col(rhs, self.m, "rhs"))
        z = np.empty(self.m)
        dptr = None if d is None else _dptr(_col(d, self.n, "d"))
        nfix = C.c_int32(0)
        self._check(self._lib.ipm_normal_solve(self._h, dptr, _dptr(rhs), _dptr(z), 1 if reuse_factor else 0, C.byref(nfix)))
        self.last_pivots_fixed = nfix.value
        return self._rows_out(z)

    def mehrotra_start(self):
        A, b, c = self._host
        ub, rc = self.ub, None
        if self.scale_info is not None and self.scale_info["passes"]:
            r, cc, _ = self.scaling()
            rc = r, cc
            if _is_sparse(A):
                A = A.copy()
                A.data = A.data * r[A.indices] * np.repeat(cc, np.diff(A.indptr))
            else:
                A = r.reshape(-1, 1) * np.asarray(A, dtype=np.float64) * cc.reshape(1, -1)
            b, c = r * np.asarray(b, dtype=np.float64).ravel(), cc * np.asarray(c, dtype=np.float64).ravel()
            ub = None if ub is None else ub / cc
        out = self._mehrotra_start_of(A, np.asarray(b, dtype=np.float64).ravel(), np.asarray(c, dtype=np.float64).ravel(), ub)
        if rc is None:
            return out
        r, cc = rc
        x, y, s = out[0] * cc, out[1] * r, out[2] / cc
        return (x, y, s) if len(out) == 3 else (x, y, s, out[3] * cc, out[4] / cc)

    def _mehrotra_start_of(self, A, b, c, ub):
        x = A.T @ self.normal_solve(b)
        y = self.normal_solve(A @ c, reuse_factor=True)
        s = c - A.T @ y
        x = np.asarray(x).ravel(); s = np.asarray(s).ravel()
        if self.bounded:
            return self._mehrotra_start_bounded(x, np.asarray(y).ravel(), s, ub)
        x = x + max(-1.5 * x.min(), 0.0)
        s = s + max(-1.5 * s.min(), 0.0)
        xs = 0.5 * float(x @ s)
        if not (np.isfinite(xs) and s.sum() > 0 and x.sum() > 0 and xs > 0):
            return np.ones(self.n), np.ones(self.m), np.ones(self.n)
        x = x + xs / s.sum()
        s = s + xs / x.sum()
        return x, np.asarray(y).ravel(), s

    def _mehrotra_start_bounded(self, x, y, r, ub):
        U = np.isfinite(ub)
        w = np.zeros(self.n); z = np.zeros(self.n)
        w[U] = ub[U] - x[U]
        s = r.copy()
        s[U] = np.maximum(r[U], 0.0)
        z[U] = np.maximum(-r[U], 0.0)
        xmin = min(x.min(), w[U].min())
        smin = min(s.min(), z[U].min())
        dp, dd = max(-1.5 * xmin, 0.0), max(-1.5 * smin, 0.0)
        x = x + dp; w[U] += dp
        s = s + dd; z[U] += dd
        xs = 0.5 * float(x @ s + w[U] @ z[U])
        sx, ss = float(x.sum() + w[U].sum()), float(s.sum() + z[U].sum())
        if not (np.isfinite(xs) and ss > 0 and sx > 0 and xs > 0):
            w[U], z[U] = 1.0, 1.0
            return np.ones(self.n), np.ones(self.m), np.ones(self.n), w, z
        x = x + xs / ss; w[U] += xs / ss
        sx = float(x.sum() + w[U].sum())
        s = s + xs / sx; z[U] += xs / sx
        return x, y, s, w, z

    def solve_linear(self, B, rhs):
        B = np.ascontiguousarray(np.asarray(B, dtype=np.float64))
        rhs = _col(rhs, self.m, "rhs")
        z = np.empty(self.m)
        nfix = C.c_int32(0)
        self._check(self._lib.ipm_solve_linear(self._h, _dptr(B), self.m, _dptr(rhs), _dptr(z), C.byref(nfix)))
        return z.reshape(-1, 1), nfix.value
```

Measured before the change: 271.3 iterations/s.

## Stream A^T*dy row pieces on a side stream while the grouped triangular sweep runs

Splits the post-solve A^T*dy product into row-chunk pieces that become final as the backward grouped triangular sweep finishes each group. Signal kernels write a progress word at entry, and gate kernels on stream3 wait on that word before launching the partial gemv_t for the finished rows. The aim is to hide the large dense gemv_t behind the serial sweep. In exchange it adds cross-stream polling, extra launches and an event join, and it competes for compute units with the sweep. It is enabled by default only when device polling, grouped trsv and stream3 are available, and it falls back on timeout.

```diff
diff --git a/include/ipm_hip.h b/include/ipm_hip.h
--- a/include/ipm_hip.h
+++ b/include/ipm_hip.h
@@ -127,6 +127,7 @@
 int ipm_get_certificate(ipm_handle* h, double* y, double* z, double* x, double info[4]);
 int ipm_get_history(ipm_handle* h, ipm_iter_record* out, int32_t capacity, int32_t* count);
 int ipm_get_schedule(ipm_handle* h, int32_t out[12]);
+int ipm_get_schedule_words(ipm_handle* h, int32_t* out, int32_t capacity, int32_t* count);
 
 int ipm_order_rows(int64_t m, int64_t n, const int32_t* colptr, const int32_t* rowind, int32_t* perm, double info[8]);
 int ipm_get_factor_info(ipm_handle* h, int64_t out[8]);
@@ -143,6 +144,7 @@
 int ipm_get_factor(ipm_handle* h, double* L, int64_t ldl);
 int ipm_set_profiling(ipm_handle* h, int enable);
 int ipm_debug_get_stamps(ipm_handle* h, long long* out);
+int ipm_debug_at_pieces(int32_t nblk, int32_t layout[4], int32_t* pieces, int32_t capacity, int32_t* count);
 int ipm_debug_ff_schedule(int32_t nblk, int32_t q, int32_t workers, unsigned char* items, int32_t capacity, int32_t* count,
                           int32_t* tile_items, double sim_us[2]);
 int ipm_get_phase_ms(ipm_handle* h, double out[4]);
diff --git a/interiorpointmethod_amd/_lib.py b/interiorpointmethod_amd/_lib.py
--- a/interiorpointmethod_amd/_lib.py
+++ b/interiorpointmethod_amd/_lib.py
@@ -10,7 +10,7 @@
     "ipm_abi_version", "ipm_device_count", "ipm_default_options", "ipm_workspace_bytes", "ipm_workspace_bytes_csc", "ipm_workspace_bytes_opts",
     "ipm_create", "ipm_destroy", "ipm_last_error", "ipm_set_A_dense", "ipm_set_A_csc",
     "ipm_set_bc", "ipm_set_state", "ipm_get_state", "ipm_init_state", "ipm_init_state_mehrotra", "ipm_set_bounds", "ipm_set_bound_state", "ipm_get_bound_state", "ipm_equilibrate", "ipm_get_scaling", "ipm_newton_direction",
-    "ipm_iterate", "ipm_solve", "ipm_solve_batch", "ipm_solve_small_batch", "ipm_init_small_batch_mehrotra", "ipm_batch_create", "ipm_batch_destroy", "ipm_batch_last_error", "ipm_batch_add", "ipm_batch_step", "ipm_batch_stats", "ipm_get_history", "ipm_set_infeasibility_tol", "ipm_get_certificate", "ipm_get_schedule", "ipm_order_rows", "ipm_get_factor_info", "ipm_solve_linear", "ipm_lu_solve", "ipm_lu_factor", "ipm_normal_solve", "ipm_form_normal_matrix", "ipm_get_factor",
+    "ipm_iterate", "ipm_solve", "ipm_solve_batch", "ipm_solve_small_batch", "ipm_init_small_batch_mehrotra", "ipm_batch_create", "ipm_batch_destroy", "ipm_batch_last_error", "ipm_batch_add", "ipm_batch_step", "ipm_batch_stats", "ipm_get_history", "ipm_set_infeasibility_tol", "ipm_get_certificate", "ipm_get_schedule", "ipm_get_schedule_words", "ipm_debug_at_pieces", "ipm_order_rows", "ipm_get_factor_info", "ipm_solve_linear", "ipm_lu_solve", "ipm_lu_factor", "ipm_normal_solve", "ipm_form_normal_matrix", "ipm_get_factor",
     "ipm_set_profiling", "ipm_get_phase_ms", "ipm_debug_get_stamps", "ipm_debug_ff_schedule", "ipm_debug_ff_trace", "ipm_debug_get_block_inverse", "ipm_debug_ls_merge",
 ]
 
@@ -129,6 +129,8 @@
     lib.ipm_batch_stats.argtypes = [vp, i32, C.POINTER(Stats)]
     lib.ipm_get_history.argtypes = [vp, C.POINTER(IterRecord), i32, C.POINTER(i32)]
     lib.ipm_get_schedule.argtypes = [vp, C.POINTER(i32)]
+    lib.ipm_get_schedule_words.argtypes = [vp, C.POINTER(i32), i32, C.POINTER(i32)]
+    lib.ipm_debug_at_pieces.argtypes = [i32, C.POINTER(i32), C.POINTER(i32), i32, C.POINTER(i32)]
     lib.ipm_set_infeasibility_tol.argtypes = [vp, dbl, dbl]
     lib.ipm_get_certificate.argtypes = [vp, pd, pd, pd, pd]
     lib.ipm_order_rows.argtypes = [i64, i64, C.POINTER(i32), C.POINTER(i32), C.POINTER(i32), pd]
diff --git a/interiorpointmethod_amd/csrc/handoff.h b/interiorpointmethod_amd/csrc/handoff.h
--- a/interiorpointmethod_amd/csrc/handoff.h
+++ b/interiorpointmethod_amd/csrc/handoff.h
@@ -75,4 +75,8 @@
     return false;
 }
 
+__device__ __forceinline__ void handoff_signal_at_entry(unsigned* word, unsigned value) {
+    if (blockIdx.x == 0 && blockIdx.y == 0 && threadIdx.x == 0) __hip_atomic_store(word, value, __ATOMIC_RELAXED, __HIP_MEMORY_SCOPE_AGENT);
 }
+
+}
diff --git a/interiorpointmethod_amd/csrc/host_factor_solve.h b/interiorpointmethod_amd/csrc/host_factor_solve.h
--- a/interiorpointmethod_amd/csrc/host_factor_solve.h
+++ b/interiorpointmethod_amd/csrc/host_factor_solve.h
@@ -255,8 +255,9 @@
 }
 
 static void launch_dense_gemv_n(ipm_handle* h, const double* A, int64_t lda, int rows, int cols, const double* v, double sa,
-                                double sb, const double* add, double* out) {
-    launch_twin<LS_GEMV_N>(h, (unsigned)((rows + 3) / 4), {A, lda, rows, cols, v, sa, sb, add, out, &h->sc->done});
+                                double sb, const double* add, double* out, unsigned* signal = nullptr, unsigned value = 0) {
+    if (signal) hipLaunchKernelGGL(gemv_n_signal_kernel, dim3((unsigned)((rows + 3) / 4)), dim3(256), 0, h->stream, A, lda, rows, cols, v, sa, sb, add, out, &h->sc->done, signal, value);
+    else launch_twin<LS_GEMV_N>(h, (unsigned)((rows + 3) / 4), {A, lda, rows, cols, v, sa, sb, add, out, &h->sc->done});
 }
 
 static void enqueue_block_steps(ipm_handle* h, int k0, double* r, double* z, double* out) {
@@ -276,7 +277,29 @@
     }
 }
 
-static int enqueue_potrs_grouped(ipm_handle* h, double* r, double* out, hipEvent_t wait_last = nullptr) {
+struct AtPiece { int first_row, chunk0, chunk1; };
+static std::vector<AtPiece> at_piece_schedule(int64_t mp, int gsz, int nblk, int rc_chunks, int rows_per_chunk) {
+    std::vector<AtPiece> ev;
+    if (gsz <= 0 || nblk < gsz || rc_chunks <= 0 || rows_per_chunk <= 0 || (int64_t)rc_chunks * rows_per_chunk != mp || mp != (int64_t)nblk * NB) return ev;
+    const int nG = nblk / gsz;
+    const int64_t GR = (int64_t)gsz * NB;
+    int hi = rc_chunks;
+    auto event = [&](int64_t first) {
+        const int lo = (int)std::min<int64_t>(hi, (first + rows_per_chunk - 1) / rows_per_chunk);
+        ev.push_back({(int)first, lo, hi});
+        hi = lo;
+    };
+    if (nblk > nG * gsz) event(nG * GR);
+    for (int g = nG - 1; g >= 0; --g) event(g * GR);
+    return ev;
+}
+struct SweepHook {
+    unsigned* word;
+    unsigned base;
+    std::function<void(int)> released;
+};
+
+static int enqueue_potrs_grouped(ipm_handle* h, double* r, double* out, hipEvent_t wait_last = nullptr, const SweepHook* hook = nullptr) {
     const int GS = h->gsz;
     const int GR = GS * 128;
     const int nG = h->nblk / GS;
@@ -294,22 +317,31 @@
         }
     }
     enqueue_block_steps(h, nG * GS, r, z, out);
+    int e = 0;
+    bool pending = hook && h->nblk > nG * GS;
     for (int g = nG - 1; g >= 0; --g) {
-        launch_dense_gemv_n(h, h->gXT + (int64_t)g * GR * GR, GR, GR, GR, z + (int64_t)g * GR, 1.0, 0.0, nullptr, out + (int64_t)g * GR);
+        launch_dense_gemv_n(h, h->gXT + (int64_t)g * GR * GR, GR, GR, GR, z + (int64_t)g * GR, 1.0, 0.0, nullptr, out + (int64_t)g * GR,
+                            pending ? hook->word : nullptr, pending ? hook->base + (unsigned)e + 1u : 0u);
+        if (pending) { hook->released(e); ++e; pending = false; }
         int left = g * GR;
         const int c0 = h->use_env ? std::min(left, h->env_first[g * GS] * NB) : 0;
         left -= c0;
         if (left > 0) {
             const unsigned gx = (unsigned)((left + 511) / 512);
-            launch_twin<LS_GEMV_T>(h, gx * 16u, {h->B + (int64_t)g * GR * h->mp + c0, h->mp, GR / 16, left, out + (int64_t)g * GR, h->gPart, done, gx});
+            const LsArgs<LS_GEMV_T> t{h->B + (int64_t)g * GR * h->mp + c0, h->mp, GR / 16, left, out + (int64_t)g * GR, h->gPart, done, gx};
+            if (hook) {
+                hipLaunchKernelGGL(gemv_t_signal_kernel, dim3(gx, 16u), dim3(256), 0, h->stream, t.A, t.lda, t.rows_per_chunk, t.np, t.u, t.part, t.done,
+                                   hook->word, hook->base + (unsigned)e + 1u);
+                hook->released(e); ++e;
+            } else launch_twin<LS_GEMV_T>(h, gx * 16u, t);
             launch_twin<LS_SUB_PARTIALS>(h, (unsigned)((left + 255) / 256), {z + c0, h->gPart, left, 16, done});
-        }
-    }
-    HIP_TRY(h, hipGetLastError());
-    return IPM_OK;
-}
-
-static int enqueue_potrs(ipm_handle* h, double* r, double* out, hipEvent_t wait_last = nullptr) {
+        } else if (hook && g > 0) pending = true;
+    }
+    HIP_TRY(h, hipGetLastError());
+    return IPM_OK;
+}
+
+static int enqueue_potrs(ipm_handle* h, double* r, double* out, hipEvent_t wait_last = nullptr, const SweepHook* hook = nullptr) {
     if (sp_on(h)) {
         const int rm = std::max(16, h->sp_rmax);
         unsigned ep = ++h->sp_epoch;
@@ -326,7 +358,7 @@
         HIP_TRY(h, hipGetLastError());
         return IPM_OK;
     }
-    if (h->grouped_trsv) return enqueue_potrs_grouped(h, r, out, wait_last);
+    if (h->grouped_trsv) return enqueue_potrs_grouped(h, r, out, wait_last, hook);
     if (wait_last) HIP_TRY(h, hipStreamWaitEvent(h->stream, wait_last, 0));
     enqueue_block_steps(h, 0, r, h->t2, out);
     HIP_TRY(h, hipGetLastError());
diff --git a/interiorpointmethod_amd/csrc/host_handle.h b/interiorpointmethod_amd/csrc/host_handle.h
--- a/interiorpointmethod_amd/csrc/host_handle.h
+++ b/interiorpointmethod_amd/csrc/host_handle.h
@@ -12,6 +12,9 @@
     hipStream_t stream2 = nullptr;
     hipStream_t stream3 = nullptr;
     hipEvent_t ev_mid = nullptr, ev_res = nullptr, ev_grp = nullptr, ev_last = nullptr;
+    int stream_at = 1;
+    unsigned at_epoch = 0;
+    hipEvent_t ev_at = nullptr;
     std::vector<hipEvent_t> ev_crit, ev_bulk;
     hipEvent_t ev_fork = nullptr;
     int lookahead = 1;
@@ -166,6 +169,7 @@
 static inline bool wants_polling(const ipm_handle* h) { return lookahead_on(h) && h->flag_sync != 0; }
 static inline bool polls_device(const ipm_handle* h) { return wants_polling(h) && alone_on_device(h); }
 static inline unsigned* timeout_word(const ipm_handle* h) { return h->d_flags + 2 * (size_t)h->nblk; }
+static inline unsigned* at_progress_word(const ipm_handle* h) { return timeout_word(h) + 1; }
 static inline const int* factor_done(const ipm_handle* h) { return h->fdone ? h->fdone : &h->sc->done; }
 
 static std::atomic<int> g_pool_state[64];
diff --git a/interiorpointmethod_amd/csrc/host_iteration.h b/interiorpointmethod_amd/csrc/host_iteration.h
--- a/interiorpointmethod_amd/csrc/host_iteration.h
+++ b/interiorpointmethod_amd/csrc/host_iteration.h
@@ -1,10 +1,34 @@
 #pragma once
 static int enqueue_solve_direction(ipm_handle* h, hipEvent_t* ev, double* dy, int corr, hipEvent_t wait_last = nullptr) {
     if (ev) HIP_TRY(h, hipEventRecord(ev[0], h->stream));
-    int rc = enqueue_potrs(h, h->t1, dy, wait_last);
-    if (rc) return rc;
-    if (ev) HIP_TRY(h, hipEventRecord(ev[1], h->stream));
-    launch_gemv_t(h, dy);
+    std::vector<AtPiece> pieces;
+    if (stream_at_on(h)) pieces = at_piece_schedule(h->mp, h->gsz, h->nblk, h->rc_chunks, h->rows_per_chunk);
+    if (pieces.empty()) {
+        int rc = enqueue_potrs(h, h->t1, dy, wait_last);
+        if (rc) return rc;
+        if (ev) HIP_TRY(h, hipEventRecord(ev[1], h->stream));
+        launch_gemv_t(h, dy);
+    } else {
+        bool streamed = false;
+        SweepHook hook;
+        hook.word = at_progress_word(h); hook.base = h->at_epoch;
+        h->at_epoch += (unsigned)pieces.size();
+        hook.released = [&](int e) {
+            const AtPiece& p = pieces[(size_t)e];
+            if (p.chunk1 <= p.chunk0) return;
+            hipLaunchKernelGGL(ff_gate_kernel, dim3(1), dim3(64), 0, h->stream3, hook.word, hook.base + (unsigned)e + 1u, timeout_word(h), &h->sc->done);
+            launch_gemv_t_rows(h, dy, p.chunk0, p.chunk1, h->stream3);
+            streamed = true;
+        };
+        int rc = enqueue_potrs(h, h->t1, dy, wait_last, &hook);
+        if (rc) return rc;
+        if (ev) HIP_TRY(h, hipEventRecord(ev[1], h->stream));
+        launch_gemv_t_rows(h, dy, pieces.back().chunk0, pieces.back().chunk1, h->stream);
+        if (streamed) {
+            HIP_TRY(h, hipEventRecord(h->ev_at, h->stream3));
+            HIP_TRY(h, hipStreamWaitEvent(h->stream, h->ev_at, 0));
+        }
+    }
     launch_direction(h, corr);
     HIP_TRY(h, hipGetLastError());
     return IPM_OK;
@@ -107,6 +131,7 @@
 
 static void poll_fallback(ipm_handle* h) {
     if (h->spf) h->sp_serial = true;
+    h->stream_at = 0;
     if (h->ff_last) h->ff_enabled = 0;
     else h->flag_sync = 0;
     ++h->timeouts_recovered;
diff --git a/interiorpointmethod_amd/csrc/host_residuals.h b/interiorpointmethod_amd/csrc/host_residuals.h
--- a/interiorpointmethod_amd/csrc/host_residuals.h
+++ b/interiorpointmethod_amd/csrc/host_residuals.h
@@ -7,6 +7,12 @@
 static void launch_gemv_t(ipm_handle* h, const double* u, hipStream_t st = nullptr) {
     if (h->sparse) launch_twin<LS_SPMV_CSC_T>(h, (unsigned)((h->np + 15) / 16), {sparse_view(h), (int)h->np, u, h->atp, &h->sc->done}, st);
     else launch_untwinned(h, gemv_t_kernel, dim3((unsigned)((h->np + 511) / 512), (unsigned)h->rc_chunks), dim3(256), st, h->A, h->np, h->rows_per_chunk, (int)h->np, u, h->atp, &h->sc->done);
+}
+static void launch_gemv_t_rows(ipm_handle* h, const double* u, int chunk0, int chunk1, hipStream_t st) {
+    if (chunk1 <= chunk0) return;
+    const int64_t r0 = (int64_t)chunk0 * h->rows_per_chunk;
+    hipLaunchKernelGGL(gemv_t_kernel, dim3((unsigned)((h->np + 511) / 512), (unsigned)(chunk1 - chunk0)), dim3(256), 0, st ? st : h->stream,
+                       h->A + r0 * h->np, h->np, h->rows_per_chunk, (int)h->np, u + r0, h->atp + (int64_t)chunk0 * h->np, &h->sc->done);
 }
 
 template <LsType T> static void launch_vec_step(ipm_handle* h, void (*bounded)(VecArgs, BndArgs), hipStream_t st = nullptr) {
@@ -58,3 +64,6 @@
 static bool overlap_residuals(const ipm_handle* h) {
     return h->stream3 != nullptr && h->profiling < 2;
 }
+static bool stream_at_on(const ipm_handle* h) {
+    return h->stream_at != 0 && overlap_residuals(h) && h->grouped_trsv && !h->sparse && polls_device(h) && !h->ls_rec;
+}
diff --git a/interiorpointmethod_amd/csrc/ipm_api.hip b/interiorpointmethod_amd/csrc/ipm_api.hip
--- a/interiorpointmethod_amd/csrc/ipm_api.hip
+++ b/interiorpointmethod_amd/csrc/ipm_api.hip
@@ -7,6 +7,7 @@
 #include <string.h>
 
 #include <deque>
+#include <functional>
 #include <vector>
 
 #include "../../include/ipm_hip.h"
@@ -106,6 +107,17 @@
     if (const char* e = getenv("IPM_FF_CHAIN_MODE")) h->ff_chain_mode0 = atoi(e) == 0;
     if (const char* e = getenv("IPM_FF_REF_ENGINE")) h->ff_ref_engine = atoi(e) != 0;
     if (const char* e = getenv("IPM_FF_Q")) h->ff_q = std::max(1, std::min(16, atoi(e)));
+    if (const char* e = getenv("IPM_STREAM_AT")) h->stream_at = atoi(e);
+}
+
+static int group_size(int nblk, bool ragged) {
+    int gsz = 0;
+    if (nblk >= 2 * GS_MAX) { if (ragged || nblk % GS_MAX == 0) gsz = GS_MAX; }
+    else {
+        for (int p2 = GS_MAX; p2 >= 2; p2 /= 2) if (nblk % p2 == 0) { gsz = p2; break; }
+        if (ragged && nblk > GS_MAX && gsz < 4) gsz = GS_MAX;
+    }
+    return gsz;
 }
 
 extern "C" int ipm_create(int device, int64_t m, int64_t n, const ipm_options* opts, void* workspace,
@@ -209,15 +221,7 @@
     if (h->lockstep && h->ls_block_steps) h->grouped_trsv = 0;
     if (h->lockstep) h->ss_small_blocks = 1 << 20;
     if (h->no_dense) h->grouped_trsv = 0;
-    h->gsz = 0;
-    if (h->grouped_trsv) {
-        const bool ragged = h->ragged_groups;
-        if (h->nblk >= 2 * GS_MAX) { if (ragged || h->nblk % GS_MAX == 0) h->gsz = GS_MAX; }
-        else {
-            for (int p2 = GS_MAX; p2 >= 2; p2 /= 2) if (h->nblk % p2 == 0) { h->gsz = p2; break; }
-            if (ragged && h->nblk > GS_MAX && h->gsz < 4) h->gsz = GS_MAX;
-        }
-    }
+    h->gsz = h->grouped_trsv ? group_size(h->nblk, h->ragged_groups) : 0;
     if (h->gsz > 0) {
         const size_t nG = (size_t)h->nblk / h->gsz, GR = (size_t)h->gsz * 128;
         CREATE_TRY(dev_malloc(device, h->stream, (void**)&h->gXT, sizeof(double) * nG * GR * GR));
@@ -244,6 +248,7 @@
     CREATE_TRY(hipEventCreateWithFlags(&h->ev_res, hipEventDisableTiming));
     CREATE_TRY(hipEventCreateWithFlags(&h->ev_grp, hipEventDisableTiming));
     CREATE_TRY(hipEventCreateWithFlags(&h->ev_last, hipEventDisableTiming));
+    CREATE_TRY(hipEventCreateWithFlags(&h->ev_at, hipEventDisableTiming));
     if (h->ff_chain_mode0) {
         int rc_ = fail(nullptr, IPM_ERR_INVALID_ARG, "IPM_FF_CHAIN_MODE=0 is not supported (that structure of the fused launch was removed)");
         ipm_destroy(h);
@@ -282,6 +287,7 @@
     if (h->ev_res) (void)hipEventDestroy(h->ev_res);
     if (h->ev_grp) (void)hipEventDestroy(h->ev_grp);
     if (h->ev_last) (void)hipEventDestroy(h->ev_last);
+    if (h->ev_at) (void)hipEventDestroy(h->ev_at);
     if (h->stream2) (void)hipStreamDestroy(h->stream2);
     if (h->ev0) (void)hipEventDestroy(h->ev0);
     if (h->ev1) (void)hipEventDestroy(h->ev1);
@@ -518,14 +524,37 @@
     return IPM_OK;
 }
 
+static const int SCHEDULE_WORDS = 13;
+extern "C" int ipm_get_schedule_words(ipm_handle* h, int32_t* out, int32_t capacity, int32_t* count) {
+    if (!h || !out || capacity < 0) return fail(h, IPM_ERR_INVALID_ARG, "ipm_get_schedule_words: bad arguments");
+    const int live = live_on_device(h);
+    int32_t w[SCHEDULE_WORDS];
+    w[0] = h->nblk; w[1] = h->last_gs; w[2] = h->grouped_trsv;
+    w[3] = (may_poll(h) && live <= 1) ? 1 : 0;
+    w[4] = h->n_counter_steps; w[5] = h->n_event_steps; w[6] = h->use_env ? 1 : 0; w[7] = live;
+    w[8] = h->timeouts_recovered; w[9] = h->small ? 1 : 0;
+    w[10] = h->ff_last ? 1 : 0; w[11] = (h->spf && sp_level(h)) ? 1 : 0;
+    w[12] = stream_at_on(h) ? 1 : 0;
+    const int n = std::min<int>(capacity, SCHEDULE_WORDS);
+    memcpy(out, w, sizeof(int32_t) * (size_t)n);
+    if (count) *count = n;
+    return IPM_OK;
+}
 extern "C" int ipm_get_schedule(ipm_handle* h, int32_t out[12]) {
     if (!h || !out) return fail(h, IPM_ERR_INVALID_ARG, "ipm_get_schedule: bad arguments");
-    const int live = live_on_device(h);
-    out[0] = h->nblk; out[1] = h->last_gs; out[2] = h->grouped_trsv;
-    out[3] = (may_poll(h) && live <= 1) ? 1 : 0;
-    out[4] = h->n_counter_steps; out[5] = h->n_event_steps; out[6] = h->use_env ? 1 : 0; out[7] = live;
-    out[8] = h->timeouts_recovered; out[9] = h->small ? 1 : 0;
-    out[10] = h->ff_last ? 1 : 0; out[11] = (h->spf && sp_level(h)) ? 1 : 0;
+    return ipm_get_schedule_words(h, out, 12, nullptr);
+}
+
+extern "C" int ipm_debug_at_pieces(int32_t nblk, int32_t layout[4], int32_t* pieces, int32_t capacity, int32_t* count) {
+    if (nblk < 1 || nblk > (1 << 13) || !layout || !count) return fail(nullptr, IPM_ERR_INVALID_ARG, "ipm_debug_at_pieces: bad arguments");
+    const Layout L = make_layout((int64_t)nblk * NB, 64);
+    if (layout[0] <= 0) layout[0] = (int32_t)L.mp;
+    if (layout[1] <= 0) layout[1] = group_size(nblk, true);
+    if (layout[2] <= 0) layout[2] = L.rc_chunks;
+    if (layout[3] <= 0) layout[3] = L.rows_per_chunk;
+    const std::vector<AtPiece> ev = at_piece_schedule(layout[0], layout[1], nblk, layout[2], layout[3]);
+    *count = (int32_t)ev.size();
+    if (pieces) for (size_t e = 0; e < ev.size() && (int64_t)e < capacity; ++e) { pieces[3 * e] = ev[e].first_row; pieces[3 * e + 1] = ev[e].chunk0; pieces[3 * e + 2] = ev[e].chunk1; }
     return IPM_OK;
 }
 
diff --git a/interiorpointmethod_amd/csrc/vector_ops.h b/interiorpointmethod_amd/csrc/vector_ops.h
--- a/interiorpointmethod_amd/csrc/vector_ops.h
+++ b/interiorpointmethod_amd/csrc/vector_ops.h
@@ -2,6 +2,7 @@
 #include <hip/hip_runtime.h>
 #include <stdint.h>
 #include "gemm_nt_f64.h"
+#include "handoff.h"
 #include "iteration_rules.h"
 
 namespace ipm {
@@ -99,6 +100,20 @@
 __global__ __launch_bounds__(256) void gemv_t_kernel(const double* __restrict__ A, int64_t lda, int rows_per_chunk,
                                                      int np, const double* __restrict__ u, double* part,
                                                      const int* done) { gemv_t_kernel_body(A, lda, rows_per_chunk, np, u, part, done, blockIdx.x, blockIdx.y); }
+
+__global__ __launch_bounds__(256) void gemv_n_signal_kernel(const double* __restrict__ A, int64_t lda, int mp,
+                                                            int np, const double* __restrict__ v, double sa,
+                                                            double sb, const double* __restrict__ add,
+                                                            double* out, const int* done, unsigned* progress, unsigned value) {
+    handoff_signal_at_entry(progress, value);
+    gemv_n_kernel_body(A, lda, mp, np, v, sa, sb, add, out, done, blockIdx.x, gridDim.x);
+}
+__global__ __launch_bounds__(256) void gemv_t_signal_kernel(const double* __restrict__ A, int64_t lda, int rows_per_chunk,
+                                                            int np, const double* __restrict__ u, double* part,
+                                                            const int* done, unsigned* progress, unsigned value) {
+    handoff_signal_at_entry(progress, value);
+    gemv_t_kernel_body(A, lda, rows_per_chunk, np, u, part, done, blockIdx.x, blockIdx.y);
+}
 
 struct VecArgs {
     int m, n, np, rc_chunks;
diff --git a/interiorpointmethod_amd/handle.py b/interiorpointmethod_amd/handle.py
--- a/interiorpointmethod_amd/handle.py
+++ b/interiorpointmethod_amd/handle.py
@@ -239,10 +239,10 @@
                 "normalization": float(info[1]), "violation": float(info[2]), "k": int(info[3])}
 
     def schedule(self):
-        out = (C.c_int32 * 12)()
-        self._check(self._lib.ipm_get_schedule(self._h, out))
+        out = (C.c_int32 * 13)()
+        self._check(self._lib.ipm_get_schedule_words(self._h, out, 13, None))
         keys = ("blocks", "group_steps", "grouped_trsv", "device_polling", "counter_steps", "event_steps", "envelope",
-                "live_handles", "timeouts_recovered", "fused_small", "fused_factor", "sparse_level_mode")
+                "live_handles", "timeouts_recovered", "fused_small", "fused_factor", "sparse_level_mode", "stream_at")
         return dict(zip(keys, (int(v) for v in out)))
 
     def factor_info(self):
```

Result: faster. 274.6 iterations/s (median of 6 runs) (+1.2%).
